# forsaken628/katib

Measured on AMD Instinct MI355X. Metric: darts_cifar10_search_wall_clock_s, lower is better.
Workload: dtype fp32; 1 GPU; model=darts-cnn-cifar10 supernet (b5: C=4, L=2, N=3, stem x1, 6 primitives + none), global_batch=128, per_gpu_batch=128, parallelism=dp1, epochs=2, steps_per_epoch=196, ops=hip, hip_graph=True, sync_bn=False, hessian=concurrent

## Files before the change

### katib_amd/csrc/hip/darts_bind.cpp

```cpp
#include <torch/extension.h>
#include <c10/hip/HIPStream.h>

#include "darts_ops.h"

using namespace katib_hip;
using at::Tensor;
using OptT = c10::optional<Tensor>;

namespace {

hipStream_t cur_stream() { return c10::hip::getCurrentHIPStream().stream(); }

void check_f32(const Tensor& t, const char* name) {
  TORCH_CHECK(t.is_cuda(), name, " must be a GPU tensor");
  TORCH_CHECK(t.scalar_type() == at::kFloat, name, " must be float32");
  TORCH_CHECK(t.is_contiguous(), name, " must be contiguous");
}

constexpr at::ScalarType kZType = kZbf16 ? at::kBFloat16 : at::kFloat;

void check_z(const Tensor& t, const char* name) {
  TORCH_CHECK(t.is_cuda(), name, " must be a GPU tensor");
  TORCH_CHECK(t.scalar_type() == kZType, name, " must be ", kZbf16 ? "bfloat16" : "float32",
              " (the per-op intermediates' storage type of this build)");
  TORCH_CHECK(t.is_contiguous(), name, " must be contiguous");
}

zt* zptr(const Tensor& t) { return reinterpret_cast<zt*>(t.data_ptr()); }

template <typename T>
T* ptr_or_null(const OptT& t) {
  return t.has_value() && t->defined() ? t->data_ptr<T>() : nullptr;
}

BNRef make_bn(const py::tuple& b, int C) {
  BNRef r{};
  TORCH_CHECK(b.size() == 8, "bn tuple has 8 fields");
  OptT sums = b[0].cast<OptT>(), rm = b[1].cast<OptT>(), rv = b[2].cast<OptT>();
  r.rep = b[6].cast<int>();
  r.rstride = b[7].cast<int>();
  TORCH_CHECK(r.rep >= 1 && r.rep <= kRep && r.rstride >= 2 * C, "bn replica layout");
  if (sums.has_value() && sums->defined()) {
    TORCH_CHECK(sums->scalar_type() == at::kDouble && sums->is_contiguous() &&
                    sums->numel() >= (int64_t)(r.rep - 1) * r.rstride + 2 * C,
                "bn sums must be f64 with rep x rstride doubles");
  }
  r.sums = ptr_or_null<double>(sums);
  r.rmean = ptr_or_null<float>(rm);
  r.rvar = ptr_or_null<float>(rv);
  r.inv_count = b[3].cast<float>();
  r.eval = b[4].cast<bool>() ? 1 : 0;
  r.eps = b[5].cast<float>();
  r.C = C;
  TORCH_CHECK(r.eval ? (r.rmean && r.rvar) : (r.sums != nullptr), "bn reference lacks its statistics");
  return r;
}

int64_t storage_doubles_after(const Tensor& t) {
  return (int64_t)(t.storage().nbytes() / sizeof(double)) - t.storage_offset();
}

int64_t gs_numel(const py::tuple& t) {
  return t[1].cast<Tensor>().numel();
}

GradSrc make_gs(const py::tuple& t, int C) {
  GradSrc g{};
  TORCH_CHECK(t.size() == 9, "grad-source tuple has 9 fields");
  Tensor gt = t[0].cast<Tensor>(), zt = t[1].cast<Tensor>();
  check_f32(gt, "g");
  check_z(zt, "z");
  g.g = gt.data_ptr<float>();
  g.z = zptr(zt);
  OptT s1 = t[2].cast<OptT>(), s2 = t[3].cast<OptT>();
  g.S1 = ptr_or_null<double>(s1);
  g.S2 = ptr_or_null<double>(s2);
  g.bn = make_bn(t[4].cast<py::tuple>(), C);
  g.eval = g.bn.eval;
  TORCH_CHECK(g.eval || (g.S1 && g.S2), "training-mode BN backward needs S1/S2 reductions");
  OptT w = t[5].cast<OptT>();
  g.w = ptr_or_null<float>(w);
  g.widx = t[6].cast<int>();
  g.rep = t[7].cast<int>();
  g.rstride = t[8].cast<int>();
  TORCH_CHECK(g.rep >= 1 && g.rep <= kRep, "replicas");
  if (!g.eval) {
    for (int k = 2; k <= 3; ++k) {
      Tensor sv = *t[k].cast<OptT>();
      TORCH_CHECK(sv.scalar_type() == at::kDouble &&
                      storage_doubles_after(sv) >= (int64_t)(g.rep - 1) * g.rstride + C,
                  "S1/S2 replicas exceed their buffer");
    }
  }
  return g;
}

struct CtrRing {
  unsigned* base = nullptr;
  int size = 0;
  int cursor = 0;
};
CtrRing g_ring[64];
bool g_selffold = false;

void set_selffold(bool on) { g_selffold = on; }

int cur_device() {
  int d = 0;
  TORCH_CHECK(hipGetDevice(&d) == hipSuccess, "hipGetDevice");
  return d;
}

void set_fold_counters(Tensor t) {
  TORCH_CHECK(t.is_cuda() && t.scalar_type() == at::kInt && t.is_contiguous() && t.numel() >= 4 * kFoldCtrSlot,
              "fold counters: contiguous int32 GPU tensor of >= 4 launch slots");
  const int d = t.get_device();
  TORCH_CHECK(d >= 0 && d < 64, "device index");
  g_ring[d] = CtrRing{reinterpret_cast<unsigned*>(t.data_ptr<int>()), (int)(t.numel() / kFoldCtrSlot), 0};
}

bool selffold_ready() { return g_selffold && g_ring[cur_device()].base != nullptr; }

void tail_begin(FoldTail& t) {
  t.nseg = 0;
  t.ctr = nullptr;
  if (!g_selffold) return;
  CtrRing& r = g_ring[cur_device()];
  if (!r.base) return;
  t.ctr = r.base + (size_t)r.cursor * kFoldCtrSlot;
  r.cursor = (r.cursor + 1) % r.size;
}

void tail_add(FoldTail& t, double* p, int n, int rs) {
  if (!t.ctr || !p) return;
  for (int s = 0; s < t.nseg; ++s)
    if (t.p[s] == p) {
      t.n[s] = std::max(t.n[s], n);
      return;
    }
  TORCH_CHECK(t.nseg < kTailSeg, "self-fold: too many reduction segments in one launch");
  t.p[t.nseg] = p;
  t.n[t.nseg] = n;
  t.rs[t.nseg] = rs;
  ++t.nseg;
}

void tail_close(FoldTail& t) {
  if (t.nseg == 0) t.ctr = nullptr;
}

int pick_chunk(int C, int per_channel_floats, int fixed_floats) {
  const int budget = 16384 - fixed_floats;
  int ch = C;
  while (ch > 1 && ch * per_channel_floats > budget) ch = (ch + 1) / 2;
  return std::max(ch, 1);
}

template <typename Bt>
void check_batch(const std::vector<py::tuple>& calls) {
  TORCH_CHECK(!calls.empty() && (int)calls.size() <= Bt::kCap, "batch of 1..", Bt::kCap, " edges");
}

#define SAME_SHAPE(b, fld) TORCH_CHECK(b.e[i].fld == b.e[0].fld, "edges in a batch must share " #fld)

static bool fill_dwpw(const py::tuple& t, DwPwFwdArgs& a, int64_t K, int64_t dil, int64_t S, int64_t pad, int nentries,
                      bool use_mfma) {
  Tensor x = t[0].cast<Tensor>(), dw = t[1].cast<Tensor>(), pw = t[2].cast<Tensor>();
  auto inbn = t[3].cast<c10::optional<py::tuple>>();
  Tensor d = t[4].cast<Tensor>(), z = t[5].cast<Tensor>();
  OptT stats = t[6].cast<OptT>();
  const bool has_inbn = t[3].cast<c10::optional<py::tuple>>().has_value();
  if (has_inbn) check_z(x, "x (previous stage z)");
  else check_f32(x, "x");
  check_f32(dw, "dw"); check_f32(pw, "pw"); check_z(d, "d"); check_z(z, "z");
  TORCH_CHECK(x.dim() == 4, "x must be NCHW");
  TORCH_CHECK((K == 3 || K == 5) && (dil == 1 || dil == 2) && (S == 1 || S == 2), "K in {3,5}, dil, S in {1,2}");
  const int N = x.size(0), C = x.size(1), H = x.size(2), W = x.size(3);
  const int Ho = z.size(2), Wo = z.size(3);
  TORCH_CHECK(dw.numel() == C * K * K && pw.numel() == C * C, "weight shapes");
  TORCH_CHECK(z.size(0) == N && z.size(1) == C && d.sizes() == z.sizes(), "output shapes");
  TORCH_CHECK(64 % Wo == 0 && Ho % (64 / Wo) == 0, "tile constraint: 64 % Wo == 0 and Ho % (64/Wo) == 0");
  TORCH_CHECK(C <= kMaxC, "C too large");
  TORCH_CHECK(Ho == (H + 2 * pad - dil * (K - 1) - 1) / S + 1, "output height mismatch");
  a.x = x.data_ptr(); a.dw = dw.data_ptr<float>(); a.pw = pw.data_ptr<float>();
  a.d = zptr(d); a.z = zptr(z); a.stats = ptr_or_null<double>(stats);
  if (a.stats) TORCH_CHECK(stats->scalar_type() == at::kDouble && stats->numel() >= kRep * 2 * C, "stats f64 [kRep][2C]");
  a.N = N; a.C = C; a.H = H; a.W = W; a.Ho = Ho; a.Wo = Wo; a.pad = pad;
  const int TR = 64 / Wo;
  const int IR = (TR - 1) * S + (K - 1) * dil + 1, IW = (Wo - 1) * S + (K - 1) * dil + 1;
  a.chunk = pick_chunk(C, IR * IW, C * 64 + 4 * C);
  if (C == 4 || C == 8 || C == 16) {
    int nb = std::max(1, std::min(Ho / 4, 2048 / std::max(N * nentries, 1)));
    auto band_bytes = [&](int b) {
      const int BR = (Ho + b - 1) / b;
      return (size_t)C * ((BR - 1) * S + (K - 1) * dil + 1) * (W + 2 * pad) * sizeof(float);
    };
    while (band_bytes(nb) > 65536 && nb < Ho) ++nb;
    a.chunk = nb;
  }
  a.use_mfma = (use_mfma && C % 16 == 0) ? 1 : 0;
  const bool prebn = inbn.has_value();
  if (prebn) a.inbn = make_bn(*inbn, C);
  a.variant = (((K == 5) * 4 + (dil == 2) * 2 + (S == 2)) * 4) + (prebn ? 2 : 0);
  return prebn;
}

void dwpw_fwd(std::vector<py::tuple> calls, int64_t K, int64_t dil, int64_t S, int64_t pad, bool use_mfma) {
  check_batch<DwPwFwdBatch>(calls);
  DwPwFwdBatch bt{};
  bt.n = calls.size();
  bool prebn = false;
  for (int i = 0; i < bt.n; ++i) {
    const bool pb = fill_dwpw(calls[i], bt.e[i], K, dil, S, pad, bt.n, use_mfma);
    if (i == 0) prebn = pb;
    TORCH_CHECK(pb == prebn, "edges in a batch must agree on the input BN");
    SAME_SHAPE(bt, N); SAME_SHAPE(bt, C); SAME_SHAPE(bt, H); SAME_SHAPE(bt, W);
  }
  tail_begin(bt.tail);
  for (int i = 0; i < bt.n; ++i) tail_add(bt.tail, bt.e[i].stats, 2 * bt.e[i].C, 2 * bt.e[i].C);
  tail_close(bt.tail);
  launch_dwpw_fwd(bt, K, dil, S, prebn, cur_stream());
}

static void fill_dwpw_multi(const std::vector<py::tuple>& calls, DwPwMultiBatch& bt, int64_t* kk, int64_t* dd,
                            int64_t* ss, int64_t* pp, bool* pre) {
  TORCH_CHECK(!calls.empty() && (int)calls.size() <= DwPwMultiBatch::kCap, "1..", DwPwMultiBatch::kCap, " entries");
  bt.n = calls.size();
  for (int i = 0; i < bt.n; ++i) {
    const py::tuple& t = calls[i];
    TORCH_CHECK(t.size() == 11, "dwpw_fwd_multi entry: (x, dw, pw, inbn, d, z, stats, K, dil, S, pad)");
    kk[i] = t[7].cast<int64_t>(); dd[i] = t[8].cast<int64_t>(); ss[i] = t[9].cast<int64_t>(); pp[i] = t[10].cast<int64_t>();
    pre[i] = fill_dwpw(t, bt.e[i], kk[i], dd[i], ss[i], pp[i], bt.n, true);
    SAME_SHAPE(bt, N); SAME_SHAPE(bt, C); SAME_SHAPE(bt, Ho); SAME_SHAPE(bt, Wo);
  }
  tail_begin(bt.tail);
  for (int i = 0; i < bt.n; ++i) tail_add(bt.tail, bt.e[i].stats, 2 * bt.e[i].C, 2 * bt.e[i].C);
  tail_close(bt.tail);
}

void dwpw_fwd_multi(std::vector<py::tuple> calls) {
  DwPwMultiBatch bt{};
  int64_t kk[DwPwMultiBatch::kCap], dd[DwPwMultiBatch::kCap], ss[DwPwMultiBatch::kCap], pp[DwPwMultiBatch::kCap];
  bool pre[DwPwMultiBatch::kCap];
  fill_dwpw_multi(calls, bt, kk, dd, ss, pp, pre);
  if (launch_dwpw_multi(bt, cur_stream())) return;
  for (int i = 0; i < bt.n; ++i) {
    DwPwFwdBatch one{};
    one.n = 1;
    one.tail = bt.tail;
    fill_dwpw(calls[i], one.e[0], kk[i], dd[i], ss[i], pp[i], 1, true);
    launch_dwpw_fwd(one, kk[i], dd[i], ss[i], pre[i], cur_stream());
  }
}

void pw_fwd(std::vector<py::tuple> calls, int64_t S) {
  check_batch<PwFwdBatch>(calls);
  PwFwdBatch bt{};
  bt.n = calls.size();
  for (int i = 0; i < bt.n; ++i) {
    const py::tuple& t = calls[i];
    Tensor x = t[0].cast<Tensor>(), pw = t[1].cast<Tensor>(), z = t[2].cast<Tensor>();
    OptT stats = t[3].cast<OptT>();
    const int co_off = t[4].cast<int>(), off = t[5].cast<int>();
    check_f32(x, "x"); check_f32(pw, "pw"); check_z(z, "z");
    const bool nm = x.dim() == 5;
    const int xnodes = nm ? x.size(0) : 1;
    const int N = nm ? x.size(1) : x.size(0), Cin = nm ? x.size(0) * x.size(2) : x.size(1);
    const int H = x.size(nm ? 3 : 2), W = x.size(nm ? 4 : 3);
    const int Cout = pw.size(0), Ho = z.size(2), Wo = z.size(3);
    TORCH_CHECK(pw.size(1) == Cin && co_off + Cout <= z.size(1) && z.size(0) == N, "pw shapes");
    TORCH_CHECK((Ho * Wo) % 64 == 0, "Ho*Wo must be a multiple of 64");
    TORCH_CHECK(Cin <= kMaxC && Cout <= kMaxC, "channels");
    PwFwdArgs& a = bt.e[i];
    a.x = x.data_ptr<float>(); a.pw = pw.data_ptr<float>(); a.z = zptr(z);
    a.stats = ptr_or_null<double>(stats);
    if (a.stats)
      TORCH_CHECK(stats->scalar_type() == at::kDouble && stats->numel() >= kRep * 2 * z.size(1), "stats [kRep][2Ctot]");
    a.N = N; a.Cin = Cin; a.Cout = Cout; a.CoutTotal = z.size(1); a.co_off = co_off;
    a.H = H; a.W = W; a.Ho = Ho; a.Wo = Wo; a.S = S; a.off = off; a.relu = 1; a.xnodes = xnodes;
    SAME_SHAPE(bt, N); SAME_SHAPE(bt, Cin); SAME_SHAPE(bt, Cout); SAME_SHAPE(bt, Ho); SAME_SHAPE(bt, Wo);
  }
  tail_begin(bt.tail);
  for (int i = 0; i < bt.n; ++i) tail_add(bt.tail, bt.e[i].stats, 2 * bt.e[i].CoutTotal, 2 * bt.e[i].CoutTotal);
  tail_close(bt.tail);
  launch_pw_fwd(bt, cur_stream());
}

static void fill_pool_fwd(const std::vector<py::tuple>& calls, int64_t S_all, PoolFwdBatch& bt) {
  check_batch<PoolFwdBatch>(calls);
  bt.n = calls.size();
  for (int i = 0; i < bt.n; ++i) {
    const py::tuple& t = calls[i];
    const int64_t S = S_all > 0 ? S_all : t[6].cast<int64_t>();
    TORCH_CHECK(S == 1 || S == 2, "pool stride must be 1 or 2");
    bt.e[i].S = (int)S;
    Tensor x = t[0].cast<Tensor>(), zavg = t[1].cast<Tensor>(), zmax = t[2].cast<Tensor>();
    OptT sa = t[3].cast<OptT>(), sm = t[4].cast<OptT>(), amax = t[5].cast<OptT>();
    check_f32(x, "x"); check_z(zavg, "zavg"); check_z(zmax, "zmax");
    PoolFwdArgs& a = bt.e[i];
    if (amax.has_value() && amax->defined()) {
      TORCH_CHECK(amax->scalar_type() == at::kByte && amax->numel() == zmax.numel(), "amax must be uint8 like zmax");
      a.amax = amax->data_ptr<uint8_t>();
    }
    a.x = x.data_ptr<float>(); a.zavg = zptr(zavg); a.zmax = zptr(zmax);
    a.stats_avg = ptr_or_null<double>(sa); a.stats_max = ptr_or_null<double>(sm);
    if (a.stats_avg) TORCH_CHECK(sa->scalar_type() == at::kDouble && sa->numel() >= kRep * 2 * x.size(1), "stats");
    if (a.stats_max) TORCH_CHECK(sm->scalar_type() == at::kDouble && sm->numel() >= kRep * 2 * x.size(1), "stats");
    a.N = x.size(0); a.C = x.size(1); a.H = x.size(2); a.W = x.size(3); a.Ho = zavg.size(2); a.Wo = zavg.size(3);
    TORCH_CHECK(a.Ho == (a.H - 1) / S + 1 && zmax.sizes() == zavg.sizes(), "pool shapes");
    SAME_SHAPE(bt, N); SAME_SHAPE(bt, C);
    if (S_all > 0) { SAME_SHAPE(bt, H); SAME_SHAPE(bt, W); }
  }
  tail_begin(bt.tail);
  for (int i = 0; i < bt.n; ++i) {
    tail_add(bt.tail, bt.e[i].stats_avg, 2 * bt.e[i].C, 2 * bt.e[i].C);
    tail_add(bt.tail, bt.e[i].stats_max, 2 * bt.e[i].C, 2 * bt.e[i].C);
  }
  tail_close(bt.tail);
}

static void pool_fwd_impl(std::vector<py::tuple> calls, int64_t S_all) {
  PoolFwdBatch bt{};
  fill_pool_fwd(calls, S_all, bt);
  if (S_all > 0) launch_pool_fwd(bt, S_all, cur_stream());
  else launch_pool_fwd_multi(bt, cur_stream());
}

void pool_fwd(std::vector<py::tuple> calls, int64_t S) { pool_fwd_impl(calls, S); }
void pool_fwd_multi(std::vector<py::tuple> calls) { pool_fwd_impl(calls, -1); }

void dwpw_pool_fwd_multi(std::vector<py::tuple> dcalls, std::vector<py::tuple> pcalls) {
  DwPwMultiBatch bt{};
  int64_t kk[DwPwMultiBatch::kCap], dd[DwPwMultiBatch::kCap], ss[DwPwMultiBatch::kCap], pp[DwPwMultiBatch::kCap];
  bool pre[DwPwMultiBatch::kCap];
  fill_dwpw_multi(dcalls, bt, kk, dd, ss, pp, pre);
  PoolFwdBatch pb{};
  fill_pool_fwd(pcalls, -1, pb);
  if (launch_dwpw_pool_multi(bt, pb, cur_stream())) return;
  dwpw_fwd_multi(dcalls);
  launch_pool_fwd_multi(pb, cur_stream());
}

void combine_fwd(std::vector<py::tuple> calls, OptT gamma, OptT beta, Tensor out, double momentum,
                 bool update_running, bool accumulate) {
  check_f32(out, "out");
  check_batch<CombineFwdBatch>(calls);
  CombineFwdBatch bt{};
  bt.n = calls.size();
  const int C = out.size(1);
  TORCH_CHECK(C <= kMaxC, "C too large");
  TORCH_CHECK((int64_t)2 * bt.n * kMaxOps * C * 4 <= 65536, "combine LDS budget exceeded");
  for (int e = 0; e < bt.n; ++e) {
    const py::tuple& t = calls[e];
    auto zs = t[0].cast<std::vector<Tensor>>();
    auto bns = t[1].cast<std::vector<py::tuple>>();
    auto widx = t[2].cast<std::vector<int64_t>>();
    OptT w = t[3].cast<OptT>();
    const int id_idx = t[4].cast<int>();
    OptT xid = t[5].cast<OptT>();
    auto upd = t[6].cast<std::vector<py::tuple>>();
    TORCH_CHECK(zs.size() == bns.size() && zs.size() == widx.size() && (int)zs.size() <= kMaxOps, "ops");
    CombineFwdArgs& a = bt.e[e];
    a.N = out.size(0); a.C = C; a.HW = out.size(2) * out.size(3);
    a.nops = zs.size();
    for (size_t k = 0; k < zs.size(); ++k) {
      check_z(zs[k], "z");
      TORCH_CHECK(zs[k].sizes() == out.sizes(), "combine input shape");
      a.z[k] = zptr(zs[k]);
      a.bn[k] = make_bn(bns[k], C);
      a.widx[k] = widx[k];
    }
    TORCH_CHECK((int)upd.size() <= kMaxUpd, "too many update-only BN layers");
    a.nupd = upd.size();
    for (size_t k = 0; k < upd.size(); ++k) a.upd[k] = make_bn(upd[k], C);
    a.w = ptr_or_null<float>(w); a.id_idx = id_idx; a.xid = ptr_or_null<float>(xid);
    if (a.xid) {
      check_f32(*xid, "xid");
      TORCH_CHECK(xid->sizes() == out.sizes(), "identity shape");
    }
    a.gamma = ptr_or_null<float>(gamma); a.beta = ptr_or_null<float>(beta);
    a.out = out.data_ptr<float>(); a.momentum = momentum; a.update_running = update_running;
    a.accumulate = accumulate;
  }
  launch_combine_fwd(bt, cur_stream());
}

void combine_bwd_reduce(std::vector<py::tuple> calls) {
  check_batch<CombineBwdBatch>(calls);
  CombineBwdBatch bt{};
  bt.n = calls.size();
  for (int i = 0; i < bt.n; ++i) {
    const py::tuple& t = calls[i];
    Tensor dout = t[0].cast<Tensor>();
    auto zs = t[1].cast<std::vector<Tensor>>();
    auto bns = t[2].cast<std::vector<py::tuple>>();
    OptT xid = t[3].cast<OptT>();
    Tensor red = t[4].cast<Tensor>();
    auto widx = t[5].cast<std::vector<int64_t>>();
    const int id_idx = t[6].cast<int>();
    OptT gw = t[7].cast<OptT>();
    check_f32(dout, "dout");
    TORCH_CHECK(red.scalar_type() == at::kDouble, "red must be f64");
    CombineBwdArgs& a = bt.e[i];
    a.N = dout.size(0); a.C = dout.size(1); a.HW = dout.size(2) * dout.size(3);
    a.nops = zs.size();
    a.rstride = (a.nops + 1) * a.C + 1;
    TORCH_CHECK(a.nops <= kMaxOps && red.numel() >= (int64_t)kRep * a.rstride, "red size [kRep][(nops+1)C+1]");
    for (int k = 0; k < a.nops; ++k) {
      TORCH_CHECK(zs[k].sizes() == dout.sizes(), "z shape");
      check_z(zs[k], "z");
      a.z[k] = zptr(zs[k]);
      a.bn[k] = make_bn(bns[k], a.C);
    }
    a.dout = dout.data_ptr<float>(); a.xid = ptr_or_null<float>(xid); a.red = red.data_ptr<double>();
    a.gw = ptr_or_null<double>(gw); a.id_idx = id_idx;
    if (a.gw) {
      TORCH_CHECK(gw->scalar_type() == at::kDouble && gw->numel() % kRep == 0, "gw must be f64 [kRep][nw]");
      a.gwstride = gw->numel() / kRep;
      TORCH_CHECK((int)widx.size() == a.nops, "widx per op");
      for (int k = 0; k < a.nops; ++k) {
        TORCH_CHECK(widx[k] >= 0 && widx[k] < a.gwstride, "widx out of range");
        a.widx[k] = widx[k];
      }
      TORCH_CHECK(id_idx < a.gwstride, "id_idx out of range");
    }
    SAME_SHAPE(bt, N); SAME_SHAPE(bt, C); SAME_SHAPE(bt, HW);
  }
  tail_begin(bt.tail);
  for (int i = 0; i < bt.n; ++i) {
    tail_add(bt.tail, bt.e[i].red, bt.e[i].rstride, bt.e[i].rstride);
    tail_add(bt.tail, bt.e[i].gw, bt.e[i].gwstride, bt.e[i].gwstride);
  }
  tail_close(bt.tail);
  launch_combine_bwd_reduce(bt, cur_stream());
}

void check_grad_sink(const OptT& gW, int64_t numel, int64_t gstride) {
  if (!gW.has_value() || !gW->defined()) return;
  TORCH_CHECK(gW->scalar_type() == at::kFloat && gW->is_contiguous() && gW->numel() == numel, "gW shape");
  TORCH_CHECK(gstride == 0 || (gstride >= numel && (int64_t)(gW->storage().nbytes() / sizeof(float)) -
                                                           gW->storage_offset() >= (kRep - 1) * gstride + numel),
              "gW replicas exceed their buffer");
}

void pw_bwd(std::vector<py::tuple> calls, int64_t S, int64_t mode, bool need_dx) {
  check_batch<PwBwdBatch>(calls);
  PwBwdBatch bt{};
  bt.n = calls.size();
  for (int i = 0; i < bt.n; ++i) {
    const py::tuple& t = calls[i];
    py::tuple gs = t[0].cast<py::tuple>();
    Tensor pw = t[1].cast<Tensor>();
    OptT ain = t[2].cast<OptT>();
    Tensor x = t[3].cast<Tensor>();
    OptT dd = t[4].cast<OptT>(), gx = t[5].cast<OptT>(), gW = t[6].cast<OptT>();
    const int co_off = t[7].cast<int>(), off = t[8].cast<int>();
    const int64_t gstride = t[9].cast<int64_t>();
    const bool overwrite = t.size() > 10 && t[10].cast<bool>();
    check_f32(pw, "pw");
    if (mode != 0) check_f32(x, "x");
    PwBwdArgs& a = bt.e[i];
    a.overwrite = overwrite;
    TORCH_CHECK(!overwrite || (mode == 1 && S == 1 && off == 0), "gx overwrite needs the stride-1 full-coverage form");
    const int Cout = pw.size(0), Cin = pw.size(1);
    Tensor g = gs[0].cast<Tensor>();
    a.N = g.size(0); a.CoutTotal = g.size(1); a.Ho = g.size(2); a.Wo = g.size(3);
    a.gs = make_gs(gs, a.CoutTotal);
    a.Cin = Cin; a.Cout = Cout; a.co_off = co_off; a.S = S; a.off = off; a.mode = mode;
    a.need_dx = need_dx;
    const bool nm = mode != 0 && x.dim() == 5;
    a.xnodes = nm ? x.size(0) : 1;
    a.H = x.size(nm ? 3 : 2); a.W = x.size(nm ? 4 : 3);
    if (mode != 0) {
      TORCH_CHECK(x.numel() == (int64_t)a.N * Cin * a.H * a.W && (!nm || x.size(1) == a.N),
                  "pw_bwd: x must be [N][Cin][H][W] or node-major [nodes][N][Cin/nodes][H][W]");
      if (gx.has_value() && gx->defined()) TORCH_CHECK(gx->sizes() == x.sizes(), "pw_bwd: gx must have the shape of x");
    }
    TORCH_CHECK(Cin * Cout <= 8192, "pw_bwd supports Cin*Cout <= 8192");
    TORCH_CHECK((a.Ho * a.Wo) % 64 == 0, "Ho*Wo % 64");
    a.pw = pw.data_ptr<float>(); a.x = mode != 0 ? x.data_ptr<float>() : nullptr;
    if (ain.has_value() && ain->defined()) check_z(*ain, "ain (depthwise output d)");
    a.ain = ain.has_value() && ain->defined() ? zptr(*ain) : nullptr;
    a.dd = ptr_or_null<float>(dd); a.gx = ptr_or_null<float>(gx);
    a.gW = ptr_or_null<float>(gW);
    if (mode == 0) {
      TORCH_CHECK(a.ain && (!need_dx || a.dd), "mode 0 needs ain (and dd)");
    } else {
      TORCH_CHECK(!need_dx || a.gx, "mode 1 needs gx");
    }
    check_grad_sink(gW, (int64_t)Cin * Cout, gstride);
    a.gstride = gstride;
    SAME_SHAPE(bt, N); SAME_SHAPE(bt, Cin); SAME_SHAPE(bt, Cout); SAME_SHAPE(bt, Ho); SAME_SHAPE(bt, Wo);
  }
  launch_pw_bwd(bt, cur_stream());
}

void dw_bwd_fill(std::vector<py::tuple>& calls, DwBwdBatch& bt, const int64_t* Ks, const int64_t* dils,
                 const int64_t* Ss, bool& prebn);

void dw_bwd(std::vector<py::tuple> calls, int64_t K, int64_t dil, int64_t S, int64_t pad) {
  check_batch<DwBwdBatch>(calls);
  DwBwdBatch bt{};
  int64_t Ks[DwBwdBatch::kCap], Ds[DwBwdBatch::kCap], Ss[DwBwdBatch::kCap];
  for (int i = 0; i < DwBwdBatch::kCap; ++i) Ks[i] = K, Ds[i] = dil, Ss[i] = S;
  TORCH_CHECK(pad == (K - 1) / 2 * dil, "dw_bwd padding must be 'same'");
  bool prebn = false;
  dw_bwd_fill(calls, bt, Ks, Ds, Ss, prebn);
  tail_close(bt.tail);
  launch_dw_bwd(bt, K, dil, S, prebn, cur_stream());
}

void dw_bwd_multi(std::vector<py::tuple> calls) {
  check_batch<DwBwdBatch>(calls);
  DwBwdBatch bt{};
  int64_t Ks[DwBwdBatch::kCap], Ds[DwBwdBatch::kCap], Ss[DwBwdBatch::kCap];
  for (size_t i = 0; i < calls.size(); ++i) {
    TORCH_CHECK(calls[i].size() == 10 || calls[i].size() == 12,
                "dw_bwd_multi entry: (x, inbn, dw, dd, gout, gW, red, gstride, overwrite, K[, dil, S])");
    Ks[i] = calls[i][9].cast<int64_t>();
    Ds[i] = calls[i].size() == 12 ? calls[i][10].cast<int64_t>() : 1;
    Ss[i] = calls[i].size() == 12 ? calls[i][11].cast<int64_t>() : 1;
    TORCH_CHECK((Ks[i] == 3 || Ks[i] == 5) && (Ds[i] == 1 || Ds[i] == 2) && (Ss[i] == 1 || Ss[i] == 2),
                "K in {3, 5}, dil and S in {1, 2}");
  }
  bool prebn = false;
  dw_bwd_fill(calls, bt, Ks, Ds, Ss, prebn);
  for (int i = 0; i < bt.n; ++i) {
    TORCH_CHECK(prebn || bt.e[i].overwrite, "dw_bwd_multi: input-gradient entries must own (overwrite) their output");
    TORCH_CHECK(!prebn || (Ds[i] == 1 && Ss[i] == 1), "dw_bwd_multi: input-BN entries are stride-1 separable stages");
    bt.e[i].variant = dw_bwd_variant((int)Ks[i], (int)Ds[i], (int)Ss[i], prebn);
  }
  for (int i = 0; i < bt.n; ++i)
    for (int j = i + 1; j < bt.n; ++j) TORCH_CHECK(bt.e[i].gout != bt.e[j].gout, "dw_bwd_multi entries share an output");
  tail_close(bt.tail);
  if (launch_dw_bwd_multi(bt, cur_stream())) return;
  for (int v = 0; v < 16; ++v) {
    DwBwdBatch one{};
    one.tail = bt.tail;
    for (int i = 0; i < bt.n; ++i)
      if (bt.e[i].variant == v) one.e[one.n++] = bt.e[i];
    if (one.n) launch_dw_bwd(one, dw_variant_k(v), dw_variant_dil(v), dw_variant_s(v), prebn, cur_stream());
  }
}

void dw_bwd_fill(std::vector<py::tuple>& calls, DwBwdBatch& bt, const int64_t* Ks, const int64_t* dils,
                 const int64_t* Ss, bool& prebn) {
  bt.n = calls.size();
  bool has_gw = false;
  for (int i = 0; i < bt.n; ++i) {
    const py::tuple& t = calls[i];
    const int64_t K = Ks[i], dil = dils[i], S = Ss[i], pad = (K - 1) / 2 * dil;
    Tensor x = t[0].cast<Tensor>();
    auto inbn = t[1].cast<c10::optional<py::tuple>>();
    Tensor dw = t[2].cast<Tensor>(), dd = t[3].cast<Tensor>(), gout = t[4].cast<Tensor>();
    OptT gW = t[5].cast<OptT>(), red = t[6].cast<OptT>();
    const int64_t gstride = t[7].cast<int64_t>();
    const bool overwrite = t[8].cast<bool>();
    if (inbn.has_value()) check_z(x, "x (stage-1 z)");
    else check_f32(x, "x");
    check_f32(dw, "dw"); check_f32(dd, "dd"); check_f32(gout, "gout");
    DwBwdArgs& a = bt.e[i];
    a.N = x.size(0); a.C = x.size(1); a.H = x.size(2); a.W = x.size(3); a.Ho = dd.size(2); a.Wo = dd.size(3);
    TORCH_CHECK(64 % a.Wo == 0 && a.Ho % (64 / a.Wo) == 0, "tile constraint");
    TORCH_CHECK(a.H == a.Ho * S && a.W == a.Wo * S, "dw_bwd needs H == Ho*S");
    TORCH_CHECK(gout.sizes() == x.sizes(), "gout shape");
    TORCH_CHECK(dw.numel() == a.C * K * K && dd.size(1) == a.C, "dw_bwd weight / grad shapes");
    a.x = x.data_ptr(); a.dw = dw.data_ptr<float>(); a.dd = dd.data_ptr<float>();
    a.gout = gout.data_ptr<float>(); a.gW = ptr_or_null<float>(gW); a.red = ptr_or_null<double>(red);
    check_grad_sink(gW, (int64_t)a.C * K * K, gstride);
    a.gstride = gstride;
    a.overwrite = overwrite;
    if (a.red) TORCH_CHECK(red->scalar_type() == at::kDouble && red->numel() >= kRep * 2 * a.C, "red [kRep][2C]");
    a.pad = pad;
    if (i == 0) {
      prebn = inbn.has_value();
      has_gw = a.gW != nullptr;
    }
    TORCH_CHECK(inbn.has_value() == prebn, "edges in a batch must agree on the input BN");
    TORCH_CHECK((a.gW != nullptr) == has_gw, "edges in a batch must agree on weight-gradient sinks");
    TORCH_CHECK(!(prebn && overwrite), "overwrite applies to the input-gradient (non-BN) form");
    const int TR = 64 / a.Wo, r = (K - 1) / 2 * dil, h = (r + S - 1) / S, OR = TR + 2 * h;
    const int IR = (TR - 1) * S + (K - 1) * dil + 1, IW = (a.Wo - 1) * S + (K - 1) * dil + 1;
    a.chunk = pick_chunk(a.C, OR * a.Wo + IR * IW, 4 * a.C + (a.gW ? a.C * (int)(K * K) : 0));
    if (prebn) a.inbn = make_bn(*inbn, a.C);
    SAME_SHAPE(bt, N); SAME_SHAPE(bt, C); SAME_SHAPE(bt, Ho); SAME_SHAPE(bt, Wo);
  }
  tail_begin(bt.tail);
  if (prebn)
    for (int i = 0; i < bt.n; ++i) tail_add(bt.tail, bt.e[i].red, 2 * bt.e[i].C, 2 * bt.e[i].C);
}

static void pool_bwd_impl(std::vector<py::tuple> calls, int64_t S_all) {
  check_batch<PoolBwdBatch>(calls);
  PoolBwdBatch bt{};
  bt.n = calls.size();
  for (int i = 0; i < bt.n; ++i) {
    const py::tuple& t = calls[i];
    const int64_t S = S_all > 0 ? S_all : t[9].cast<int64_t>();
    TORCH_CHECK(S == 1 || S == 2, "pool stride must be 1 or 2");
    bt.e[i].S = (int)S;
    auto ga = t[0].cast<c10::optional<py::tuple>>(), gm = t[1].cast<c10::optional<py::tuple>>();
    Tensor x = t[2].cast<Tensor>();
    OptT dout_id = t[3].cast<OptT>(), w = t[4].cast<OptT>();
    const int id_idx = t[5].cast<int>();
    Tensor gx = t[6].cast<Tensor>();
    OptT amax = t[7].cast<OptT>();
    check_f32(x, "x"); check_f32(gx, "gx");
    PoolBwdArgs& a = bt.e[i];
    a.N = x.size(0); a.C = x.size(1); a.H = x.size(2); a.W = x.size(3);
    a.Ho = (a.H - 1) / S + 1; a.Wo = (a.W - 1) / S + 1;
    TORCH_CHECK(a.Ho * a.Wo <= 8192, "pool_bwd stages one output plane in LDS (Ho*Wo <= 8192)");
    TORCH_CHECK(gx.sizes() == x.sizes(), "gx shape");
    TORCH_CHECK(!gm.has_value() || (amax.has_value() && amax->defined() && amax->scalar_type() == at::kByte &&
                                    amax->numel() == (int64_t)a.N * a.C * a.Ho * a.Wo),
                "max-pool backward needs the uint8 argmax from pool_fwd");
    if (amax.has_value() && amax->defined()) a.amax = amax->data_ptr<uint8_t>();
    if (ga.has_value()) a.ga = make_gs(*ga, a.C);
    if (gm.has_value()) a.gm = make_gs(*gm, a.C);
    a.x = x.data_ptr<float>(); a.dout_id = ptr_or_null<float>(dout_id); a.w = ptr_or_null<float>(w);
    if (a.dout_id) TORCH_CHECK(dout_id->sizes() == x.sizes(), "identity gradient shape");
    a.id_idx = id_idx; a.gx = gx.data_ptr<float>();
    a.overwrite = t[8].cast<bool>();
    if (S_all <= 0 && t.size() > 10) {
      auto ex = t[10].cast<std::vector<Tensor>>();
      TORCH_CHECK(ex.size() <= 4, "pool_bwd: at most 4 extra gradient parts");
      a.nextra = ex.size();
      for (size_t j = 0; j < ex.size(); ++j) {
        check_f32(ex[j], "extra");
        TORCH_CHECK(ex[j].sizes() == gx.sizes(), "extra gradient part shape");
        TORCH_CHECK(ex[j].data_ptr() != gx.data_ptr(), "extra part aliases gx");
        a.extra[j] = ex[j].data_ptr<float>();
      }
    }
    SAME_SHAPE(bt, N); SAME_SHAPE(bt, C);
    if (S_all > 0) { SAME_SHAPE(bt, H); SAME_SHAPE(bt, W); }
  }
  for (int i = 0; i < bt.n; ++i)
    for (int j = i + 1; j < bt.n; ++j) TORCH_CHECK(bt.e[i].gx != bt.e[j].gx, "pool_bwd entries share a gx buffer");
  if (S_all > 0) launch_pool_bwd(bt, S_all, cur_stream());
  else launch_pool_bwd_multi(bt, cur_stream());
}

void pool_bwd(std::vector<py::tuple> calls, int64_t S) { pool_bwd_impl(calls, S); }

bool edge_bwd(std::vector<py::tuple> calls) {
  check_batch<EdgeBwdBatch>(calls);
  EdgeBwdBatch bt{};
  bt.n = calls.size();
  const int Ks[4] = {3, 5, 3, 5};
  for (int i = 0; i < bt.n; ++i) {
    const py::tuple& t = calls[i];
    TORCH_CHECK(t.size() == 11, "edge_bwd entry: (x, gx, overwrite, convs, ga, gm, amax, dout_id, w, id_idx, S)");
    Tensor x = t[0].cast<Tensor>(), gx = t[1].cast<Tensor>();
    check_f32(x, "x"); check_f32(gx, "gx");
    TORCH_CHECK(x.dim() == 4 && gx.sizes() == x.sizes(), "gx shape");
    EdgeBwdArgs& a = bt.e[i];
    a.x = x.data_ptr<float>(); a.gx = gx.data_ptr<float>(); a.overwrite = t[2].cast<bool>();
    a.S = t[10].cast<int>();
    TORCH_CHECK(a.S == 1 || a.S == 2, "stride");
    a.N = x.size(0); a.C = x.size(1); a.H = x.size(2); a.W = x.size(3);
    a.Ho = (a.H - 1) / a.S + 1; a.Wo = (a.W - 1) / a.S + 1;
    auto convs = t[3].cast<std::vector<py::object>>();
    TORCH_CHECK(convs.size() == 4, "4 conv slots");
    for (int v = 0; v < 4; ++v) {
      if (convs[v].is_none()) continue;
      py::tuple c = convs[v].cast<py::tuple>();
      Tensor dw = c[0].cast<Tensor>(), dd = c[1].cast<Tensor>();
      OptT gW = c[2].cast<OptT>();
      const int64_t gstride = c[3].cast<int64_t>();
      check_f32(dw, "dw"); check_f32(dd, "dd");
      TORCH_CHECK(dw.numel() == a.C * Ks[v] * Ks[v], "dw shape");
      TORCH_CHECK(dd.dim() == 4 && dd.size(0) == a.N && dd.size(1) == a.C && dd.size(2) == a.Ho && dd.size(3) == a.Wo,
                  "dd shape");
      check_grad_sink(gW, (int64_t)a.C * Ks[v] * Ks[v], gstride);
      a.dw[v] = dw.data_ptr<float>(); a.dd[v] = dd.data_ptr<float>(); a.gW[v] = ptr_or_null<float>(gW);
      a.gstride[v] = gstride;
      a.conv_mask |= 1 << v;
    }
    auto ga = t[4].cast<c10::optional<py::tuple>>(), gm = t[5].cast<c10::optional<py::tuple>>();
    OptT amax = t[6].cast<OptT>(), dout_id = t[7].cast<OptT>(), w = t[8].cast<OptT>();
    if (ga.has_value()) {
      a.ga = make_gs(*ga, a.C);
      TORCH_CHECK(gs_numel(*ga) == (int64_t)a.N * a.C * a.Ho * a.Wo, "avg-pool gradient source shape");
    }
    if (gm.has_value()) {
      a.gm = make_gs(*gm, a.C);
      TORCH_CHECK(gs_numel(*gm) == (int64_t)a.N * a.C * a.Ho * a.Wo, "max-pool gradient source shape");
      TORCH_CHECK(amax.has_value() && amax->defined() && amax->scalar_type() == at::kByte &&
                      amax->numel() == (int64_t)a.N * a.C * a.Ho * a.Wo,
                  "max-pool backward needs the uint8 argmax from pool_fwd");
      a.amax = amax->data_ptr<uint8_t>();
    }
    a.dout_id = ptr_or_null<float>(dout_id); a.w = ptr_or_null<float>(w); a.id_idx = t[9].cast<int>();
    if (a.dout_id) {
      check_f32(*dout_id, "dout_id");
      TORCH_CHECK(dout_id->sizes() == x.sizes() && a.S == 1, "identity gradient shape");
    }
    SAME_SHAPE(bt, N); SAME_SHAPE(bt, C);
  }
  for (int i = 0; i < bt.n; ++i)
    for (int j = i + 1; j < bt.n; ++j) TORCH_CHECK(bt.e[i].gx != bt.e[j].gx, "edge_bwd entries share a gx buffer");
  return launch_edge_bwd(bt, cur_stream());
}
void pool_bwd_multi(std::vector<py::tuple> calls) { pool_bwd_impl(calls, -1); }

void fold_rows(Tensor buf) {
  check_f32(buf, "buf");
  TORCH_CHECK(buf.dim() == 2, "buf must be [rows][n]");
  FoldArgs a{};
  a.buf = buf.data_ptr<float>();
  a.rows = buf.size(0);
  a.n = buf.size(1);
  launch_fold_rows(a, cur_stream());
}

void fold_f64(std::vector<py::tuple> segs) {
  TORCH_CHECK(!segs.empty() && (int)segs.size() <= kMaxSeg, "1..kMaxSeg segments");
  FoldF64Args a{};
  a.nseg = segs.size();
  for (int k = 0; k < a.nseg; ++k) {
    Tensor t = segs[k][0].cast<Tensor>();
    int n = segs[k][1].cast<int>(), rs = segs[k][2].cast<int>();
    TORCH_CHECK(t.is_cuda() && t.scalar_type() == at::kDouble && t.is_contiguous(), "fold segment must be f64");
    TORCH_CHECK(n >= 1 && rs >= n && t.numel() >= (int64_t)(kRep - 1) * rs + n, "fold segment size");
    a.p[k] = t.data_ptr<double>();
    a.n[k] = n;
    a.rstride[k] = rs;
    a.total += n;
  }
  launch_fold_f64(a, cur_stream());
}

}

void register_xgmi(py::module& m);
void register_conv(py::module& m);
void register_transformer(py::module& m);
void register_batchnorm(py::module& m);
void register_mlp(py::module& m);
void register_stem(py::module& m);
void register_enas(py::module& m);
void register_dwconv(py::module& m);
void register_darts_optim(py::module& m);
void register_darts_head(py::module& m);
void register_resnet(py::module& m);

PYBIND11_MODULE(TORCH_EXTENSION_NAME, m) {
  m.doc() = "katib_amd HIP kernels for gfx950 (DARTS edge ops, implicit-GEMM conv, transformer, xGMI all-reduce)";
  m.def("dwpw_fwd", &dwpw_fwd);
  m.def("pw_fwd", &pw_fwd);
  m.def("pool_fwd", &pool_fwd);
  m.def("combine_fwd", &combine_fwd);
  m.def("combine_bwd_reduce", &combine_bwd_reduce);
  m.def("pw_bwd", &pw_bwd);
  m.def("dw_bwd", &dw_bwd);
  m.def("dw_bwd_multi", &dw_bwd_multi, "separable second-stage depthwise backward of mixed kernel size in one launch");
  m.def("pool_bwd", &pool_bwd);
  m.def("dwpw_fwd_multi", &dwpw_fwd_multi, "mixed (K, dil, S) dw-pw entries of one node stage in one launch");
  m.def("pool_fwd_multi", &pool_fwd_multi, "stride-1 and stride-2 pools in one launch");
  m.def("dwpw_pool_fwd_multi", &dwpw_pool_fwd_multi, "a node's stage-1 dw-pw entries and its pools in one launch");
  m.def("pool_bwd_multi", &pool_bwd_multi, "stride-1 and stride-2 pool backward in one launch");
  m.def("edge_bwd", &edge_bwd, "whole input gradient of a node's edges (convs, pools, identity) in one launch");
  m.def("set_max_blocks", &set_max_blocks);
  m.def("stamps_arm", [](int kind, int call, torch::Tensor buf) {
    TORCH_CHECK(!buf.defined() || kind == 0 || (buf.is_cuda() && buf.scalar_type() == torch::kInt64 &&
                                               buf.is_contiguous() && buf.numel() >= 65536 * 8),
                "stamps_arm: int64 CUDA buffer of >= 65536 * 8 entries");
    stamps_arm(kind, call, kind == 0 ? nullptr : reinterpret_cast<unsigned long long*>(buf.data_ptr<int64_t>()));
  }, "diagnostic build: phase-stamp the call-th launch of kind (StampKind) into buf[wg * 8 + phase]");
  m.def("stamps_compiled", &stamps_compiled);
  m.def("fold_rows", &fold_rows);
  m.def("fold_f64", &fold_f64);
  m.def("set_fold_counters", &set_fold_counters, "register the current device's self-fold counter ring (int32, zeroed)");
  m.def("selffold_ready", &selffold_ready, "launches on the current device fold their own f64 replicas");
  m.def("set_selffold", &set_selffold, "turn self-folding launches on / off (default off: measured slower)");
  m.attr("REP") = kRep;
  m.attr("ZBF16") = kZbf16;
  m.def("max_blocks", &max_blocks);
  register_xgmi(m);
  register_conv(m);
  register_transformer(m);
  register_batchnorm(m);
  register_enas(m);
  register_dwconv(m);
  register_mlp(m);
  register_stem(m);
  register_darts_optim(m);
  register_darts_head(m);
  register_resnet(m);
}
```

### katib_amd/csrc/hip/darts_ops.h

```cpp
#pragma once
#include <hip/hip_runtime.h>
#include <hip/hip_bf16.h>

namespace katib_hip {

#ifdef KATIB_DARTS_ZBF16
typedef __hip_bfloat16 zt;
constexpr bool kZbf16 = true;
#else
typedef float zt;
constexpr bool kZbf16 = false;
#endif
typedef float zf4 __attribute__((ext_vector_type(4)));

__device__ __forceinline__ float z2f(float v) { return v; }
__device__ __forceinline__ float z2f(__hip_bfloat16 v) { return __bfloat162float(v); }
__device__ __forceinline__ void zput(float* p, float v) { *p = v; }
__device__ __forceinline__ void zput(__hip_bfloat16* p, float v) { *p = __float2bfloat16(v); }
__device__ __forceinline__ zf4 zld4(const float* p) { return *reinterpret_cast<const zf4*>(p); }
__device__ __forceinline__ zf4 zld4(const __hip_bfloat16* p) {
  const uint2 u = *reinterpret_cast<const uint2*>(p);
  return zf4{__uint_as_float(u.x << 16), __uint_as_float(u.x & 0xffff0000u), __uint_as_float(u.y << 16),
             __uint_as_float(u.y & 0xffff0000u)};
}
__device__ __forceinline__ void zst4(float* p, zf4 v) { *reinterpret_cast<zf4*>(p) = v; }
__device__ __forceinline__ void zst4(__hip_bfloat16* p, zf4 v) {
  __hip_bfloat16 b[4] = {__float2bfloat16(v.x), __float2bfloat16(v.y), __float2bfloat16(v.z), __float2bfloat16(v.w)};
  *reinterpret_cast<uint2*>(p) = *reinterpret_cast<const uint2*>(b);
}

__host__ __device__ __forceinline__ size_t plane_off(int n, int c, int N, int C, int nodes, size_t HW) {
  if (nodes <= 1) return ((size_t)n * C + c) * HW;
  const int Cn = C / nodes, k = c / Cn;
  return (((size_t)k * N + n) * Cn + (c - k * Cn)) * HW;
}

constexpr int kMaxOps = 8;
constexpr int kMaxUpd = 4;
constexpr int kMaxC = 256;
#ifndef KATIB_HIP_REP
#define KATIB_HIP_REP 32
#endif
constexpr int kRep = KATIB_HIP_REP;

struct BNRef {
  const double* sums;
  float* rmean;
  float* rvar;
  float inv_count;
  float eps;
  int eval;
  int C;
  int rep;
  int rstride;
};

struct GradSrc {
  const float* g;
  const zt* z;
  const double* S1;
  const double* S2;
  BNRef bn;
  const float* w;
  int widx;
  int eval;
  int rep;
  int rstride;
};

struct DwPwFwdArgs {
  const void* x;
  BNRef inbn; const float* dw; const float* pw;
  zt* d; zt* z; double* stats;
  int N, C, H, W, Ho, Wo, pad, chunk, use_mfma;
  int variant;
  int nblk;
  int vout = 0;
};

struct PwFwdArgs {
  const void* x;
  const float* pw; zt* z; double* stats;
  int N, Cin, Cout, CoutTotal, co_off, H, W, Ho, Wo, S, off;
  int relu;
  int xnodes;
};

struct PoolFwdArgs {
  const float* x; zt* zavg; zt* zmax; double* stats_avg; double* stats_max; unsigned char* amax;
  int N, C, H, W, Ho, Wo;
  int S, nblk;
};

struct CombineFwdArgs {
  const zt* z[kMaxOps]; BNRef bn[kMaxOps]; int widx[kMaxOps]; int nops;
  BNRef upd[kMaxUpd]; int nupd;
  const float* w; int id_idx; const float* xid; const float* gamma; const float* beta;
  float* out; int N, C, HW; float momentum; int update_running; int accumulate;
};

struct CombineBwdArgs {
  const float* dout; const zt* z[kMaxOps]; BNRef bn[kMaxOps]; int nops;
  const float* xid; double* red; int N, C, HW;
  double* gw; int widx[kMaxOps]; int id_idx;
  int rstride, gwstride;
};

struct PwBwdArgs {
  GradSrc gs; const float* pw; const zt* ain; const float* x; float* dd; float* gx; float* gW;
  int gstride;
  int N, Cin, Cout, CoutTotal, co_off, H, W, Ho, Wo, S, off, mode, need_dx;
  int overwrite;
  int xnodes;
};

struct DwBwdArgs {
  const void* x;
  BNRef inbn; const float* dw; const float* dd; float* gout; float* gW; double* red;
  int gstride;
  int N, C, H, W, Ho, Wo, pad, chunk;
  int overwrite;
  int variant, nbands, nblk;
  int vin = 0;
};
constexpr int dw_bwd_variant(int K, int dil, int S, bool prebn) {
  return (((K == 5) * 4 + (dil == 2) * 2 + (S == 2)) << 1) | (prebn ? 1 : 0);
}
constexpr int dw_variant_k(int v) { return (v >> 3) & 1 ? 5 : 3; }
constexpr int dw_variant_dil(int v) { return (v >> 2) & 1 ? 2 : 1; }
constexpr int dw_variant_s(int v) { return (v >> 1) & 1 ? 2 : 1; }
constexpr bool dw_variant_prebn(int v) { return v & 1; }

struct FoldArgs {
  float* buf; int n; int rows;
};

constexpr int kMaxSeg = 128;
struct FoldF64Args {
  double* p[kMaxSeg]; int n[kMaxSeg]; int rstride[kMaxSeg]; int nseg; int total;
};

struct PoolBwdArgs {
  GradSrc ga; GradSrc gm; const float* x; const float* dout_id; const float* w; int id_idx; float* gx;
  const unsigned char* amax;
  const float* extra[4]; int nextra;
  int overwrite;
  int N, C, H, W, Ho, Wo;
  int S;
};

constexpr int kTailSeg = 16;
constexpr int kFoldShards = 32;
constexpr int kFoldCtrStride = 32;
constexpr int kFoldCtrSlot = (1 + kFoldShards) * kFoldCtrStride;
struct FoldTail {
  unsigned* ctr;
  int nseg;
  double* p[kTailSeg];
  int n[kTailSeg];
  int rs[kTailSeg];
};

template <typename A, int M>
struct Batch {
  A e[M];
  int n;
  FoldTail tail;
  static constexpr int kCap = M;
};
using DwPwFwdBatch = Batch<DwPwFwdArgs, 16>;
using CombineFwdBatch = Batch<CombineFwdArgs, 4>;
using PwFwdBatch = Batch<PwFwdArgs, 32>;
using PoolFwdBatch = Batch<PoolFwdArgs, 16>;
using CombineBwdBatch = Batch<CombineBwdArgs, 8>;
using PwBwdBatch = Batch<PwBwdArgs, 32>;
using DwBwdBatch = Batch<DwBwdArgs, 40>;
using PoolBwdBatch = Batch<PoolBwdArgs, 16>;
using DwPwMultiBatch = Batch<DwPwFwdArgs, 40>;

struct EdgeBwdArgs {
  const float* x; float* gx; int overwrite;
  const float* dw[4]; const float* dd[4]; float* gW[4]; int gstride[4]; int conv_mask;
  GradSrc ga; GradSrc gm; const unsigned char* amax;
  const float* dout_id; const float* w; int id_idx;
  int N, C, H, W, Ho, Wo, S, nb, nblk;
};
using EdgeBwdBatch = Batch<EdgeBwdArgs, 4>;
constexpr size_t kKernargMax = 24576;
static_assert(sizeof(EdgeBwdBatch) <= kKernargMax, "edge_bwd batch exceeds the kernarg budget");
static_assert(sizeof(DwPwFwdBatch) <= kKernargMax && sizeof(CombineFwdBatch) <= kKernargMax &&
                  sizeof(PwFwdBatch) <= kKernargMax && sizeof(PoolFwdBatch) <= kKernargMax &&
                  sizeof(CombineBwdBatch) <= kKernargMax && sizeof(PwBwdBatch) <= kKernargMax &&
                  sizeof(DwBwdBatch) <= kKernargMax && sizeof(PoolBwdBatch) <= kKernargMax &&
                  sizeof(DwPwMultiBatch) <= kKernargMax,
              "kernel argument batches exceed the kernarg budget");

void launch_dwpw_fwd(const DwPwFwdBatch& b, int K, int dil, int S, bool prebn, hipStream_t st);
void launch_dw_bwd(const DwBwdBatch& b, int K, int dil, int S, bool prebn, hipStream_t st);
bool launch_dw_bwd_multi(DwBwdBatch b, hipStream_t st);
void launch_pw_fwd(const PwFwdBatch& b, hipStream_t st);
void launch_pool_fwd(const PoolFwdBatch& b, int S, hipStream_t st);
void launch_pool_bwd(const PoolBwdBatch& b, int S, hipStream_t st);
bool launch_dwpw_multi(DwPwMultiBatch b, hipStream_t st);
void launch_pool_fwd_multi(PoolFwdBatch b, hipStream_t st);
struct PoolFwdEntries {
  PoolFwdArgs e[PoolFwdBatch::kCap];
  int n;
};
static_assert(sizeof(DwPwMultiBatch) + sizeof(PoolFwdEntries) <= kKernargMax, "kernarg budget");
bool launch_dwpw_pool_multi(DwPwMultiBatch b, const PoolFwdBatch& pb, hipStream_t st);
void launch_pool_bwd_multi(const PoolBwdBatch& b, hipStream_t st);
void launch_combine_fwd(const CombineFwdBatch& b, hipStream_t st);
bool launch_edge_bwd(EdgeBwdBatch b, hipStream_t st);
void launch_combine_bwd_reduce(const CombineBwdBatch& b, hipStream_t st);
void launch_pw_bwd(const PwBwdBatch& b, hipStream_t st);
int max_blocks();
void launch_fold_rows(const FoldArgs& a, hipStream_t st);
void launch_fold_f64(const FoldF64Args& a, hipStream_t st);
void set_max_blocks(int n);
void stamps_arm(int kind, int call, unsigned long long* buf);
bool stamps_compiled();

}
```

### katib_amd/csrc/hip/darts_ops_dev.h

```cpp
#pragma once
#include <hip/hip_runtime.h>

#include <algorithm>
#include <cmath>
#include <cstdint>
#include <cstdlib>

#include "darts_ops.h"

namespace katib_hip {

int max_blocks();

#ifdef KATIB_HIP_STAMPS
static __device__ unsigned long long* g_stamps = nullptr;
#define KSTAMP(k)                                                                          \
  do {                                                                                     \
    unsigned long long* _sp = g_stamps;                                                    \
    if (_sp != nullptr && threadIdx.x == 0) {                                              \
      const unsigned _wg = blockIdx.y * gridDim.x + blockIdx.x;                            \
      if (_wg < 65536u) _sp[(size_t)_wg * 8 + (k)] = __builtin_amdgcn_s_memrealtime();     \
    }                                                                                      \
  } while (0)
bool stamp_take(int kind);
unsigned long long* stamp_buffer();
#define KSTAMP_ARM(kind, st)                                                               \
  const bool _stamp_armed = stamp_take(kind);                                              \
  if (_stamp_armed) {                                                                      \
    static unsigned long long* _on;                                                        \
    _on = stamp_buffer();                                                                  \
    (void)hipMemcpyToSymbolAsync(HIP_SYMBOL(g_stamps), &_on, sizeof(_on), 0, hipMemcpyHostToDevice, st); \
  }
#define KSTAMP_DISARM(st)                                                                  \
  if (_stamp_armed) {                                                                      \
    static unsigned long long* _off = nullptr;                                             \
    (void)hipMemcpyToSymbolAsync(HIP_SYMBOL(g_stamps), &_off, sizeof(_off), 0, hipMemcpyHostToDevice, st); \
  }
#else
#define KSTAMP(k)
#define KSTAMP_ARM(kind, st)
#define KSTAMP_DISARM(st)
#endif
enum StampKind { kStampDwBwd = 1, kStampDwPw = 2, kStampPoolBwd = 3, kStampPoolFwd = 4, kStampCombineFwd = 5,
                 kStampCombineBwd = 6, kStampPwBwd = 7 };
#define KEEP_WEIGHT_READS_LOCAL() asm volatile("" ::: "memory")
__host__ __device__ constexpr int plane_head_floats(int C) { return (C * 25 + C * C + 3) & ~3; }
__host__ __device__ constexpr int dwb_head_floats(int C) { return (2 * C * 25 + 3) & ~3; }
__host__ __device__ constexpr int lds_pitch(int w) {
  return (((w + 3) & ~3) >> 2) & 1 ? ((w + 3) & ~3) : ((w + 3) & ~3) + 4;
}
int vec_mask();

__device__ __forceinline__ void sum_replicas(const double* p, int rep, int rs, int off2, double& s, double& s2) {
  s = 0.0;
  s2 = 0.0;
  for (int r0 = 0; r0 < rep; r0 += 8) {
    double a[8], b[8];
#pragma unroll
    for (int u = 0; u < 8; ++u) {
      const bool ok = r0 + u < rep;
      a[u] = ok ? p[(size_t)(r0 + u) * rs] : 0.0;
      b[u] = ok ? p[(size_t)(r0 + u) * rs + off2] : 0.0;
    }
#pragma unroll
    for (int u = 0; u < 8; ++u) {
      s += a[u];
      s2 += b[u];
    }
  }
}

__device__ __forceinline__ void bn_moments(const BNRef& b, int c, double& m, double& v) {
  double s, s2;
  sum_replicas(b.sums + c, b.rep, b.rstride, b.C, s, s2);
  m = s * (double)b.inv_count;
  v = s2 * (double)b.inv_count - m * m;
  if (v < 0) v = 0;
}

__device__ __forceinline__ void bn_coeffs(const BNRef& b, int c, float& mean, float& invstd) {
  if (b.eval) {
    mean = b.rmean[c];
    invstd = rsqrtf(b.rvar[c] + b.eps);
  } else {
    double m, v;
    bn_moments(b, c, m, v);
    mean = (float)m;
    invstd = rsqrtf((float)v + b.eps);
  }
}

__device__ __forceinline__ void gs_means(const GradSrc& gs, int c, float& m1, float& m2) {
  if (gs.eval) {
    m1 = m2 = 0.f;
    return;
  }
  double s1 = 0.0, s2 = 0.0;
  if (gs.rep == 1) {
    s1 = gs.S1[c];
    s2 = gs.S2[c];
  } else {
    sum_replicas(gs.S1 + c, gs.rep, gs.rstride, (int)(gs.S2 - gs.S1), s1, s2);
  }
  m1 = (float)(s1 * (double)gs.bn.inv_count);
  m2 = (float)(s2 * (double)gs.bn.inv_count);
}

__device__ __forceinline__ void coop_pair_sums(const double* p1, const double* p2, int rep, int rs, int n,
                                               double scale, float* o1, float* o2, bool bn, float eps) {
  const int tid = threadIdx.x, j = tid & 15;
  for (int cb = 0; cb < n; cb += 16) {
    const int ch = cb + (tid >> 4);
    double s = 0.0, s2 = 0.0;
    if (ch < n) {
#pragma unroll 2
      for (int r = j; r < rep; r += 16) {
        s += p1[(size_t)r * rs + ch];
        s2 += p2[(size_t)r * rs + ch];
      }
    }
#pragma unroll
    for (int o = 8; o > 0; o >>= 1) {
      s += __shfl_xor(s, o, 64);
      s2 += __shfl_xor(s2, o, 64);
    }
    if (ch < n && j == 0) {
      if (bn) {
        const double m = s * scale;
        double v = s2 * scale - m * m;
        if (v < 0) v = 0;
        o1[ch] = (float)m;
        o2[ch] = rsqrtf((float)v + eps);
      } else {
        o1[ch] = (float)(s * scale);
        o2[ch] = (float)(s2 * scale);
      }
    }
  }
}

__device__ __forceinline__ void bn_coeffs_coop(const BNRef& b, int c0, int n, float* mean, float* inv) {
  if (b.eval || b.rep == 1) {
    for (int c = threadIdx.x; c < n; c += blockDim.x) bn_coeffs(b, c0 + c, mean[c], inv[c]);
    return;
  }
  coop_pair_sums(b.sums + c0, b.sums + b.C + c0, b.rep, b.rstride, n, (double)b.inv_count, mean, inv, true, b.eps);
}

__device__ __forceinline__ void gs_means_coop(const GradSrc& gs, int c0, int n, float* m1, float* m2) {
  if (gs.eval || gs.rep == 1) {
    for (int c = threadIdx.x; c < n; c += blockDim.x) gs_means(gs, c0 + c, m1[c], m2[c]);
    return;
  }
  coop_pair_sums(gs.S1 + c0, gs.S2 + c0, gs.rep, gs.rstride, n, (double)gs.bn.inv_count, m1, m2, false, 0.f);
}

struct BnRaw {
  double s, s2;
  float rm, rv;
};
__device__ __forceinline__ BnRaw bn_raw(const BNRef& b, int c) {
  BnRaw r{0.0, 0.0, 0.f, 1.f};
  if (b.eval) {
    r.rm = b.rmean[c];
    r.rv = b.rvar[c];
  } else if (b.rep == 1) {
    r.s = b.sums[c];
    r.s2 = b.sums[b.C + c];
  } else {
    sum_replicas(b.sums + c, b.rep, b.rstride, b.C, r.s, r.s2);
  }
  return r;
}
__device__ __forceinline__ void bn_finish(const BNRef& b, const BnRaw& r, float& mean, float& invstd) {
  if (b.eval) {
    mean = r.rm;
    invstd = rsqrtf(r.rv + b.eps);
  } else {
    const double m = r.s * (double)b.inv_count;
    double v = r.s2 * (double)b.inv_count - m * m;
    if (v < 0) v = 0;
    mean = (float)m;
    invstd = rsqrtf((float)v + b.eps);
  }
}

__device__ __forceinline__ void bn_gs_coop(const GradSrc& gs, int c0, int n, float* mean, float* inv, float* m1,
                                           float* m2) {
  const BNRef& b = gs.bn;
  if (32 * n > (int)blockDim.x) {
    for (int c = threadIdx.x; c < n; c += blockDim.x) bn_coeffs(b, c0 + c, mean[c], inv[c]);
    gs_means_coop(gs, c0, n, m1, m2);
    return;
  }
  const int grp = threadIdx.x >> 4, j = threadIdx.x & 15;
  const bool stats = grp < n, act = grp < 2 * n;
  const int ch = c0 + (stats ? grp : grp - n);
  double s = 0.0, s2 = 0.0;
  if (act && stats && !b.eval) {
    for (int r = j; r < b.rep; r += 16) {
      s += b.sums[(size_t)r * b.rstride + ch];
      s2 += b.sums[(size_t)r * b.rstride + b.C + ch];
    }
  } else if (act && !stats && !gs.eval) {
    const int rs = gs.rep == 1 ? 0 : gs.rstride;
    const size_t off2 = gs.S2 - gs.S1;
    for (int r = j; r < gs.rep; r += 16) {
      s += gs.S1[(size_t)r * rs + ch];
      s2 += gs.S1[(size_t)r * rs + off2 + ch];
    }
  }
#pragma unroll
  for (int o = 8; o > 0; o >>= 1) {
    s += __shfl_xor(s, o, 64);
    s2 += __shfl_xor(s2, o, 64);
  }
  if (act && j == 0) {
    const int k = ch - c0;
    if (stats) {
      if (b.eval) {
        mean[k] = b.rmean[ch];
        inv[k] = rsqrtf(b.rvar[ch] + b.eps);
      } else {
        const double m = s * (double)b.inv_count;
        double v = s2 * (double)b.inv_count - m * m;
        if (v < 0) v = 0;
        mean[k] = (float)m;
        inv[k] = rsqrtf((float)v + b.eps);
      }
    } else {
      m1[k] = gs.eval ? 0.f : (float)(s * (double)b.inv_count);
      m2[k] = gs.eval ? 0.f : (float)(s2 * (double)b.inv_count);
    }
  }
}

__device__ __forceinline__ int rep_slot() { return blockIdx.x % kRep; }

__device__ __forceinline__ float wave_sum(float v) {
#pragma unroll
  for (int o = 32; o > 0; o >>= 1) v += __shfl_xor(v, o, 64);
  return v;
}

template <int H, int D>
__device__ __forceinline__ void reduce_scatter_level(float* acc, int lane) {
  if constexpr (H >= 1) {
    const bool up = (lane & D) != 0;
#pragma unroll
    for (int i = 0; i < H; ++i) {
      const float keep = up ? acc[i + H] : acc[i];
      const float send = up ? acc[i] : acc[i + H];
      acc[i] = keep + __shfl_xor(send, D, 64);
    }
    reduce_scatter_level<H / 2, D / 2>(acc, lane);
  }
}

template <int M>
__device__ __forceinline__ float wave_reduce_scatter(float* acc) {
  const int lane = threadIdx.x & 63;
  reduce_scatter_level<M / 2, 32>(acc, lane);
  float v = acc[0];
#pragma unroll
  for (int d = 32 / M; d >= 1; d >>= 1) v += __shfl_xor(v, d, 64);
  return v;
}

template <int M>
__device__ __forceinline__ int wave_scatter_index(int lane) {
  int idx = 0;
#pragma unroll
  for (int h = M / 2, d = 32; h >= 1; h >>= 1, d >>= 1)
    if (lane & d) idx += h;
  return idx;
}

template <int M>
__device__ __forceinline__ void wave_sums_to_lds(float* acc, float* dst, int lane) {
  if constexpr (M > 0) {
    constexpr int P = M >= 64 ? 64 : (M >= 32 ? 32 : (M >= 16 ? 16 : (M >= 8 ? 8 : (M >= 4 ? 4 : (M >= 2 ? 2 : 1)))));
    const float s = wave_reduce_scatter<P>(acc);
    if ((lane & (64 / P - 1)) == 0) atomicAdd(dst + wave_scatter_index<P>(lane), s);
    wave_sums_to_lds<M - P>(acc + P, dst + P, lane);
  }
}

__device__ __forceinline__ double wave_sum_d(double v) {
#pragma unroll
  for (int o = 32; o > 0; o >>= 1) v += __shfl_xor(v, o, 64);
  return v;
}

template <bool Z>
__device__ __forceinline__ float xval(const void* p, size_t i) {
  if constexpr (Z) return z2f(static_cast<const zt*>(p)[i]);
  else return static_cast<const float*>(p)[i];
}
template <bool Z>
__device__ __forceinline__ float4 xval4(const void* p, size_t i) {
  if constexpr (Z) {
    const zf4 t = zld4(static_cast<const zt*>(p) + i);
    return make_float4(t.x, t.y, t.z, t.w);
  } else {
    return *reinterpret_cast<const float4*>(static_cast<const float*>(p) + i);
  }
}

__device__ __forceinline__ void fold_tail(const FoldTail& t) {
  __shared__ int s_last;
  asm volatile("s_waitcnt vmcnt(0)" ::: "memory");
  __syncthreads();
  if (threadIdx.x == 0) {
    const unsigned total = gridDim.x * gridDim.y * gridDim.z;
    const unsigned L = blockIdx.x + gridDim.x * (blockIdx.y + gridDim.y * blockIdx.z);
    const unsigned sh = L % kFoldShards;
    const unsigned cnt = total / kFoldShards + (sh < total % kFoldShards ? 1u : 0u);
    unsigned* cs = t.ctr + (1 + sh) * kFoldCtrStride;
    int last = 0;
    if (__hip_atomic_fetch_add(cs, 1u, __ATOMIC_RELAXED, __HIP_MEMORY_SCOPE_AGENT) == cnt - 1) {
      __hip_atomic_store(cs, 0u, __ATOMIC_RELAXED, __HIP_MEMORY_SCOPE_AGENT);
      const unsigned nsh = total < (unsigned)kFoldShards ? total : (unsigned)kFoldShards;
      last = __hip_atomic_fetch_add(t.ctr, 1u, __ATOMIC_RELAXED, __HIP_MEMORY_SCOPE_AGENT) == nsh - 1;
    }
    s_last = last;
  }
  __syncthreads();
  if (!s_last) return;
  int tot = 0;
  for (int s = 0; s < t.nseg; ++s) tot += t.n[s];
  for (int g = threadIdx.x; g < tot; g += blockDim.x) {
    int s = 0, i = g;
    while (i >= t.n[s]) i -= t.n[s++];
    double* p = t.p[s] + i;
    const size_t rs = t.rs[s];
    double v[kRep - 1];
#pragma unroll
    for (int r = 1; r < kRep; ++r)
      v[r - 1] = __hip_atomic_exchange(p + r * rs, 0.0, __ATOMIC_RELAXED, __HIP_MEMORY_SCOPE_AGENT);
    double acc = 0.0;
#pragma unroll
    for (int r = 0; r < kRep - 1; ++r) acc += v[r];
    __hip_atomic_fetch_add(p, acc, __ATOMIC_RELAXED, __HIP_MEMORY_SCOPE_AGENT);
  }
  if (threadIdx.x == 0) __hip_atomic_store(t.ctr, 0u, __ATOMIC_RELAXED, __HIP_MEMORY_SCOPE_AGENT);
}

__device__ __forceinline__ void fr2_pair(const float* plane, int W, int Wo, int off, int p, float& v0, float& v1) {
  const int oy = p / Wo, ox = p - oy * Wo;
  const float4 v = *reinterpret_cast<const float4*>(plane + (size_t)(2 * oy + off) * W + 2 * ox);
  v0 = fmaxf(off ? v.y : v.x, 0.f);
  v1 = fmaxf(off ? v.w : v.z, 0.f);
}

__device__ __forceinline__ float bn_bwd_val(const GradSrc& gs, size_t i, float mean, float inv, float wk, float m1,
                                           float m2) {
  float zh = (z2f(gs.z[i]) - mean) * inv;
  float g = gs.g[i];
  return wk * inv * (g - m1 - zh * m2);
}

__device__ __forceinline__ void wave_lds_sync() {
  __builtin_amdgcn_fence(__ATOMIC_RELEASE, "wavefront");
  __builtin_amdgcn_wave_barrier();
  __builtin_amdgcn_fence(__ATOMIC_ACQUIRE, "wavefront");
}

static inline int per_edge_blocks(int tiles, int n) { return std::max(1, std::min(tiles, max_blocks() / std::max(n, 1))); }
static inline int channel_groups(int N, int C, int n) { return std::max(1, std::min(N, max_blocks() / (C * std::max(n, 1)))); }

}
```

### katib_amd/csrc/hip/darts_ops_dwb.hip

```cpp
#include "darts_ops_dev.h"

namespace katib_hip {

template <int K, int DIL, int S, bool PREBN>
__global__ void __launch_bounds__(256) dw_bwd_kernel(DwBwdBatch bt) {
  const DwBwdArgs& a = bt.e[blockIdx.y];
  constexpr int P = 64, KK = K * K;
  const int C = a.C, H = a.H, W = a.W, Ho = a.Ho, Wo = a.Wo;
  const int TR = P / Wo;
  const int tiles = Ho / TR;
  const int ntiles = a.N * tiles;
  const int pad = a.pad;
  const int r = (K - 1) / 2 * DIL;
  const int h = (r + S - 1) / S;
  const int OR = TR + 2 * h;
  const int IR = (TR - 1) * S + (K - 1) * DIL + 1;
  const int IW = (Wo - 1) * S + (K - 1) * DIL + 1;
  extern __shared__ __attribute__((aligned(16))) float smem[];
  float* sDD = smem;
  float* sIn = sDD + a.chunk * OR * Wo;
  float* sMean = sIn + a.chunk * IR * IW;
  float* sInv = sMean + C;
  float* sRed = sInv + C;
  float* sGW = sRed + 2 * C;
  const int tid = threadIdx.x, wave = tid >> 6, lane = tid & 63;
  for (int c = tid; c < C; c += 256) {
    if (PREBN) bn_coeffs(a.inbn, c, sMean[c], sInv[c]);
    sRed[c] = 0.f;
    sRed[C + c] = 0.f;
  }
  if (a.gW)
    for (int i = tid; i < C * KK; i += 256) sGW[i] = 0.f;
  __syncthreads();
  const int own_in = TR * S;
  const int nq = own_in * W;
  for (int t = blockIdx.x; t < ntiles; t += gridDim.x) {
    const int n = t / tiles, oy0 = (t % tiles) * TR;
    const int iy0 = oy0 * S - pad;
    const size_t xin = (size_t)n * C * H * W;
    const float* ddn = a.dd + (size_t)n * C * Ho * Wo;
    for (int c0 = 0; c0 < C; c0 += a.chunk) {
      const int cn = min(a.chunk, C - c0);
      #pragma unroll 4
      for (int i = tid; i < cn * OR * Wo; i += 256) {
        int cc = i / (OR * Wo), rr = (i / Wo) % OR, q = i % Wo;
        int oy = oy0 - h + rr;
        sDD[i] = (oy >= 0 && oy < Ho) ? ddn[((size_t)(c0 + cc) * Ho + oy) * Wo + q] : 0.f;
      }
      if (a.gW) {
        #pragma unroll 4
        for (int i = tid; i < cn * IR * IW; i += 256) {
          int cc = i / (IR * IW), rr = (i / IW) % IR, q = i % IW;
          int iy = iy0 + rr, ix = -pad + q, c = c0 + cc;
          float v = 0.f;
          if (iy >= 0 && iy < H && ix >= 0 && ix < W) {
            v = xval<PREBN>(a.x, xin + ((size_t)c * H + iy) * W + ix);
            if (PREBN) v = (v - sMean[c]) * sInv[c];
            v = fmaxf(v, 0.f);
          }
          sIn[i] = v;
        }
      }
      __syncthreads();
      if (a.gW) {
        for (int job = tid; job < cn * KK; job += 256) {
          const int cc = job / KK, tap = job % KK, ky = tap / K, kx = tap % K;
          const float* dd = sDD + (cc * OR + h) * Wo;
          const float* in = sIn + (cc * IR + ky * DIL) * IW + kx * DIL;
          float s = 0.f;
          for (int ty = 0; ty < TR; ++ty)
            for (int tx = 0; tx < Wo; ++tx) s += dd[ty * Wo + tx] * in[ty * S * IW + tx * S];
          sGW[(c0 + cc) * KK + tap] += s;
        }
      }
      const int qspan = (nq < 256 && 256 % nq == 0) ? nq : 256;
      const int G = 256 / qspan;
      for (int q0 = 0; q0 < nq; q0 += qspan) {
        const int q = q0 + tid % qspan;
        const int cg = __builtin_amdgcn_readfirstlane(tid / qspan);
        const int rr = q / W, ix = q - rr * W;
        const int iy = oy0 * S + rr;
        const bool ok = q < nq && iy < H;
        int srow[K], ocol[K];
        float mrow[K], mcol[K];
#pragma unroll
        for (int k = 0; k < K; ++k) {
          int ty = iy + pad - k * DIL;
          int oy = ty >= 0 ? ty / S : -1;
          bool v = ok && ty >= 0 && (ty % S) == 0 && oy < Ho;
          srow[k] = v ? oy - (oy0 - h) : 0;
          mrow[k] = v ? 1.f : 0.f;
          int tx = ix + pad - k * DIL;
          int ox = tx >= 0 ? tx / S : -1;
          bool u = ok && tx >= 0 && (tx % S) == 0 && ox < Wo;
          ocol[k] = u ? ox : 0;
          mcol[k] = u ? 1.f : 0.f;
        }
        for (int cc = cg; cc < cn; cc += G) {
          const int c = c0 + cc;
          const float* wk = a.dw + c * KK;
          const float* dd = sDD + cc * OR * Wo;
          float ga = 0.f;
#pragma unroll
          for (int ky = 0; ky < K; ++ky) {
            float rowacc = 0.f;
#pragma unroll
            for (int kx = 0; kx < K; ++kx) rowacc += mcol[kx] * wk[ky * K + kx] * dd[srow[ky] * Wo + ocol[kx]];
            ga += mrow[ky] * rowacc;
          }
          const size_t xi = ((size_t)(n * C + c) * H + iy) * W + ix;
          if (PREBN) {
            float g = 0.f, gy = 0.f;
            if (ok) {
              float y = (xval<true>(a.x, xi) - sMean[c]) * sInv[c];
              g = y > 0.f ? ga : 0.f;
              gy = g * y;
              a.gout[xi] = g;
            }
            if (a.red) {
              g = wave_sum(g);
              gy = wave_sum(gy);
              if (lane == 0) {
                atomicAdd(sRed + c, g);
                atomicAdd(sRed + C + c, gy);
              }
            }
          } else if (ok) {
            const float gm = xval<false>(a.x, xi) > 0.f ? ga : 0.f;
            if (a.overwrite) a.gout[xi] = gm;
            else if (gm != 0.f) a.gout[xi] += gm;
          }
        }
      }
      __syncthreads();
    }
  }
  if (PREBN && a.red)
    for (int i = tid; i < 2 * C; i += 256) atomicAdd(a.red + rep_slot() * 2 * C + i, (double)sRed[i]);
  if (a.gW)
    for (int i = tid; i < C * KK; i += 256) atomicAdd(a.gW + (size_t)rep_slot() * a.gstride + i, sGW[i]);
  if (bt.tail.ctr) fold_tail(bt.tail);
}

template <int S, bool V4 = false>
__device__ __forceinline__ void pool_bwd_body(const PoolBwdArgs& a, const int bx) {
  const int C = a.C, H = a.H, W = a.W, Ho = a.Ho, Wo = a.Wo, HWo = Ho * Wo;
  const int nc = bx, c = nc % C;
  const size_t ob = (size_t)nc * HWo;
  extern __shared__ __attribute__((aligned(16))) float smem[];
  float* sGa = smem;
  float* sGm = smem + HWo;
  unsigned char* sArg = (unsigned char*)(smem + 2 * HWo);
  __shared__ float sCo[8];
  KSTAMP(0);
  if (threadIdx.x < 64) {
    const int grp = threadIdx.x >> 4, j = threadIdx.x & 15;
    const GradSrc& gs = grp & 1 ? a.gm : a.ga;
    const bool on = gs.z != nullptr, stats = grp < 2;
    const BNRef& b = gs.bn;
    double s = 0.0, s2 = 0.0;
    if (on && stats && !b.eval) {
      for (int r = j; r < b.rep; r += 16) {
        s += b.sums[(size_t)r * b.rstride + c];
        s2 += b.sums[(size_t)r * b.rstride + b.C + c];
      }
    } else if (on && !stats && !gs.eval) {
      const int rep = gs.rep, rs = gs.rep == 1 ? 0 : gs.rstride;
      const size_t off2 = gs.S2 - gs.S1;
      for (int r = j; r < rep; r += 16) {
        s += gs.S1[(size_t)r * rs + c];
        s2 += gs.S1[(size_t)r * rs + off2 + c];
      }
    }
#pragma unroll
    for (int o = 8; o > 0; o >>= 1) {
      s += __shfl_xor(s, o, 64);
      s2 += __shfl_xor(s2, o, 64);
    }
    if (j == 0) {
      float* o = sCo + 4 * (grp & 1) + (stats ? 0 : 2);
      if (!on) {
        o[0] = 0.f;
        o[1] = stats ? 1.f : 0.f;
      } else if (stats) {
        if (b.eval) {
          o[0] = b.rmean[c];
          o[1] = rsqrtf(b.rvar[c] + b.eps);
        } else {
          const double m = s * (double)b.inv_count;
          double v = s2 * (double)b.inv_count - m * m;
          if (v < 0) v = 0;
          o[0] = (float)m;
          o[1] = rsqrtf((float)v + b.eps);
        }
      } else {
        o[0] = gs.eval ? 0.f : (float)(s * (double)gs.bn.inv_count);
        o[1] = gs.eval ? 0.f : (float)(s2 * (double)gs.bn.inv_count);
      }
    }
  }
  __syncthreads();
  KSTAMP(1);
  const float ma = sCo[0], ia = sCo[1], a1 = a.ga.z ? sCo[2] : 0.f, a2 = a.ga.z ? sCo[3] : 0.f;
  const float mm = sCo[4], im = sCo[5], m1 = a.gm.z ? sCo[6] : 0.f, m2 = a.gm.z ? sCo[7] : 0.f;
  const float wa = a.ga.w ? a.ga.w[a.ga.widx] : 0.f;
  const float wm = a.gm.w ? a.gm.w[a.gm.widx] : 0.f;
  const float wid = (a.w && a.id_idx >= 0) ? a.w[a.id_idx] : 0.f;
  if constexpr (V4) {
    typedef float f4 __attribute__((ext_vector_type(4)));
    const float* gsrc = a.ga.z ? a.ga.g : a.gm.g;
    for (int o4 = threadIdx.x * 4; o4 < HWo; o4 += 1024) {
      const f4 g = *reinterpret_cast<const f4*>(gsrc + ob + o4);
      if (a.ga.z) {
        const f4 z = zld4(a.ga.z + ob + o4);
        const f4 d = wa * ia * (g - a1 - ((z - ma) * ia) * a2);
#pragma unroll
        for (int t = 0; t < 4; ++t) {
          const int o = o4 + t, oy = o / Wo, ox = o - oy * Wo;
          const int y0 = max(oy * S - 1, 0), y1 = min(oy * S + 1, H - 1);
          const int x0 = max(ox * S - 1, 0), x1 = min(ox * S + 1, W - 1);
          sGa[o] = d[t] / (float)((y1 - y0 + 1) * (x1 - x0 + 1));
        }
      } else {
        *reinterpret_cast<f4*>(sGa + o4) = f4{0.f, 0.f, 0.f, 0.f};
      }
      if (a.gm.z) {
        const f4 z = zld4(a.gm.z + ob + o4);
        *reinterpret_cast<f4*>(sGm + o4) = wm * im * (g - m1 - ((z - mm) * im) * m2);
        *reinterpret_cast<unsigned*>(sArg + o4) = *reinterpret_cast<const unsigned*>(a.amax + ob + o4);
      } else {
        *reinterpret_cast<f4*>(sGm + o4) = f4{0.f, 0.f, 0.f, 0.f};
        *reinterpret_cast<unsigned*>(sArg + o4) = 0xffffffffu;
      }
    }
    __syncthreads();
    KSTAMP(2);
    const size_t pb = (size_t)nc * H * W;
    for (int q4 = threadIdx.x * 4; q4 < H * W; q4 += 1024) {
      f4 g = {0.f, 0.f, 0.f, 0.f};
      if (a.dout_id) g = wid * *reinterpret_cast<const f4*>(a.dout_id + pb + q4);
#pragma unroll
      for (int j = 0; j < 4; ++j)
        if (j < a.nextra) g += *reinterpret_cast<const f4*>(a.extra[j] + pb + q4);
      const int iy = q4 / W, ix0 = q4 - iy * W;
      if constexpr (S == 1) {
        float wa[3][6], wm[3][6];
        unsigned char wt[3][6];
#pragma unroll
        for (int r = 0; r < 3; ++r) {
          const int oy = iy - 1 + r;
          const bool rok = oy >= 0 && oy < Ho;
          const int o = (rok ? oy : 0) * Wo + ix0;
          const f4 ga4 = *reinterpret_cast<const f4*>(sGa + o), gm4 = *reinterpret_cast<const f4*>(sGm + o);
          const unsigned t4 = *reinterpret_cast<const unsigned*>(sArg + o);
#pragma unroll
          for (int k = 0; k < 4; ++k) {
            wa[r][k + 1] = rok ? ga4[k] : 0.f;
            wm[r][k + 1] = rok ? gm4[k] : 0.f;
            wt[r][k + 1] = rok ? (unsigned char)(t4 >> (8 * k)) : 255;
          }
          const bool lok = rok && ix0 > 0, hok = rok && ix0 + 4 < Wo;
          wa[r][0] = lok ? sGa[o - 1] : 0.f;
          wm[r][0] = lok ? sGm[o - 1] : 0.f;
          wt[r][0] = lok ? sArg[o - 1] : 255;
          wa[r][5] = hok ? sGa[o + 4] : 0.f;
          wm[r][5] = hok ? sGm[o + 4] : 0.f;
          wt[r][5] = hok ? sArg[o + 4] : 255;
        }
#pragma unroll
        for (int t = 0; t < 4; ++t) {
          float v = 0.f;
#pragma unroll
          for (int r = 0; r < 3; ++r)
#pragma unroll
            for (int cx = 0; cx < 3; ++cx) {
              v += wa[r][t + cx];
              if (wt[r][t + cx] == (2 - r) * 3 + (2 - cx)) v += wm[r][t + cx];
            }
          g[t] += v;
        }
        f4* dst = reinterpret_cast<f4*>(a.gx + pb + q4);
        *dst = a.overwrite ? g : *dst + g;
        continue;
      }
      if constexpr (S == 2) {
        float wa[2][3], wm[2][3];
        unsigned char wt[2][3];
        const int m = iy >> 1, k2 = ix0 >> 1;
#pragma unroll
        for (int r = 0; r < 2; ++r) {
          const int oy = m + r;
          const bool rok = oy < Ho && (r == 0 || (iy & 1));
          const int o = (rok ? oy : m) * Wo + k2;
          typedef float f2 __attribute__((ext_vector_type(2)));
          const f2 ga2 = *reinterpret_cast<const f2*>(sGa + o), gm2 = *reinterpret_cast<const f2*>(sGm + o);
          const unsigned short t2 = *reinterpret_cast<const unsigned short*>(sArg + o);
#pragma unroll
          for (int c = 0; c < 2; ++c) {
            wa[r][c] = rok ? ga2[c] : 0.f;
            wm[r][c] = rok ? gm2[c] : 0.f;
            wt[r][c] = rok ? (unsigned char)(t2 >> (8 * c)) : 255;
          }
          const bool hok = rok && k2 + 2 < Wo;
          wa[r][2] = hok ? sGa[o + 2] : 0.f;
          wm[r][2] = hok ? sGm[o + 2] : 0.f;
          wt[r][2] = hok ? sArg[o + 2] : 255;
        }
#pragma unroll
        for (int t = 0; t < 4; ++t) {
          float v = 0.f;
#pragma unroll
          for (int r = 0; r < 2; ++r)
#pragma unroll
            for (int c = t / 2; c <= (t + 1) / 2; ++c) {
              v += wa[r][c];
              if (wt[r][c] == (iy - 2 * (m + r) + 1) * 3 + (t - 2 * c + 1)) v += wm[r][c];
            }
          g[t] += v;
        }
        f4* dst = reinterpret_cast<f4*>(a.gx + pb + q4);
        *dst = a.overwrite ? g : *dst + g;
        continue;
      }
      const int oy_lo = iy - 1 < 0 ? 0 : (iy - 1 + S - 1) / S, oy_hi = min((iy + 1) / S, Ho - 1);
#pragma unroll
      for (int t = 0; t < 4; ++t) {
        const int ix = ix0 + t;
        const int ox_lo = ix - 1 < 0 ? 0 : (ix - 1 + S - 1) / S, ox_hi = min((ix + 1) / S, Wo - 1);
        float v = 0.f;
        for (int oy = oy_lo; oy <= oy_hi; ++oy)
          for (int ox = ox_lo; ox <= ox_hi; ++ox) {
            const int o = oy * Wo + ox;
            v += sGa[o];
            if (sArg[o] == (iy - oy * S + 1) * 3 + (ix - ox * S + 1)) v += sGm[o];
          }
        g[t] += v;
      }
      f4* dst = reinterpret_cast<f4*>(a.gx + pb + q4);
      *dst = a.overwrite ? g : *dst + g;
    }
    KSTAMP(3);
    return;
  }
  for (int o = threadIdx.x; o < HWo; o += 256) {
    int oy = o / Wo, ox = o % Wo;
    if (a.ga.z) {
      int y0 = max(oy * S - 1, 0), y1 = min(oy * S + 1, H - 1);
      int x0 = max(ox * S - 1, 0), x1 = min(ox * S + 1, W - 1);
      sGa[o] = bn_bwd_val(a.ga, ob + o, ma, ia, wa, a1, a2) / (float)((y1 - y0 + 1) * (x1 - x0 + 1));
    } else {
      sGa[o] = 0.f;
    }
    if (a.gm.z) {
      sGm[o] = bn_bwd_val(a.gm, ob + o, mm, im, wm, m1, m2);
      sArg[o] = a.amax[ob + o];
    } else {
      sGm[o] = 0.f;
      sArg[o] = 255;
    }
  }
  __syncthreads();
  for (int q = threadIdx.x; q < H * W; q += 256) {
    int iy = q / W, ix = q % W;
    float g = 0.f;
    int oy_lo = iy - 1 < 0 ? 0 : (iy - 1 + S - 1) / S, oy_hi = min((iy + 1) / S, Ho - 1);
    int ox_lo = ix - 1 < 0 ? 0 : (ix - 1 + S - 1) / S, ox_hi = min((ix + 1) / S, Wo - 1);
    for (int oy = oy_lo; oy <= oy_hi; ++oy) {
      for (int ox = ox_lo; ox <= ox_hi; ++ox) {
        int o = oy * Wo + ox;
        g += sGa[o];
        int tap = (iy - oy * S + 1) * 3 + (ix - ox * S + 1);
        if (sArg[o] == tap) g += sGm[o];
      }
    }
    if (a.dout_id) g += wid * a.dout_id[(size_t)nc * H * W + q];
#pragma unroll
    for (int j = 0; j < 4; ++j)
      if (j < a.nextra) g += a.extra[j][(size_t)nc * H * W + q];
    if (a.overwrite) a.gx[(size_t)nc * H * W + q] = g;
    else a.gx[(size_t)nc * H * W + q] += g;
  }
}
template <int S>
__global__ void __launch_bounds__(256) pool_bwd_kernel(PoolBwdBatch bt) {
  pool_bwd_body<S>(bt.e[blockIdx.y], blockIdx.x);
}

template <bool V4>
__global__ void __launch_bounds__(256) pool_bwd_multi_kernel(PoolBwdBatch bt) {
  const PoolBwdArgs a = bt.e[blockIdx.y];
  if ((int)blockIdx.x >= a.N * a.C) return;
  if (a.S == 1) pool_bwd_body<1, V4>(a, blockIdx.x);
  else pool_bwd_body<2, V4>(a, blockIdx.x);
}


template <int K, int DIL, int S, bool PREBN, int C>
__device__ __forceinline__ void dw_bwd_plane_body(const DwBwdArgs& a, const int bx, const int nb, const int dbg) {
  constexpr int KK = K * K, PAD = (K - 1) / 2 * DIL, PO = (PAD + S - 1) / S, SH = S == 2 ? 1 : 0;
  const int H = a.H, W = a.W, Ho = a.Ho, Wo = a.Wo;
  const int G = a.C / C, grp = bx % G, nbx = bx / G, c0 = grp * C;
  const int n = nbx / nb, band = nbx - n * nb;
  const int BRi = H / nb, iy0 = band * BRi, nrow = BRi;
  const int oyA = (iy0 - PAD) >> SH;
  const int oyB = (iy0 + nrow - 1 + PAD) >> SH;
  const int ODR = oyB - oyA + 1, ODW = lds_pitch(Wo + 2 * PO), NP = nrow * W;
  const bool accum = !PREBN && !a.overwrite;
  extern __shared__ __attribute__((aligned(16))) float smem[];
  float* sWt = smem;
  float* sGW = smem + C * 25;
  float* sDD = smem + dwb_head_floats(C);
  float* sIn = sDD + C * ODR * ODW;
  float* sOld = sIn + C * NP;
  __shared__ float sMean[C], sInv[C], sRed[2 * C];
  const int tid = threadIdx.x, lane = tid & 63, wave = tid >> 6;
  KSTAMP(0);
  for (int i = tid; i < C * KK; i += 256) {
    sGW[i] = 0.f;
    sWt[i] = a.dw[c0 * KK + i];
  }
  if (tid < C) {
    if (PREBN) bn_coeffs(a.inbn, c0 + tid, sMean[tid], sInv[tid]);
    sRed[tid] = 0.f;
    sRed[C + tid] = 0.f;
  }
  if (PREBN) __syncthreads();
  KSTAMP(1);
  const float* ddn = a.dd + ((size_t)n * a.C + c0) * Ho * Wo;
  const size_t xn = ((size_t)n * a.C + c0) * H * W;
  const int va = max(oyA, 0), vb = min(oyB, Ho - 1), vrows = vb - va + 1;
  {
    const int q4 = vrows * Wo / 4;
#pragma unroll 4
    for (int i = tid; i < C * q4; i += 256) {
      const int c = i / q4, o = (i - c * q4) * 4, r = o / Wo, ox = o - r * Wo;
      const float4 v = *reinterpret_cast<const float4*>(ddn + ((size_t)c * Ho + va) * Wo + o);
      float* d = sDD + (c * ODR + va - oyA + r) * ODW + PO + ox;
      d[0] = v.x;
      d[1] = v.y;
      d[2] = v.z;
      d[3] = v.w;
    }
    for (int i = tid; i < C * ODR; i += 256) {
      const int c = i / ODR, oy = oyA + i - c * ODR;
      float* d = sDD + i * ODW;
      if (oy < 0 || oy >= Ho) {
        for (int q = 0; q < ODW; ++q) d[q] = 0.f;
      } else {
        for (int q = 0; q < PO; ++q) d[q] = d[PO + Wo + q] = 0.f;
      }
    }
  }
  {
    const int q4 = NP / 4;
#pragma unroll 4
    for (int i = tid; i < C * q4; i += 256) {
      const int c = i / q4, o = (i - c * q4) * 4;
      float4 v = xval4<PREBN>(a.x, xn + ((size_t)c * H + iy0) * W + o);
      if (PREBN) {
        const float m = sMean[c], iv = sInv[c];
        v.x = (v.x - m) * iv;
        v.y = (v.y - m) * iv;
        v.z = (v.z - m) * iv;
        v.w = (v.w - m) * iv;
      }
      v.x = fmaxf(v.x, 0.f);
      v.y = fmaxf(v.y, 0.f);
      v.z = fmaxf(v.z, 0.f);
      v.w = fmaxf(v.w, 0.f);
      *reinterpret_cast<float4*>(sIn + c * NP + o) = v;
    }
    if (accum) {
      const float* gsrc = a.gout + ((size_t)n * a.C + c0) * H * W;
#pragma unroll 4
      for (int i = tid; i < C * q4; i += 256) {
        const int c = i / q4, o = (i - c * q4) * 4;
        *reinterpret_cast<float4*>(sOld + c * NP + o) =
            *reinterpret_cast<const float4*>(gsrc + ((size_t)c * H + iy0) * W + o);
      }
    }
  }
  __syncthreads();
  KSTAMP(2);
  float st1[C], st2[C];
#pragma unroll
  for (int c = 0; c < C; ++c) st1[c] = st2[c] = 0.f;
  float* gn = a.gout + ((size_t)n * a.C + c0) * H * W;
  if (S == 1 && a.vin) {
    typedef float f4 __attribute__((ext_vector_type(4)));
    constexpr int NQ = (4 + 2 * PAD + 3) / 4;
    const int NQ4 = NP / 4;
    for (int j = tid; j < ((dbg & 1) ? 0 : C * NQ4); j += 256) {
      const int c = j / NQ4, p = (j - c * NQ4) * 4;
      const int r = p / W, ix = p - r * W, iy = iy0 + r;
      int srow[K];
#pragma unroll
      for (int k = 0; k < K; ++k) srow[k] = (iy + PAD - k * DIL - oyA) * ODW + ix;
      KEEP_WEIGHT_READS_LOCAL();
      const float* wk = sWt + c * KK;
      const float* dd = sDD + c * ODR * ODW;
      f4 ga = {0.f, 0.f, 0.f, 0.f};
#pragma unroll
      for (int ky = 0; ky < K; ++ky) {
        float v[4 * NQ];
#pragma unroll
        for (int q = 0; q < NQ; ++q) {
          const float4 t = *reinterpret_cast<const float4*>(dd + srow[ky] + 4 * q);
          v[4 * q] = t.x;
          v[4 * q + 1] = t.y;
          v[4 * q + 2] = t.z;
          v[4 * q + 3] = t.w;
        }
#pragma unroll
        for (int kx = 0; kx < K; ++kx) {
          const float w = wk[ky * K + kx];
          const int o = 2 * PAD - kx * DIL;
          ga.x += w * v[o];
          ga.y += w * v[o + 1];
          ga.z += w * v[o + 2];
          ga.w += w * v[o + 3];
        }
      }
      const int li = (c * nrow + r) * W + ix;
      const f4 act = *reinterpret_cast<const f4*>(sIn + li);
      const f4 g = {act.x > 0.f ? ga.x : 0.f, act.y > 0.f ? ga.y : 0.f, act.z > 0.f ? ga.z : 0.f,
                    act.w > 0.f ? ga.w : 0.f};
      f4* dst = reinterpret_cast<f4*>(gn + ((size_t)c * H + iy) * W + ix);
      if (PREBN) {
        *dst = g;
        const float t1 = (g.x + g.y) + (g.z + g.w);
        const float t2 = (g.x * act.x + g.y * act.y) + (g.z * act.z + g.w * act.w);
#pragma unroll
        for (int cc = 0; cc < C; ++cc)
          if (cc == c) {
            st1[cc] += t1;
            st2[cc] += t2;
          }
      } else {
        *dst = accum ? *reinterpret_cast<const f4*>(sOld + li) + g : g;
      }
    }
  }
  if constexpr (S == 2) {
    const int hw2 = W / 2, NPc = (nrow / 2) * hw2;
    for (int q = tid; q < ((dbg & 1) || !a.vin ? 0 : NP); q += 256) {
      const int cls = NPc % 64 == 0 ? __builtin_amdgcn_readfirstlane(q / NPc) : q / NPc;
      const int qq = q - cls * NPc, rr = qq / hw2, xx = qq - rr * hw2;
      const int r = 2 * rr + (cls >> 1), ix = 2 * xx + (cls & 1), iy = iy0 + r;
      const int iyc = iy0 + (cls >> 1), ixc = cls & 1;
      int srow[K], scol[K];
#pragma unroll
      for (int k = 0; k < K; ++k) {
        srow[k] = (((iy + PAD - k * DIL) >> 1) - oyA) * ODW;
        scol[k] = ((ix + PAD - k * DIL) >> 1) + PO;
      }
#pragma unroll
      for (int c = 0; c < C; ++c) {
        KEEP_WEIGHT_READS_LOCAL();
        const float* wk = sWt + c * KK;
        const float* dd = sDD + c * ODR * ODW;
        float ga = 0.f;
#pragma unroll
        for (int ky = 0; ky < K; ++ky) {
          if ((iyc + PAD - ky * DIL) & 1) continue;
#pragma unroll
          for (int kx = 0; kx < K; ++kx) {
            if ((ixc + PAD - kx * DIL) & 1) continue;
            ga += wk[ky * K + kx] * dd[srow[ky] + scol[kx]];
          }
        }
        const int li = (c * nrow + r) * W + ix;
        const float act = sIn[li];
        const size_t gi = ((size_t)c * H + iy) * W + ix;
        const float g = act > 0.f ? ga : 0.f;
        if (PREBN) {
          gn[gi] = g;
          st1[c] += g;
          st2[c] += g * act;
        } else {
          gn[gi] = accum ? sOld[li] + g : g;
        }
      }
    }
  }
  for (int p = tid; p < ((dbg & 1) || a.vin ? 0 : NP); p += 256) {
    const int r = p / W, ix = p - r * W, iy = iy0 + r;
    int srow[K], scol[K];
    float mrow[K], mcol[K];
#pragma unroll
    for (int k = 0; k < K; ++k) {
      const int t = iy + PAD - k * DIL, u = ix + PAD - k * DIL;
      srow[k] = ((t >> SH) - oyA) * ODW;
      scol[k] = (u >> SH) + PO;
      mrow[k] = (S == 1 || (t & 1) == 0) ? 1.f : 0.f;
      mcol[k] = (S == 1 || (u & 1) == 0) ? 1.f : 0.f;
    }
#pragma unroll
    for (int c = 0; c < C; ++c) {
      KEEP_WEIGHT_READS_LOCAL();
        const float* wk = sWt + c * KK;
      const float* dd = sDD + c * ODR * ODW;
      float ga = 0.f;
#pragma unroll
      for (int ky = 0; ky < K; ++ky) {
        float rowacc = 0.f;
#pragma unroll
        for (int kx = 0; kx < K; ++kx) {
          const float v = wk[ky * K + kx] * dd[srow[ky] + scol[kx]];
          rowacc += S == 1 ? v : mcol[kx] * v;
        }
        ga += S == 1 ? rowacc : mrow[ky] * rowacc;
      }
      const int li = (c * nrow + r) * W + ix;
      const float act = sIn[li];
      const size_t gi = ((size_t)c * H + iy) * W + ix;
      const float g = act > 0.f ? ga : 0.f;
      if (PREBN) {
        gn[gi] = g;
        st1[c] += g;
        st2[c] += g * act;
      } else {
        gn[gi] = accum ? sOld[li] + g : g;
      }
    }
  }
  if (PREBN && a.red) {
    float st[2 * C];
#pragma unroll
    for (int c = 0; c < C; ++c) st[c] = st1[c], st[C + c] = st2[c];
    const float v = wave_reduce_scatter<2 * C>(st);
    if ((lane & (32 / C - 1)) == 0) atomicAdd(sRed + wave_scatter_index<2 * C>(lane), v);
  }
  KSTAMP(3);
  if (a.gW && !(dbg & 2) && S == 1) {
    const int JB = C * K * nrow, W4 = W / 4;
    int XP = 1;
    while (XP * 2 * JB <= 256 && W4 % (XP * 2) == 0) XP *= 2;
    const int XW = W / XP;
    for (int j = tid; j < JB * XP; j += 256) {
      const int xp = j / JB, jj = j - xp * JB;
      const int c = jj / (K * nrow), rem = jj - c * K * nrow, ky = rem / nrow, r = rem - ky * nrow;
      const float* ddr = sDD + (c * ODR + iy0 + r + PAD - ky * DIL - oyA) * ODW + PO;
      const float* inr = sIn + c * NP + r * W;
      float acc[K];
#pragma unroll
      for (int kx = 0; kx < K; ++kx) acc[kx] = 0.f;
      for (int ix = xp * XW; ix < (xp + 1) * XW; ix += 4) {
        const float4 v = *reinterpret_cast<const float4*>(inr + ix);
        constexpr int NQ = (4 + 2 * PAD + 3) / 4;
        float dseg[4 * NQ];
#pragma unroll
        for (int q = 0; q < NQ; ++q) {
          const float4 t = *reinterpret_cast<const float4*>(ddr - PO + ix + 4 * q);
          dseg[4 * q] = t.x;
          dseg[4 * q + 1] = t.y;
          dseg[4 * q + 2] = t.z;
          dseg[4 * q + 3] = t.w;
        }
#pragma unroll
        for (int kx = 0; kx < K; ++kx) {
          const int o = 2 * PAD - kx * DIL;
          acc[kx] += v.x * dseg[o] + v.y * dseg[o + 1] + v.z * dseg[o + 2] + v.w * dseg[o + 3];
        }
      }
#pragma unroll
      for (int kx = 0; kx < K; ++kx) atomicAdd(sGW + c * KK + ky * K + kx, acc[kx]);
    }
  } else if (a.gW && !(dbg & 2)) {
    constexpr int JOBS = C * KK, T = JOBS >= 256 ? 1 : 256 / JOBS;
    for (int j = tid; j < JOBS * T; j += 256) {
      const int job = j / T, part = j - job * T;
      const int c = job / KK, tap = job - c * KK, ky = tap / K, kx = tap - ky * K;
      const float* dd = sDD + c * ODR * ODW;
      const float* in = sIn + c * NP;
      float acc = 0.f;
      for (int r = 0; r < nrow; ++r) {
        const int t = iy0 + r + PAD - ky * DIL;
        if (S == 2 && (t & 1)) continue;
        const float* ddr = dd + ((t >> SH) - oyA) * ODW + PO;
        const float* inr = in + r * W;
        for (int ix = part * S + ((S == 2) ? ((PAD - kx * DIL) & 1) : 0); ix < W; ix += T * S)
          acc += inr[ix] * ddr[(ix + PAD - kx * DIL) >> SH];
      }
      atomicAdd(sGW + job, acc);
    }
  }
  KSTAMP(4);
  __syncthreads();
  if (PREBN && a.red && tid < 2 * C)
    atomicAdd(a.red + rep_slot() * 2 * a.C + (tid < C ? c0 + tid : a.C + c0 + tid - C), (double)sRed[tid]);
  if (a.gW)
    for (int i = tid; i < C * KK; i += 256) atomicAdd(a.gW + (size_t)rep_slot() * a.gstride + c0 * KK + i, sGW[i]);
  KSTAMP(5);
}

template <int K, int DIL, int S, bool PREBN, int C>
__global__ void __launch_bounds__(256) dw_bwd_plane_kernel(DwBwdBatch bt, int nb, int dbg) {
  dw_bwd_plane_body<K, DIL, S, PREBN, C>(bt.e[blockIdx.y], blockIdx.x, nb, dbg);
  if (bt.tail.ctr) fold_tail(bt.tail);
}

#define DWB_CASE(KK, DD, SS, PB) \
  case dw_bwd_variant(KK, DD, SS, PB): dw_bwd_plane_body<KK, DD, SS, PB, C>(a, blockIdx.x, a.nbands, 0); break;
template <int C>
__global__ void __launch_bounds__(256) dw_bwd_plane_multi_kernel(DwBwdBatch bt) {
  const DwBwdArgs a = bt.e[blockIdx.y];
  if ((int)blockIdx.x < a.nblk) {
    switch (a.variant) {
      DWB_CASE(3, 1, 1, true) DWB_CASE(5, 1, 1, true)
      DWB_CASE(3, 1, 1, false) DWB_CASE(3, 1, 2, false) DWB_CASE(5, 1, 1, false) DWB_CASE(5, 1, 2, false)
      DWB_CASE(3, 2, 1, false) DWB_CASE(3, 2, 2, false) DWB_CASE(5, 2, 1, false) DWB_CASE(5, 2, 2, false)
      default: break;
    }
  }
  if (bt.tail.ctr) fold_tail(bt.tail);
}
#undef DWB_CASE

template <int K, int DIL, int S, int C>
__device__ __forceinline__ void edge_conv_part(const EdgeBwdArgs& a, const int v, const int n, const int c0,
                                               const int iy0, const int nrow, float* sDD, const float* sAct,
                                               float* sGX, float* sGW) {
  constexpr int KK = K * K, PAD = (K - 1) / 2 * DIL, PO = (PAD + S - 1) / S, SH = S == 2 ? 1 : 0;
  const int W = a.W, Ho = a.Ho, Wo = a.Wo, NP = nrow * W;
  const int oyA = (iy0 - PAD) >> SH, oyB = (iy0 + nrow - 1 + PAD) >> SH;
  const int ODR = oyB - oyA + 1, ODW = Wo + 2 * PO;
  const int tid = threadIdx.x;
  const float* ddn = a.dd[v] + ((size_t)n * a.C + c0) * Ho * Wo;
  const int va = max(oyA, 0), vb = min(oyB, Ho - 1), vrows = vb - va + 1;
  {
    const int q4 = vrows * Wo / 4;
#pragma unroll 4
    for (int i = tid; i < C * q4; i += 256) {
      const int c = i / q4, o = (i - c * q4) * 4, r = o / Wo, ox = o - r * Wo;
      const float4 f = *reinterpret_cast<const float4*>(ddn + ((size_t)c * Ho + va) * Wo + o);
      float* d = sDD + (c * ODR + va - oyA + r) * ODW + PO + ox;
      d[0] = f.x;
      d[1] = f.y;
      d[2] = f.z;
      d[3] = f.w;
    }
    for (int i = tid; i < C * ODR; i += 256) {
      const int c = i / ODR, oy = oyA + i - c * ODR;
      float* d = sDD + i * ODW;
      if (oy < 0 || oy >= Ho) {
        for (int q = 0; q < ODW; ++q) d[q] = 0.f;
      } else {
        for (int q = 0; q < PO; ++q) d[q] = d[PO + Wo + q] = 0.f;
      }
    }
    for (int i = tid; i < C * KK; i += 256) sGW[i] = 0.f;
  }
  __syncthreads();
  for (int p = tid; p < NP; p += 256) {
    const int r = p / W, ix = p - r * W, iy = iy0 + r;
    int srow[K], scol[K];
    float mrow[K], mcol[K];
#pragma unroll
    for (int k = 0; k < K; ++k) {
      const int t = iy + PAD - k * DIL, u = ix + PAD - k * DIL;
      srow[k] = ((t >> SH) - oyA) * ODW;
      scol[k] = (u >> SH) + PO;
      mrow[k] = (S == 1 || (t & 1) == 0) ? 1.f : 0.f;
      mcol[k] = (S == 1 || (u & 1) == 0) ? 1.f : 0.f;
    }
#pragma unroll
    for (int c = 0; c < C; ++c) {
      const float* wk = a.dw[v] + (c0 + c) * KK;
      const float* dd = sDD + c * ODR * ODW;
      float ga = 0.f;
#pragma unroll
      for (int ky = 0; ky < K; ++ky) {
        float rowacc = 0.f;
#pragma unroll
        for (int kx = 0; kx < K; ++kx) {
          const float t = wk[ky * K + kx] * dd[srow[ky] + scol[kx]];
          rowacc += S == 1 ? t : mcol[kx] * t;
        }
        ga += S == 1 ? rowacc : mrow[ky] * rowacc;
      }
      sGX[c * NP + p] += ga;
    }
  }
  if (a.gW[v]) {
    if (S == 1) {
      const int JB = C * K * nrow;
      for (int j = tid; j < JB; j += 256) {
        const int c = j / (K * nrow), rem = j - c * K * nrow, ky = rem / nrow, r = rem - ky * nrow;
        const float* ddr = sDD + (c * ODR + iy0 + r + PAD - ky * DIL - oyA) * ODW + PO;
        const float* inr = sAct + c * NP + r * W;
        float acc[K];
#pragma unroll
        for (int kx = 0; kx < K; ++kx) acc[kx] = 0.f;
        for (int ix = 0; ix < W; ix += 4) {
          const float4 f = *reinterpret_cast<const float4*>(inr + ix);
          float dseg[4 + 2 * PAD];
#pragma unroll
          for (int m = 0; m < 4 + 2 * PAD; ++m) dseg[m] = ddr[ix - PAD + m];
#pragma unroll
          for (int kx = 0; kx < K; ++kx) {
            const int o = 2 * PAD - kx * DIL;
            acc[kx] += f.x * dseg[o] + f.y * dseg[o + 1] + f.z * dseg[o + 2] + f.w * dseg[o + 3];
          }
        }
#pragma unroll
        for (int kx = 0; kx < K; ++kx) atomicAdd(sGW + c * KK + ky * K + kx, acc[kx]);
      }
    } else {
      constexpr int JOBS = C * KK, T = JOBS >= 256 ? 1 : 256 / JOBS;
      for (int j = tid; j < JOBS * T; j += 256) {
        const int job = j / T, part = j - job * T;
        const int c = job / KK, tap = job - c * KK, ky = tap / K, kx = tap - ky * K;
        const float* dd = sDD + c * ODR * ODW;
        const float* in = sAct + c * NP;
        float acc = 0.f;
        for (int r = 0; r < nrow; ++r) {
          const int t = iy0 + r + PAD - ky * DIL;
          if (t & 1) continue;
          const float* ddr = dd + ((t >> SH) - oyA) * ODW + PO;
          const float* inr = in + r * W;
          for (int ix = part * S + ((PAD - kx * DIL) & 1); ix < W; ix += T * S)
            acc += inr[ix] * ddr[(ix + PAD - kx * DIL) >> SH];
        }
        atomicAdd(sGW + job, acc);
      }
    }
  }
  __syncthreads();
  if (a.gW[v])
    for (int i = tid; i < C * KK; i += 256) atomicAdd(a.gW[v] + (size_t)rep_slot() * a.gstride[v] + c0 * KK + i, sGW[i]);
  __syncthreads();
}

template <int S, int C>
__device__ __forceinline__ void edge_bwd_body(const EdgeBwdArgs& a, const int bx) {
  const int H = a.H, W = a.W, Ho = a.Ho, Wo = a.Wo;
  const int G = a.C / C, grp = bx % G, nbx = bx / G, c0 = grp * C;
  const int n = nbx / a.nb, band = nbx - n * a.nb;
  const int nrow = H / a.nb, iy0 = band * nrow, NP = nrow * W;
  extern __shared__ __attribute__((aligned(16))) float smem[];
  float* sAct = smem;
  float* sGX = sAct + C * NP;
  float* sDD = sGX + C * NP;
  __shared__ float sGW[C * 25];
  __shared__ float sCo[C][10];
  const int tid = threadIdx.x;
  const float* xn = a.x + ((size_t)n * a.C + c0) * H * W;
  {
    const int q4 = NP / 4;
#pragma unroll 4
    for (int i = tid; i < C * q4; i += 256) {
      const int c = i / q4, o = (i - c * q4) * 4;
      float4 f = *reinterpret_cast<const float4*>(xn + ((size_t)c * H + iy0) * W + o);
      f.x = fmaxf(f.x, 0.f);
      f.y = fmaxf(f.y, 0.f);
      f.z = fmaxf(f.z, 0.f);
      f.w = fmaxf(f.w, 0.f);
      *reinterpret_cast<float4*>(sAct + c * NP + o) = f;
      *reinterpret_cast<float4*>(sGX + c * NP + o) = float4{0.f, 0.f, 0.f, 0.f};
    }
  }
  const bool pa = a.ga.z != nullptr, pm = a.gm.z != nullptr;
  if (tid < C) {
    float* co = sCo[tid];
    co[0] = 0.f; co[1] = 1.f; co[2] = 0.f; co[3] = 0.f; co[4] = 0.f; co[5] = 1.f; co[6] = 0.f; co[7] = 0.f;
    if (pa) {
      bn_coeffs(a.ga.bn, c0 + tid, co[0], co[1]);
      gs_means(a.ga, c0 + tid, co[2], co[3]);
    }
    if (pm) {
      bn_coeffs(a.gm.bn, c0 + tid, co[4], co[5]);
      gs_means(a.gm, c0 + tid, co[6], co[7]);
    }
    co[8] = pa && a.ga.w ? a.ga.w[a.ga.widx] : 1.f;
    co[9] = pm && a.gm.w ? a.gm.w[a.gm.widx] : 1.f;
  }
  __syncthreads();
  if (a.conv_mask & 1) edge_conv_part<3, 1, S, C>(a, 0, n, c0, iy0, nrow, sDD, sAct, sGX, sGW);
  if (a.conv_mask & 2) edge_conv_part<5, 1, S, C>(a, 1, n, c0, iy0, nrow, sDD, sAct, sGX, sGW);
  if (a.conv_mask & 4) edge_conv_part<3, 2, S, C>(a, 2, n, c0, iy0, nrow, sDD, sAct, sGX, sGW);
  if (a.conv_mask & 8) edge_conv_part<5, 2, S, C>(a, 3, n, c0, iy0, nrow, sDD, sAct, sGX, sGW);
  const int poA = max(0, (iy0 - 1 + S - 1) / S), poB = min(Ho - 1, (iy0 + nrow) / S);
  const int PR = poB - poA + 1, PP = PR * Wo;
  float* sGa = sDD;
  float* sGm = sDD + C * PP;
  unsigned char* sArg = reinterpret_cast<unsigned char*>(sDD + 2 * C * PP);
  if (pa || pm) {
    for (int i = tid; i < C * PP; i += 256) {
      const int c = i / PP, o = poA * Wo + (i - c * PP), oy = o / Wo, ox = o - oy * Wo;
      const size_t idx = ((size_t)n * a.C + c0 + c) * Ho * Wo + o;
      const float* co = sCo[c];
      float gav = 0.f, gmv = 0.f;
      unsigned char arg = 255;
      if (pa) {
        const int y0 = max(oy * S - 1, 0), y1 = min(oy * S + 1, H - 1);
        const int x0 = max(ox * S - 1, 0), x1 = min(ox * S + 1, W - 1);
        gav = bn_bwd_val(a.ga, idx, co[0], co[1], co[8], co[2], co[3]) / (float)((y1 - y0 + 1) * (x1 - x0 + 1));
      }
      if (pm) {
        gmv = bn_bwd_val(a.gm, idx, co[4], co[5], co[9], co[6], co[7]);
        arg = a.amax[idx];
      }
      sGa[i] = gav;
      sGm[i] = gmv;
      sArg[i] = arg;
    }
    __syncthreads();
  }
  const float wid = (a.dout_id && a.w && a.id_idx >= 0) ? a.w[a.id_idx] : 0.f;
  for (int p = tid; p < NP; p += 256) {
    const int r = p / W, ix = p - r * W, iy = iy0 + r;
    const int oy_lo = iy - 1 < 0 ? 0 : (iy - 1 + S - 1) / S, oy_hi = min((iy + 1) / S, Ho - 1);
    const int ox_lo = ix - 1 < 0 ? 0 : (ix - 1 + S - 1) / S, ox_hi = min((ix + 1) / S, Wo - 1);
#pragma unroll
    for (int c = 0; c < C; ++c) {
      float g = sAct[c * NP + p] > 0.f ? sGX[c * NP + p] : 0.f;
      if (pa || pm) {
        for (int oy = oy_lo; oy <= oy_hi; ++oy)
          for (int ox = ox_lo; ox <= ox_hi; ++ox) {
            const int o = c * PP + (oy - poA) * Wo + ox;
            g += sGa[o];
            if (sArg[o] == (iy - oy * S + 1) * 3 + (ix - ox * S + 1)) g += sGm[o];
          }
      }
      const size_t gi = ((size_t)n * a.C + c0 + c) * H * W + (size_t)iy * W + ix;
      if (a.dout_id) g += wid * a.dout_id[gi];
      a.gx[gi] = a.overwrite ? g : a.gx[gi] + g;
    }
  }
}

template <int C>
__global__ void __launch_bounds__(256) edge_bwd_kernel(EdgeBwdBatch bt) {
  const EdgeBwdArgs a = bt.e[blockIdx.y];
  if ((int)blockIdx.x >= a.nblk) return;
  if (a.S == 1) edge_bwd_body<1, C>(a, blockIdx.x);
  else edge_bwd_body<2, C>(a, blockIdx.x);
}

static size_t edge_bwd_floats(const EdgeBwdArgs& a, int nb, int CG) {
  const int nrow = a.H / nb, S = a.S, sh = S == 2 ? 1 : 0;
  auto fdiv = [sh](int v) { return v >= 0 ? v >> sh : -((-v + (1 << sh) - 1) >> sh); };
  size_t stage = 0;
  const int pads[4] = {1, 2, 2, 4};
  for (int v = 0; v < 4; ++v) {
    if (!(a.conv_mask & (1 << v))) continue;
    const int PAD = pads[v], PO = (PAD + S - 1) / S;
    const int ODR = fdiv(nrow - 1 + PAD) - fdiv(-PAD) + 2;
    stage = std::max(stage, (size_t)CG * ODR * (a.Wo + 2 * PO));
  }
  if (a.ga.z || a.gm.z) {
    const size_t PP = (size_t)(nrow / S + 3) * a.Wo;
    stage = std::max(stage, 2 * CG * PP + (CG * PP + 3) / 4);
  }
  return 2 * (size_t)CG * nrow * a.W + stage;
}

bool launch_edge_bwd(EdgeBwdBatch b, hipStream_t st) {
  if (b.n < 1) return true;
  const int C = b.e[0].C, N = b.e[0].N;
  if (!(C == 4 || (C % 8 == 0 && C <= kMaxC))) return false;
  const int CG = C == 4 ? 4 : 8, G = C / CG;
  int maxblk = 0;
  size_t lds = 0;
  for (int i = 0; i < b.n; ++i) {
    EdgeBwdArgs& a = b.e[i];
    if (a.C != C || a.N != N || a.H != a.Ho * a.S || a.W != a.Wo * a.S || a.W % 4 || a.Wo % 4) return false;
    uintptr_t bits = (uintptr_t)a.x;
    for (int v = 0; v < 4; ++v)
      if (a.conv_mask & (1 << v)) bits |= (uintptr_t)a.dd[v];
    if (bits & 15) return false;
    constexpr int lds_kb = 48;
    constexpr int min_wg = 1024;
    int nb = 1;
    while (nb < 32 && a.H % (2 * nb) == 0 &&
           (edge_bwd_floats(a, nb, CG) * 4 > (size_t)lds_kb * 1024 || N * nb * G * b.n < min_wg))
      nb *= 2;
    if (edge_bwd_floats(a, nb, CG) * 4 > 64 * 1024) return false;
    a.nb = nb;
    a.nblk = N * nb * G;
    maxblk = std::max(maxblk, a.nblk);
    lds = std::max(lds, edge_bwd_floats(a, nb, CG) * sizeof(float));
  }
  const dim3 grid(maxblk, b.n);
  if (CG == 4) hipLaunchKernelGGL(edge_bwd_kernel<4>, grid, dim3(256), lds, st, b);
  else hipLaunchKernelGGL(edge_bwd_kernel<8>, grid, dim3(256), lds, st, b);
  return true;
}

void launch_pool_bwd_multi(const PoolBwdBatch& b, hipStream_t st) {
  int maxblk = 0;
  size_t lds = 0;
  bool v4 = true;
  auto al = [](const void* p, uintptr_t m) { return p == nullptr || (reinterpret_cast<uintptr_t>(p) & (m - 1)) == 0; };
  for (int i = 0; i < b.n; ++i) {
    const PoolBwdArgs& a = b.e[i];
    maxblk = std::max(maxblk, a.N * a.C);
    lds = std::max(lds, sizeof(float) * 2 * a.Ho * a.Wo + a.Ho * a.Wo + 16);
    v4 = v4 && (a.Ho * a.Wo) % 4 == 0 && (a.H * a.W) % 4 == 0 && a.W % 4 == 0 && al(a.ga.g, 16) && al(a.gm.g, 16) &&
         al(a.ga.z, 4 * sizeof(zt)) && al(a.gm.z, 4 * sizeof(zt)) && al(a.amax, 4) && al(a.dout_id, 16) &&
         al(a.gx, 16) && (!a.ga.z || !a.gm.z || a.ga.g == a.gm.g);
    for (int j = 0; j < a.nextra; ++j) v4 = v4 && al(a.extra[j], 16);
  }
  KSTAMP_ARM(kStampPoolBwd, st)
  if (v4) hipLaunchKernelGGL(pool_bwd_multi_kernel<true>, dim3(maxblk, b.n), dim3(256), lds, st, b);
  else hipLaunchKernelGGL(pool_bwd_multi_kernel<false>, dim3(maxblk, b.n), dim3(256), lds, st, b);
  KSTAMP_DISARM(st)
}

static size_t dw_plane_floats(const DwBwdArgs& a, int K, int DIL, int S, int nb, bool accum, int C) {
  const int PAD = (K - 1) / 2 * DIL, PO = (PAD + S - 1) / S, sh = S == 2 ? 1 : 0, BRi = a.H / nb;
  auto fdiv = [sh](int v) { return v >= 0 ? v >> sh : -((-v + (1 << sh) - 1) >> sh); };
  const int ODR = fdiv(BRi - 1 + PAD) - fdiv(-PAD) + 2;
  return (size_t)dwb_head_floats(C) + (size_t)C * ODR * lds_pitch(a.Wo + 2 * PO) +
         (size_t)C * BRi * a.W * (accum ? 2 : 1);
}

template <int K, int DIL, int S, int C>
static void launch_dw_bwd_plane_t(const DwBwdBatch& b, bool prebn, hipStream_t st) {
  const DwBwdArgs& a = b.e[0];
  bool accum = false;
  for (int i = 0; i < b.n; ++i) accum |= !prebn && !b.e[i].overwrite;
  int nb = 1;
  const int G = a.C / C;
  while (nb < 8 && a.H % (2 * nb) == 0 &&
         (dw_plane_floats(a, K, DIL, S, nb, accum, C) * 4 > 40 * 1024 || a.N * nb * G * b.n < 1024))
    nb *= 2;
  const size_t lds = sizeof(float) * dw_plane_floats(a, K, DIL, S, nb, accum, C);
  dim3 grid(a.N * nb * G, b.n);
  constexpr int dbg = 0;
  if (prebn) hipLaunchKernelGGL((dw_bwd_plane_kernel<K, DIL, S, true, C>), grid, dim3(256), lds, st, b, nb, dbg);
  else hipLaunchKernelGGL((dw_bwd_plane_kernel<K, DIL, S, false, C>), grid, dim3(256), lds, st, b, nb, dbg);
}

static bool aligned16(const DwBwdBatch& b) {
  for (int i = 0; i < b.n; ++i)
    if (((uintptr_t)b.e[i].x | (uintptr_t)b.e[i].dd | (uintptr_t)b.e[i].gout) & 15) return false;
  return true;
}

static bool dw_plane_ok(const DwBwdBatch& b, int K, int DIL, int S) {
  const DwBwdArgs& a = b.e[0];
  return (a.C == 4 || a.C == 8 || (a.C % 16 == 0 && a.C <= kMaxC)) && a.H == a.Ho * S && a.W == a.Wo * S &&
         a.pad == (K - 1) / 2 * DIL && a.Wo % 4 == 0 && aligned16(b);
}

template <int K, int DIL, int S>
static void launch_dw_bwd_t(const DwBwdBatch& b, bool prebn, hipStream_t st) {
  const DwBwdArgs& a = b.e[0];
  if (dw_plane_ok(b, K, DIL, S)) {
    constexpr int grp = 4;
    if (a.C == 4 || grp == 4) return launch_dw_bwd_plane_t<K, DIL, S, 4>(b, prebn, st);
    if (a.C == 8 || grp == 8) return launch_dw_bwd_plane_t<K, DIL, S, 8>(b, prebn, st);
    return launch_dw_bwd_plane_t<K, DIL, S, 16>(b, prebn, st);
  }
  const int TR = 64 / a.Wo;
  const int r = (K - 1) / 2 * DIL, h = (r + S - 1) / S, OR = TR + 2 * h;
  const int IR = (TR - 1) * S + (K - 1) * DIL + 1;
  const int IW = (a.Wo - 1) * S + (K - 1) * DIL + 1;
  size_t lds = sizeof(float) * (a.chunk * OR * a.Wo + a.chunk * IR * IW + 4 * a.C + (a.gW ? a.C * K * K : 0));
  dim3 grid(per_edge_blocks(a.N * (a.Ho / TR), b.n), b.n);
  if (prebn) hipLaunchKernelGGL((dw_bwd_kernel<K, DIL, S, true>), grid, dim3(256), lds, st, b);
  else hipLaunchKernelGGL((dw_bwd_kernel<K, DIL, S, false>), grid, dim3(256), lds, st, b);
}

bool launch_dw_bwd_multi(DwBwdBatch b, hipStream_t st) {
  if (b.n < 1) return true;
  const DwBwdArgs& a0 = b.e[0];
  if (!(a0.C == 4 || a0.C == 8 || (a0.C % 16 == 0 && a0.C <= kMaxC)) || !aligned16(b)) return false;
  constexpr int grp = 4;
  const int C = (a0.C == 4 || grp == 4) ? 4 : 8;
  if (a0.C % C) return false;
  int maxblk = 0;
  size_t lds = 0;
  for (int i = 0; i < b.n; ++i) {
    DwBwdArgs& a = b.e[i];
    const int K = dw_variant_k(a.variant), DIL = dw_variant_dil(a.variant), S = dw_variant_s(a.variant);
    const bool prebn = dw_variant_prebn(a.variant);
    if (a.C != a0.C || a.H != a.Ho * S || a.W != a.Wo * S || a.pad != (K - 1) / 2 * DIL || a.Wo % 4 ||
        (prebn && (DIL != 1 || S != 1)) || (!prebn && !a.overwrite))
      return false;
    int nb = 1;
    const int G = a.C / C;
    constexpr int min_wg = 512;
    while (nb < 8 && a.H % (2 * nb) == 0 &&
           (dw_plane_floats(a, K, DIL, S, nb, false, C) * 4 > 40 * 1024 || a.N * nb * G * b.n < min_wg))
      nb *= 2;
    a.nbands = nb;
    a.nblk = a.N * nb * G;
    a.vin = S == 1 ? (vec_mask() >> (C == 4 ? 2 : 3)) & 1 : (vec_mask() >> 4) & 1;
    maxblk = std::max(maxblk, a.nblk);
    lds = std::max(lds, sizeof(float) * dw_plane_floats(a, K, DIL, S, nb, false, C));
  }
  KSTAMP_ARM(kStampDwBwd, st)
  if (C == 4) hipLaunchKernelGGL(dw_bwd_plane_multi_kernel<4>, dim3(maxblk, b.n), dim3(256), lds, st, b);
  else hipLaunchKernelGGL(dw_bwd_plane_multi_kernel<8>, dim3(maxblk, b.n), dim3(256), lds, st, b);
  KSTAMP_DISARM(st)
  return true;
}

void launch_dw_bwd(const DwBwdBatch& b, int K, int dil, int S, bool prebn, hipStream_t st) {
#define DISPATCH(KK, DD, SS) \
  if (K == KK && dil == DD && S == SS) return launch_dw_bwd_t<KK, DD, SS>(b, prebn, st);
  DISPATCH(3, 1, 1) DISPATCH(3, 1, 2) DISPATCH(5, 1, 1) DISPATCH(5, 1, 2)
  DISPATCH(3, 2, 1) DISPATCH(3, 2, 2) DISPATCH(5, 2, 1) DISPATCH(5, 2, 2)
#undef DISPATCH
}
void launch_pool_bwd(const PoolBwdBatch& b, int S, hipStream_t st) {
  const PoolBwdArgs& a = b.e[0];
  size_t lds = sizeof(float) * 2 * a.Ho * a.Wo + a.Ho * a.Wo + 16;
  dim3 grid(a.N * a.C, b.n);
  if (S == 1) hipLaunchKernelGGL(pool_bwd_kernel<1>, grid, dim3(256), lds, st, b);
  else hipLaunchKernelGGL(pool_bwd_kernel<2>, grid, dim3(256), lds, st, b);
}

}
```

### katib_amd/csrc/hip/darts_ops_fwd.hip

```cpp
#include "darts_ops_fwd_k.h"

namespace katib_hip {


template <int K, int DIL, int S, int C>
static void launch_dwpw_plane_t(const DwPwFwdBatch& b, bool prebn, hipStream_t st) {
  const DwPwFwdArgs& a = b.e[0];
  const int nb = a.chunk, BR = (a.Ho + nb - 1) / nb;
  const size_t lds = sizeof(float) * (plane_head_floats(C) + C * ((BR - 1) * S + (K - 1) * DIL + 1) * lds_pitch(a.W + 2 * a.pad));
  dim3 grid(a.N * nb, b.n);
  bool vec = a.W % 4 == 0;
  for (int i = 0; i < b.n; ++i) vec &= ((uintptr_t)b.e[i].x & 15) == 0;
  if (vec) {
    if (prebn) hipLaunchKernelGGL((dwpw_plane_kernel<K, DIL, S, true, C, true>), grid, dim3(256), lds, st, b);
    else hipLaunchKernelGGL((dwpw_plane_kernel<K, DIL, S, false, C, true>), grid, dim3(256), lds, st, b);
  } else {
    if (prebn) hipLaunchKernelGGL((dwpw_plane_kernel<K, DIL, S, true, C, false>), grid, dim3(256), lds, st, b);
    else hipLaunchKernelGGL((dwpw_plane_kernel<K, DIL, S, false, C, false>), grid, dim3(256), lds, st, b);
  }
}

static bool plane_ok(const DwPwFwdArgs& a) { return a.C == 4 || a.C == 8 || a.C == 16; }

template <int CI, int CO>
static bool try_pw_fwd_wave(const PwFwdBatch& b, hipStream_t st);

template <int K, int DIL, int S, int CG>
static bool try_dwpw_split_g(const DwPwFwdBatch& b, bool prebn, hipStream_t st, bool split16);

template <int K, int DIL, int S>
static bool try_dwpw_split(const DwPwFwdBatch& b, bool prebn, hipStream_t st) {
  const DwPwFwdArgs& a = b.e[0];
  constexpr bool split16 = true;
  constexpr int grp = 8;
  if (grp == 4) return try_dwpw_split_g<K, DIL, S, 4>(b, prebn, st, split16);
  if (grp == 8) return try_dwpw_split_g<K, DIL, S, 8>(b, prebn, st, split16);
  return try_dwpw_split_g<K, DIL, S, 16>(b, prebn, st, split16);
}

template <int K, int DIL, int S, int CG>
static bool try_dwpw_split_g(const DwPwFwdBatch& b, bool prebn, hipStream_t st, bool split16) {
  const DwPwFwdArgs& a = b.e[0];
  if (a.C % 16 != 0 || a.C > 64 || (a.C == 16 && !split16) ||
      (a.Ho * a.Wo) % 64 != 0 || a.W % 4 != 0)
    return false;
  for (int i = 0; i < b.n; ++i)
    if (((uintptr_t)b.e[i].x | (uintptr_t)b.e[i].d | (uintptr_t)b.e[i].z) & 15) return false;
  const int G = a.C / CG;
  int nb = std::max(1, std::min(a.Ho / 4, 2048 / std::max(a.N * b.n * G, 1)));
  auto band_bytes = [&](int v) {
    const int BR = (a.Ho + v - 1) / v;
    return ((size_t)plane_head_floats(CG) + (size_t)CG * ((BR - 1) * S + (K - 1) * DIL + 1) * lds_pitch(a.W + 2 * a.pad)) * sizeof(float);
  };
  while (band_bytes(nb) > 65536 && nb < a.Ho) ++nb;
  DwPwFwdBatch db = b;
  db.tail.ctr = nullptr;
  for (int i = 0; i < b.n; ++i) db.e[i].chunk = nb;
  dim3 grid(a.N * nb * G, b.n);
  const size_t lds = band_bytes(nb);
  if (prebn) hipLaunchKernelGGL((dwpw_plane_kernel<K, DIL, S, true, CG, true, false>), grid, dim3(256), lds, st, db);
  else hipLaunchKernelGGL((dwpw_plane_kernel<K, DIL, S, false, CG, true, false>), grid, dim3(256), lds, st, db);
  PwFwdBatch pb{};
  pb.n = b.n;
  pb.tail = b.tail;
  for (int i = 0; i < b.n; ++i) {
    const DwPwFwdArgs& e = b.e[i];
    PwFwdArgs& p = pb.e[i];
    p.x = e.d; p.pw = e.pw; p.z = e.z; p.stats = e.stats;
    p.N = e.N; p.Cin = e.C; p.Cout = e.C; p.CoutTotal = e.C; p.co_off = 0;
    p.H = e.Ho; p.W = e.Wo; p.Ho = e.Ho; p.Wo = e.Wo; p.S = 1; p.off = 0; p.relu = 0;
  }
  if (try_pw_fwd_wave<16, 16>(pb, st) || try_pw_fwd_wave<32, 32>(pb, st) || try_pw_fwd_wave<64, 64>(pb, st))
    return true;
  launch_pw_fwd(pb, st);
  return true;
}

template <int K, int DIL, int S>
static void launch_dwpw_fwd_t(const DwPwFwdBatch& b, bool prebn, hipStream_t st) {
  const DwPwFwdArgs& a = b.e[0];
  if (try_dwpw_split<K, DIL, S>(b, prebn, st)) return;
  if (plane_ok(a)) {
    if (a.C == 4) return launch_dwpw_plane_t<K, DIL, S, 4>(b, prebn, st);
    if (a.C == 8) return launch_dwpw_plane_t<K, DIL, S, 8>(b, prebn, st);
    return launch_dwpw_plane_t<K, DIL, S, 16>(b, prebn, st);
  }
  const int TR = 64 / a.Wo;
  const int IR = (TR - 1) * S + (K - 1) * DIL + 1;
  const int IW = (a.Wo - 1) * S + (K - 1) * DIL + 1;
  size_t lds = sizeof(float) * (a.C * 64 + a.chunk * IR * IW + 4 * a.C);
  dim3 grid(per_edge_blocks(a.N * (a.Ho / TR), b.n), b.n);
  if (prebn) hipLaunchKernelGGL((dwpw_fwd_kernel<K, DIL, S, true>), grid, dim3(256), lds, st, b);
  else hipLaunchKernelGGL((dwpw_fwd_kernel<K, DIL, S, false>), grid, dim3(256), lds, st, b);
}

void launch_dwpw_fwd(const DwPwFwdBatch& b, int K, int dil, int S, bool prebn, hipStream_t st) {
#define DISPATCH(KK, DD, SS) \
  if (K == KK && dil == DD && S == SS) return launch_dwpw_fwd_t<KK, DD, SS>(b, prebn, st);
  DISPATCH(3, 1, 1) DISPATCH(3, 1, 2) DISPATCH(5, 1, 1) DISPATCH(5, 1, 2)
  DISPATCH(3, 2, 1) DISPATCH(3, 2, 2) DISPATCH(5, 2, 1) DISPATCH(5, 2, 2)
#undef DISPATCH
}


static bool dwpw_multi_prep(DwPwMultiBatch& b, bool& fused, int& maxblk, size_t& lds) {
  const int C = b.e[0].C, N = b.e[0].N;
  constexpr bool split16 = true;
  fused = C == 4 || C == 8 || (C == 16 && !split16);
  const bool split = !fused && C % 16 == 0 && C <= 64;
  if (!fused && !split) return false;
  const int CG = fused ? C : 8, G = C / CG;
  maxblk = 0;
  lds = 0;
  for (int i = 0; i < b.n; ++i) {
    DwPwFwdArgs& a = b.e[i];
    if (a.C != C || a.N != N) return false;
    const int code = a.variant >> 2;
    const int K = (code & 4) ? 5 : 3, DIL = (code & 2) ? 2 : 1, S = (code & 1) ? 2 : 1;
    const bool aligned = ((((uintptr_t)a.x) | (uintptr_t)a.d | (uintptr_t)a.z) & 15) == 0;
    if (split && (!aligned || (a.Ho * a.Wo) % 64 != 0 || a.W % 4 != 0)) return false;
    int nb = std::max(1, std::min(a.Ho / 4, 512 / std::max(N * b.n * G, 1)));
    auto band_bytes = [&](int v) {
      const int BR = (a.Ho + v - 1) / v;
      return ((size_t)plane_head_floats(CG) + (size_t)CG * ((BR - 1) * S + (K - 1) * DIL + 1) * lds_pitch(a.W + 2 * a.pad)) * sizeof(float);
    };
    while (band_bytes(nb) > 65536 && nb < a.Ho) ++nb;
    a.chunk = nb;
    a.nblk = N * nb * G;
    const bool vec = a.W % 4 == 0 && (((uintptr_t)a.x) & 15) == 0;
    a.variant = (a.variant & ~1) | (vec ? 1 : 0);
    a.vout = (vec_mask() >> (CG == 4 ? 0 : 1)) & 1;
    maxblk = std::max(maxblk, a.nblk);
    lds = std::max(lds, band_bytes(nb));
  }
  return true;
}

bool launch_dwpw_multi(DwPwMultiBatch b, hipStream_t st) {
  if (b.n < 1) return true;
  const int C = b.e[0].C;
  bool fused;
  int maxblk;
  size_t lds;
  if (!dwpw_multi_prep(b, fused, maxblk, lds)) return false;
  const dim3 grid(maxblk, b.n);
  if (fused) {
    if (C == 4) launch_dwpw_plane_multi_t<4>(true, grid, lds, st, b);
    else if (C == 8) launch_dwpw_plane_multi_t<8>(true, grid, lds, st, b);
    else launch_dwpw_plane_multi_t<16>(true, grid, lds, st, b);
    return true;
  }
  {
    DwPwMultiBatch db = b;
    db.tail.ctr = nullptr;
    launch_dwpw_plane_multi_t<8>(false, grid, lds, st, db);
  }
  PwFwdBatch pb{};
  pb.n = b.n;
  pb.tail = b.tail;
  for (int i = 0; i < b.n; ++i) {
    const DwPwFwdArgs& e = b.e[i];
    PwFwdArgs& p = pb.e[i];
    p.x = e.d; p.pw = e.pw; p.z = e.z; p.stats = e.stats;
    p.N = e.N; p.Cin = e.C; p.Cout = e.C; p.CoutTotal = e.C; p.co_off = 0;
    p.H = e.Ho; p.W = e.Wo; p.Ho = e.Ho; p.Wo = e.Wo; p.S = 1; p.off = 0; p.relu = 0;
  }
  bool same_hw = true;
  for (int i = 1; i < b.n; ++i) same_hw &= b.e[i].Ho == b.e[0].Ho && b.e[i].Wo == b.e[0].Wo;
  if (same_hw && (try_pw_fwd_wave<16, 16>(pb, st) || try_pw_fwd_wave<32, 32>(pb, st) || try_pw_fwd_wave<64, 64>(pb, st)))
    return true;
  for (int i = 0; i < b.n; ++i) {
    PwFwdBatch one{};
    one.n = 1;
    one.tail = pb.tail;
    one.e[0] = pb.e[i];
    if (!(try_pw_fwd_wave<16, 16>(one, st) || try_pw_fwd_wave<32, 32>(one, st) || try_pw_fwd_wave<64, 64>(one, st)))
      launch_pw_fwd(one, st);
  }
  return true;
}

static bool pool_fwd_prep(PoolFwdArgs* e, int n, int& maxblk, size_t& lds) {
  bool v4 = true;
  auto al = [](const void* p, uintptr_t m) { return p == nullptr || (reinterpret_cast<uintptr_t>(p) & (m - 1)) == 0; };
  maxblk = 0;
  lds = 0;
  for (int i = 0; i < n; ++i) {
    PoolFwdArgs& a = e[i];
    a.nblk = a.C * channel_groups(a.N, a.C, n);
    maxblk = std::max(maxblk, a.nblk);
    v4 = v4 && a.W % 4 == 0 && a.Wo % 4 == 0 && (a.S == 1 || a.W == 2 * a.Wo) && al(a.x, 16) &&
         al(a.zavg, 4 * sizeof(zt)) && al(a.zmax, 4 * sizeof(zt)) && al(a.amax, 4);
  }
  return v4;
}

void launch_pool_fwd_multi(PoolFwdBatch b, hipStream_t st) {
  int maxblk;
  size_t lds;
  if (pool_fwd_prep(b.e, b.n, maxblk, lds))
    hipLaunchKernelGGL(pool_fwd_multi_kernel<true>, dim3(maxblk, b.n), dim3(256), lds, st, b);
  else hipLaunchKernelGGL(pool_fwd_multi_kernel<false>, dim3(maxblk, b.n), dim3(256), 0, st, b);
}

bool launch_dwpw_pool_multi(DwPwMultiBatch b, const PoolFwdBatch& pb, hipStream_t st) {
  constexpr bool off = false;
  if (off || b.n < 1 || pb.n < 1 || b.tail.ctr || pb.tail.ctr || b.n + pb.n > 65535) return false;
  const int C = b.e[0].C;
  bool fused;
  int maxblk;
  size_t lds;
  if (!dwpw_multi_prep(b, fused, maxblk, lds) || !fused || (C != 4 && C != 8)) return false;
  PoolFwdEntries pe{};
  pe.n = pb.n;
  for (int i = 0; i < pb.n; ++i) pe.e[i] = pb.e[i];
  int pblk;
  size_t plds;
  if (!pool_fwd_prep(pe.e, pe.n, pblk, plds)) return false;
  const dim3 grid(std::max(maxblk, pblk), b.n + pb.n);
  lds = std::max(lds, plds);
  if (C == 4) launch_dwpw_pool_t<4>(grid, lds, st, b, pe);
  else launch_dwpw_pool_t<8>(grid, lds, st, b, pe);
  return true;
}

template <int CI, int CO>
static bool try_pw_fwd_wave(const PwFwdBatch& b, hipStream_t st) {
  const PwFwdArgs& a = b.e[0];
  constexpr int BO = CO / 16;
  if (a.Cin != CI || a.Cout != CO || (a.Ho * a.Wo) % 64 != 0) return false;
  for (int e = 0; e < b.n; ++e) {
    const PwFwdArgs& x = b.e[e];
    const bool flat = !x.relu || (x.S == 1 && x.off == 0 && x.H == x.Ho && x.W == x.Wo);
    if ((((uintptr_t)x.z) | (flat ? (uintptr_t)x.x : 0)) & 15) return false;
  }
  const int chunks = a.N * a.Ho * a.Wo / 64;
  int ns = 1;
  while (BO % (2 * ns) == 0 && chunks * ns * b.n < 4096) ns *= 2;
  const int per_edge = std::max(1, std::min((chunks * ns + 3) / 4, max_blocks() / std::max(b.n, 1)));
  const dim3 grid(per_edge, b.n);
  if (ns == 1) hipLaunchKernelGGL((pw_fwd_wave_kernel<CI, CO, 1>), grid, dim3(256), 0, st, b);
  else if constexpr (BO % 2 == 0) {
    if (ns == 2) hipLaunchKernelGGL((pw_fwd_wave_kernel<CI, CO, 2>), grid, dim3(256), 0, st, b);
    else if constexpr (BO % 4 == 0) hipLaunchKernelGGL((pw_fwd_wave_kernel<CI, CO, 4>), grid, dim3(256), 0, st, b);
  }
  return true;
}

void launch_pw_fwd(const PwFwdBatch& b, hipStream_t st) {
  const PwFwdArgs& a = b.e[0];
  if (try_pw_fwd_wave<48, 16>(b, st) || try_pw_fwd_wave<48, 32>(b, st) || try_pw_fwd_wave<64, 32>(b, st) ||
      try_pw_fwd_wave<32, 16>(b, st) || try_pw_fwd_wave<16, 16>(b, st) || try_pw_fwd_wave<32, 32>(b, st) ||
      try_pw_fwd_wave<64, 64>(b, st) || try_pw_fwd_wave<128, 64>(b, st))
    return;
  size_t lds = sizeof(float) * (a.Cin * 64 + 2 * a.Cout);
  dim3 grid(per_edge_blocks(a.N * a.Ho * a.Wo / 64, b.n), b.n);
  hipLaunchKernelGGL(pw_fwd_kernel, grid, dim3(256), lds, st, b);
}

void launch_pool_fwd(const PoolFwdBatch& b, int S, hipStream_t st) {
  const PoolFwdArgs& a = b.e[0];
  dim3 grid(a.C * channel_groups(a.N, a.C, b.n), b.n);
  if (S == 1) hipLaunchKernelGGL(pool_fwd_kernel<1>, grid, dim3(256), 0, st, b);
  else hipLaunchKernelGGL(pool_fwd_kernel<2>, grid, dim3(256), 0, st, b);
}

}
```

### katib_amd/csrc/hip/darts_ops_fwd_k.h

```cpp
#pragma once
#include "darts_ops_dev.h"

namespace katib_hip {

template <int K, int DIL, int S, bool PREBN>
__global__ void __launch_bounds__(256) dwpw_fwd_kernel(DwPwFwdBatch bt) {
  const DwPwFwdArgs& a = bt.e[blockIdx.y];
  constexpr int P = 64;
  const int C = a.C, H = a.H, W = a.W, Ho = a.Ho, Wo = a.Wo;
  const int TR = P / Wo;
  const int tiles = Ho / TR;
  const int ntiles = a.N * tiles;
  const int pad = a.pad;
  const int IR = (TR - 1) * S + (K - 1) * DIL + 1;
  const int IW = (Wo - 1) * S + (K - 1) * DIL + 1;
  extern __shared__ __attribute__((aligned(16))) float smem[];
  float* sD = smem;
  float* sIn = smem + C * P;
  float* sMean = sIn + a.chunk * IR * IW;
  float* sInv = sMean + C;
  float* sStat = sInv + C;
  const int tid = threadIdx.x;
  const int wave = tid >> 6, lane = tid & 63;
  for (int c = tid; c < C; c += 256) {
    if (PREBN) bn_coeffs(a.inbn, c, sMean[c], sInv[c]);
    sStat[c] = 0.f;
    sStat[C + c] = 0.f;
  }
  __syncthreads();
  for (int t = blockIdx.x; t < ntiles; t += gridDim.x) {
    const int n = t / tiles, oy0 = (t % tiles) * TR;
    const int iy0 = oy0 * S - pad, ix0 = -pad;
    const size_t xin = (size_t)n * C * H * W;
    for (int c0 = 0; c0 < C; c0 += a.chunk) {
      const int cn = min(a.chunk, C - c0);
      const int tot = cn * IR * IW;
      #pragma unroll 4
      for (int i = tid; i < tot; i += 256) {
        int cc = i / (IR * IW), r = (i / IW) % IR, q = i % IW;
        int iy = iy0 + r, ix = ix0 + q, c = c0 + cc;
        float v = 0.f;
        if (iy >= 0 && iy < H && ix >= 0 && ix < W) {
          v = xval<PREBN>(a.x, xin + ((size_t)c * H + iy) * W + ix);
          if (PREBN) v = (v - sMean[c]) * sInv[c];
          v = fmaxf(v, 0.f);
        }
        sIn[i] = v;
      }
      __syncthreads();
      for (int i = tid; i < cn * P; i += 256) {
        const int cc = __builtin_amdgcn_readfirstlane(i / P);
        const int p = i % P;
        const int c = c0 + cc;
        int ty = p / Wo, tx = p % Wo;
        const float* wk = a.dw + c * K * K;
        const float* src = sIn + (cc * IR + ty * S) * IW + tx * S;
        float acc = 0.f;
#pragma unroll
        for (int ky = 0; ky < K; ++ky)
#pragma unroll
          for (int kx = 0; kx < K; ++kx) acc += wk[ky * K + kx] * src[ky * DIL * IW + kx * DIL];
        sD[c * P + p] = acc;
        zput(a.d + (((size_t)n * C + c) * Ho + oy0 + ty) * Wo + tx, acc);
      }
      __syncthreads();
    }
    if (a.use_mfma) {
      typedef float f4 __attribute__((ext_vector_type(4)));
      for (int cob = wave * 16; cob < C; cob += 64) {
        f4 acc[4] = {{0, 0, 0, 0}, {0, 0, 0, 0}, {0, 0, 0, 0}, {0, 0, 0, 0}};
        for (int k0 = 0; k0 < C; k0 += 4) {
          float av = a.pw[(cob + (lane & 15)) * C + k0 + (lane >> 4)];
#pragma unroll
          for (int pb = 0; pb < 4; ++pb) {
            float bv = sD[(k0 + (lane >> 4)) * P + pb * 16 + (lane & 15)];
            acc[pb] = __builtin_amdgcn_mfma_f32_16x16x4f32(av, bv, acc[pb], 0, 0, 0);
          }
        }
#pragma unroll
        for (int r = 0; r < 4; ++r) {
          int co = cob + (lane >> 4) * 4 + r;
          float s = 0.f, s2 = 0.f;
#pragma unroll
          for (int pb = 0; pb < 4; ++pb) {
            int p = pb * 16 + (lane & 15);
            float v = acc[pb][r];
            zput(a.z + (((size_t)n * C + co) * Ho + oy0 + p / Wo) * Wo + p % Wo, v);
            s += v;
            s2 += v * v;
          }
#pragma unroll
          for (int o = 8; o > 0; o >>= 1) {
            s += __shfl_xor(s, o, 64);
            s2 += __shfl_xor(s2, o, 64);
          }
          if ((lane & 15) == 0) {
            sStat[co] += s;
            sStat[C + co] += s2;
          }
        }
      }
    } else {
      for (int co = wave; co < C; co += 4) {
        const int cou = __builtin_amdgcn_readfirstlane(co);
        const float* wrow = a.pw + cou * C;
        float v = 0.f;
        for (int ci = 0; ci < C; ++ci) v += wrow[ci] * sD[ci * P + lane];
        zput(a.z + (((size_t)n * C + cou) * Ho + oy0 + lane / Wo) * Wo + lane % Wo, v);
        float s = wave_sum(v), s2 = wave_sum(v * v);
        if (lane == 0) {
          sStat[cou] += s;
          sStat[C + cou] += s2;
        }
      }
    }
    __syncthreads();
  }
  if (a.stats)
    for (int i = tid; i < 2 * C; i += 256) atomicAdd(a.stats + rep_slot() * 2 * C + i, (double)sStat[i]);
  if (bt.tail.ctr) fold_tail(bt.tail);
}

template <int K, int DIL, int S, bool PREBN, int C, bool VEC, bool PW>
__device__ __forceinline__ void dwpw_plane_body(const DwPwFwdArgs& a, const int bx) {
  constexpr int KK = K * K;
  const int H = a.H, W = a.W, Ho = a.Ho, Wo = a.Wo, pad = a.pad;
  const int nb = a.chunk, BR = (Ho + nb - 1) / nb;
  const int G = PW ? 1 : a.C / C, c0 = PW ? 0 : (bx % G) * C, nbx = PW ? bx : bx / G;
  const int n = nbx / nb, band = nbx - n * nb;
  const int oy0 = band * BR, oy1 = min(Ho, oy0 + BR);
  const int HP = (BR - 1) * S + (K - 1) * DIL + 1, WP = lds_pitch(W + 2 * pad), PL = HP * WP;
  const int iyb = oy0 * S - pad;
  extern __shared__ __attribute__((aligned(16))) float smem[];
  float* sWt = smem;
  float* sPw = smem + C * 25;
  float* sIn = smem + plane_head_floats(C);
  __shared__ float sMean[C], sInv[C], sStat[2 * C];
  const int tid = threadIdx.x, lane = tid & 63, wave = tid >> 6;
  KSTAMP(0);
  for (int i = tid; i < C * KK; i += 256) sWt[i] = a.dw[c0 * KK + i];
  if (PW)
    for (int i = tid; i < C * C; i += 256) sPw[i] = a.pw[i];
  if (PREBN) bn_coeffs_coop(a.inbn, c0, C, sMean, sInv);
  if (tid < C) {
    sStat[tid] = 0.f;
    sStat[C + tid] = 0.f;
  }
  if (PREBN) __syncthreads();
  KSTAMP(1);
  const size_t xin = ((size_t)n * a.C + c0) * H * W;
  if (VEC) {
    const int va = max(iyb, 0), vb = min(iyb + HP, H), q4 = (vb - va) * W / 4;
#pragma unroll 4
    for (int i = tid; i < C * q4; i += 256) {
      const int c = i / q4, o = (i - c * q4) * 4, r = o / W, ix = o - r * W;
      float4 v = xval4<PREBN>(a.x, xin + ((size_t)c * H + va) * W + o);
      if (PREBN) {
        const float m = sMean[c], iv = sInv[c];
        v.x = (v.x - m) * iv;
        v.y = (v.y - m) * iv;
        v.z = (v.z - m) * iv;
        v.w = (v.w - m) * iv;
      }
      float* d = sIn + (c * HP + va - iyb + r) * WP + pad + ix;
      d[0] = fmaxf(v.x, 0.f);
      d[1] = fmaxf(v.y, 0.f);
      d[2] = fmaxf(v.z, 0.f);
      d[3] = fmaxf(v.w, 0.f);
    }
    for (int i = tid; i < C * HP; i += 256) {
      const int iy = iyb + i % HP;
      float* d = sIn + i * WP;
      if (iy < 0 || iy >= H) {
        for (int q = 0; q < WP; ++q) d[q] = 0.f;
      } else {
        for (int q = 0; q < pad; ++q) d[q] = d[pad + W + q] = 0.f;
      }
    }
  } else {
#pragma unroll 4
    for (int row = wave; row < C * HP; row += 4) {
      const int c = row / HP, r = row - c * HP, iy = iyb + r;
      const bool rok = iy >= 0 && iy < H;
      const size_t src = xin + ((size_t)c * H + (rok ? iy : 0)) * W;
      for (int q = lane; q < WP; q += 64) {
        const int ix = q - pad;
        float v = 0.f;
        if (rok && ix >= 0 && ix < W) {
          v = xval<PREBN>(a.x, src + ix);
          if (PREBN) v = (v - sMean[c]) * sInv[c];
          v = fmaxf(v, 0.f);
        }
        sIn[row * WP + q] = v;
      }
    }
  }
  __syncthreads();
  KSTAMP(2);
  float st1[C], st2[C];
#pragma unroll
  for (int c = 0; c < C; ++c) st1[c] = st2[c] = 0.f;
  const int HWo = Ho * Wo;
  zt* dn = a.d + ((size_t)n * a.C + c0) * HWo;
  zt* zn = a.z + (size_t)n * C * HWo;
  const bool vout = VEC && Wo % 4 == 0 && a.vout;
  if (vout) {
    constexpr int SPAN = 3 * S + (K - 1) * DIL + 1, NQ = (SPAN + 3) / 4;
    for (int p = oy0 * Wo + 4 * tid; p < oy1 * Wo; p += 1024) {
      const int oy = p / Wo, ox0 = p - oy * Wo;
      zf4 d[C];
#pragma unroll
      for (int c = 0; c < C; ++c) {
        const float* src = sIn + c * PL + ((oy - oy0) * S) * WP + ox0 * S;
        KEEP_WEIGHT_READS_LOCAL();
        const float* wk = sWt + c * KK;
        zf4 acc = {0.f, 0.f, 0.f, 0.f};
#pragma unroll
        for (int ky = 0; ky < K; ++ky) {
          float v[4 * NQ];
#pragma unroll
          for (int q = 0; q < NQ; ++q) {
            const float4 t = *reinterpret_cast<const float4*>(src + ky * DIL * WP + 4 * q);
            v[4 * q] = t.x;
            v[4 * q + 1] = t.y;
            v[4 * q + 2] = t.z;
            v[4 * q + 3] = t.w;
          }
#pragma unroll
          for (int kx = 0; kx < K; ++kx) {
            const float w = wk[ky * K + kx];
            acc.x += w * v[kx * DIL];
            acc.y += w * v[kx * DIL + S];
            acc.z += w * v[kx * DIL + 2 * S];
            acc.w += w * v[kx * DIL + 3 * S];
          }
        }
        d[c] = acc;
        zst4(dn + (size_t)c * HWo + p, acc);
      }
      if (!PW) continue;
#pragma unroll
      for (int co = 0; co < C; ++co) {
        KEEP_WEIGHT_READS_LOCAL();
        zf4 z = {0.f, 0.f, 0.f, 0.f};
#pragma unroll
        for (int ci = 0; ci < C; ++ci) z += sPw[co * C + ci] * d[ci];
        zst4(zn + (size_t)co * HWo + p, z);
        st1[co] += (z.x + z.y) + (z.z + z.w);
        st2[co] += (z.x * z.x + z.y * z.y) + (z.z * z.z + z.w * z.w);
      }
    }
  }
  for (int p = oy0 * Wo + tid; p < (vout ? 0 : oy1 * Wo); p += 256) {
    const int oy = p / Wo, ox = p - oy * Wo;
    float d[C];
#pragma unroll
    for (int c = 0; c < C; ++c) {
      const float* src = sIn + c * PL + ((oy - oy0) * S) * WP + ox * S;
      KEEP_WEIGHT_READS_LOCAL();
        const float* wk = sWt + c * KK;
      float acc = 0.f;
#pragma unroll
      for (int ky = 0; ky < K; ++ky)
#pragma unroll
        for (int kx = 0; kx < K; ++kx) acc += wk[ky * K + kx] * src[ky * DIL * WP + kx * DIL];
      d[c] = acc;
      zput(dn + (size_t)c * HWo + p, acc);
    }
    if (!PW) continue;
#pragma unroll
    for (int co = 0; co < C; ++co) {
      KEEP_WEIGHT_READS_LOCAL();
      float z = 0.f;
#pragma unroll
      for (int ci = 0; ci < C; ++ci) z += sPw[co * C + ci] * d[ci];
      zput(zn + (size_t)co * HWo + p, z);
      st1[co] += z;
      st2[co] += z * z;
    }
  }
  KSTAMP(3);
  if (!PW || !a.stats) return;
  {
    float st[2 * C];
#pragma unroll
    for (int c = 0; c < C; ++c) st[c] = st1[c], st[C + c] = st2[c];
    const float v = wave_reduce_scatter<2 * C>(st);
    if ((lane & (32 / C - 1)) == 0) atomicAdd(sStat + wave_scatter_index<2 * C>(lane), v);
  }
  __syncthreads();
  if (tid < 2 * C) atomicAdd(a.stats + (bx % kRep) * 2 * C + tid, (double)sStat[tid]);
  KSTAMP(4);
}
template <int K, int DIL, int S, bool PREBN, int C, bool VEC, bool PW = true>
__global__ void __launch_bounds__(256) dwpw_plane_kernel(DwPwFwdBatch bt) {
  dwpw_plane_body<K, DIL, S, PREBN, C, VEC, PW>(bt.e[blockIdx.y], blockIdx.x);
  if (bt.tail.ctr) fold_tail(bt.tail);
}

#define DWPW_CASE(KK, DD, SS)                                                                      \
  case ((KK == 5) * 4 + (DD == 2) * 2 + (SS == 2)) * 4 + 0: dwpw_plane_body<KK, DD, SS, false, C, false, PW>(a, bx); break; \
  case ((KK == 5) * 4 + (DD == 2) * 2 + (SS == 2)) * 4 + 1: dwpw_plane_body<KK, DD, SS, false, C, true, PW>(a, bx); break;  \
  case ((KK == 5) * 4 + (DD == 2) * 2 + (SS == 2)) * 4 + 2: dwpw_plane_body<KK, DD, SS, true, C, false, PW>(a, bx); break;  \
  case ((KK == 5) * 4 + (DD == 2) * 2 + (SS == 2)) * 4 + 3: dwpw_plane_body<KK, DD, SS, true, C, true, PW>(a, bx); break;
template <int C, bool PW>
__global__ void __launch_bounds__(256) dwpw_plane_multi_kernel(DwPwMultiBatch bt) {
  const DwPwFwdArgs a = bt.e[blockIdx.y];
  const int bx = blockIdx.x;
  if (bx < a.nblk) {
    switch (a.variant) {
      DWPW_CASE(3, 1, 1) DWPW_CASE(3, 1, 2) DWPW_CASE(5, 1, 1) DWPW_CASE(5, 1, 2)
      DWPW_CASE(3, 2, 1) DWPW_CASE(3, 2, 2) DWPW_CASE(5, 2, 1) DWPW_CASE(5, 2, 2)
      default: break;
    }
  }
  if (bt.tail.ctr) fold_tail(bt.tail);
}



template <int CI, int CO, int NS = 1>
__global__ void __launch_bounds__(256) pw_fwd_wave_kernel(PwFwdBatch bt) {
  static_assert(CI % 16 == 0 && CO % 16 == 0 && CI <= 128 && CO <= 64 && (CO / 16) % NS == 0, "16-channel blocks");
  constexpr int BO = CO / 16 / NS, KS = CI / 4;
  typedef float f4 __attribute__((ext_vector_type(4)));
  const PwFwdArgs& a = bt.e[blockIdx.y];
  const int HWo = a.Ho * a.Wo, Wo = a.Wo;
  const int nchunks = a.N * HWo / 64;
  __shared__ float sStat[2 * CO];
  const int tid = threadIdx.x, wave = tid >> 6, lane = tid & 63, c16 = lane & 15, q = lane >> 4;
  for (int i = tid; i < 2 * CO; i += 256) sStat[i] = 0.f;
  __syncthreads();
  const int grp = (blockIdx.x * 4 + wave) % NS, cb0 = grp * BO * 16;
  float wA[BO][KS];
#pragma unroll
  for (int bo = 0; bo < BO; ++bo)
#pragma unroll
    for (int k = 0; k < KS; ++k) wA[bo][k] = a.pw[(cb0 + bo * 16 + c16) * CI + 4 * k + q];
  const bool flat = !a.relu || (a.S == 1 && a.off == 0 && a.H == a.Ho && a.W == a.Wo);
  const bool fr2 = a.S == 2 && a.H == 2 * a.Ho && a.W == 2 * a.Wo && a.W % 4 == 0 && a.off <= 1 &&
                   ((uintptr_t)a.x & 15) == 0;
  f4 s1[BO], s2[BO];
#pragma unroll
  for (int bo = 0; bo < BO; ++bo) s1[bo] = s2[bo] = f4{0.f, 0.f, 0.f, 0.f};
  for (int w = blockIdx.x * 4 + wave; w < nchunks * NS; w += gridDim.x * 4) {
    const int pix0 = (w / NS) * 64, n = pix0 / HWo, prem = pix0 - n * HWo;
    const int pp = prem + 4 * c16;
    f4 acc[BO][4];
#pragma unroll
    for (int bo = 0; bo < BO; ++bo)
#pragma unroll
      for (int t = 0; t < 4; ++t) acc[bo][t] = f4{0.f, 0.f, 0.f, 0.f};
#pragma unroll
    for (int k = 0; k < KS; ++k) {
      const int ci = 4 * k + q;
      f4 v;
      if (flat) {
        if (a.relu) {
          const size_t o = plane_off(n, ci, a.N, CI, a.xnodes, HWo) + pp;
          v = *reinterpret_cast<const f4*>(static_cast<const float*>(a.x) + o);
          v = f4{fmaxf(v.x, 0.f), fmaxf(v.y, 0.f), fmaxf(v.z, 0.f), fmaxf(v.w, 0.f)};
        } else {
          v = zld4(static_cast<const zt*>(a.x) + ((size_t)n * CI + ci) * HWo + pp);
        }
      } else if (fr2) {
        const float* plane = static_cast<const float*>(a.x) + plane_off(n, ci, a.N, CI, a.xnodes, (size_t)a.H * a.W);
        float v0, v1, v2, v3;
        fr2_pair(plane, a.W, Wo, a.off, pp, v0, v1);
        fr2_pair(plane, a.W, Wo, a.off, pp + 2, v2, v3);
        v = f4{v0, v1, v2, v3};
      } else {
#pragma unroll
        for (int t = 0; t < 4; ++t) {
          const int p = pp + t, oy = p / Wo, ox = p - oy * Wo, iy = oy * a.S + a.off, ix = ox * a.S + a.off;
          v[t] = (iy < a.H && ix < a.W)
                     ? fmaxf(static_cast<const float*>(a.x)[plane_off(n, ci, a.N, CI, a.xnodes, (size_t)a.H * a.W) +
                                                             (size_t)iy * a.W + ix], 0.f)
                     : 0.f;
        }
      }
#pragma unroll
      for (int bo = 0; bo < BO; ++bo)
#pragma unroll
        for (int t = 0; t < 4; ++t) acc[bo][t] = __builtin_amdgcn_mfma_f32_16x16x4f32(wA[bo][k], v[t], acc[bo][t], 0, 0, 0);
    }
#pragma unroll
    for (int bo = 0; bo < BO; ++bo)
#pragma unroll
      for (int r = 0; r < 4; ++r) {
        const f4 z = f4{acc[bo][0][r], acc[bo][1][r], acc[bo][2][r], acc[bo][3][r]};
        zst4(a.z + ((size_t)n * a.CoutTotal + a.co_off + cb0 + bo * 16 + 4 * q + r) * HWo + pp, z);
        s1[bo][r] += (z.x + z.y) + (z.z + z.w);
        s2[bo][r] += (z.x * z.x + z.y * z.y) + (z.z * z.z + z.w * z.w);
      }
  }
  if (a.stats) {
#pragma unroll
  for (int bo = 0; bo < BO; ++bo)
#pragma unroll
    for (int r = 0; r < 4; ++r) {
      float u = s1[bo][r], w = s2[bo][r];
#pragma unroll
      for (int o = 8; o > 0; o >>= 1) {
        u += __shfl_xor(u, o, 64);
        w += __shfl_xor(w, o, 64);
      }
      if (c16 == 0) {
        atomicAdd(sStat + cb0 + bo * 16 + 4 * q + r, u);
        atomicAdd(sStat + CO + cb0 + bo * 16 + 4 * q + r, w);
      }
    }
  __syncthreads();
  for (int i = tid; i < 2 * CO; i += 256) {
    const int hi = i >= CO;
    atomicAdd(a.stats + rep_slot() * 2 * a.CoutTotal + hi * a.CoutTotal + a.co_off + (i - hi * CO), (double)sStat[i]);
  }
  }
  if (bt.tail.ctr) fold_tail(bt.tail);
}

static __global__ void __launch_bounds__(256) pw_fwd_kernel(PwFwdBatch bt) {
  const PwFwdArgs& a = bt.e[blockIdx.y];
  constexpr int P = 64;
  const int Cin = a.Cin, Cout = a.Cout, H = a.H, W = a.W, Ho = a.Ho, Wo = a.Wo;
  const int HWo = Ho * Wo;
  const int ntiles = a.N * HWo / P;
  extern __shared__ __attribute__((aligned(16))) float smem[];
  float* sX = smem;
  float* sStat = sX + Cin * P;
  const int tid = threadIdx.x, wave = tid >> 6, lane = tid & 63;
  for (int i = tid; i < 2 * Cout; i += 256) sStat[i] = 0.f;
  for (int t = blockIdx.x; t < ntiles; t += gridDim.x) {
    const int pix0 = t * P;
    const int n = pix0 / HWo, prem = pix0 % HWo;
    #pragma unroll 4
    for (int i = tid; i < Cin * P; i += 256) {
      int ci = i / P, p = i % P;
      int pp = prem + p, oy = pp / Wo, ox = pp % Wo;
      int iy = oy * a.S + a.off, ix = ox * a.S + a.off;
      float v = 0.f;
      if (iy < H && ix < W) {
        const size_t xi = a.relu ? plane_off(n, ci, a.N, Cin, a.xnodes, (size_t)H * W) + (size_t)iy * W + ix
                                 : (((size_t)n * Cin + ci) * H + iy) * W + ix;
        v = a.relu ? fmaxf(static_cast<const float*>(a.x)[xi], 0.f) : z2f(static_cast<const zt*>(a.x)[xi]);
      }
      sX[i] = v;
    }
    __syncthreads();
    for (int co = wave; co < Cout; co += 4) {
      const int cou = __builtin_amdgcn_readfirstlane(co);
      const float* wrow = a.pw + cou * Cin;
      float v = 0.f;
      for (int ci = 0; ci < Cin; ++ci) v += wrow[ci] * sX[ci * P + lane];
      zput(a.z + ((size_t)n * a.CoutTotal + a.co_off + cou) * HWo + prem + lane, v);
      float s = wave_sum(v), s2 = wave_sum(v * v);
      if (lane == 0) {
        sStat[cou] += s;
        sStat[Cout + cou] += s2;
      }
    }
    __syncthreads();
  }
  if (a.stats)
    for (int i = tid; i < 2 * Cout; i += 256) {
      int hi = i >= Cout;
      atomicAdd(a.stats + rep_slot() * 2 * a.CoutTotal + hi * a.CoutTotal + a.co_off + (i - hi * Cout),
                (double)sStat[i]);
    }
  if (bt.tail.ctr) fold_tail(bt.tail);
}

template <int S, bool V4 = false>
__device__ __forceinline__ void pool_fwd_body(const PoolFwdArgs& a, const int bx, const int gx) {
  const int C = a.C, H = a.H, W = a.W, Ho = a.Ho, Wo = a.Wo;
  const int c = bx % C, g0 = bx / C, G = gx / C;
  float sa = 0, sa2 = 0, sm = 0, sm2 = 0;
  if constexpr (V4) {
    constexpr int WC = S == 1 ? 6 : 9;
    const int HWo = Ho * Wo;
    for (int n = g0; n < a.N; n += G) {
      const int nc = n * C + c;
      const float* xp = a.x + (size_t)nc * H * W;
      for (int o4 = threadIdx.x * 4; o4 < HWo; o4 += 1024) {
        const int oy = o4 / Wo, ox0 = o4 - oy * Wo, ib = ox0 * S;
        float win[3][WC];
        bool rv[3];
#pragma unroll
        for (int r = 0; r < 3; ++r) {
          const int iy = oy * S - 1 + r;
          rv[r] = iy >= 0 && iy < H;
          const float* row = xp + (size_t)(rv[r] ? iy : 0) * W;
          const float4 m0 = *reinterpret_cast<const float4*>(row + ib);
          win[r][1] = m0.x;
          win[r][2] = m0.y;
          win[r][3] = m0.z;
          win[r][4] = m0.w;
          if (S == 1) {
            win[r][5] = ib + 4 < W ? row[ib + 4] : 0.f;
          } else {
            const float4 m1 = *reinterpret_cast<const float4*>(row + ib + 4);
            win[r][5] = m1.x;
            win[r][6] = m1.y;
            win[r][7] = m1.z;
            win[r][8] = m1.w;
          }
          win[r][0] = ib > 0 ? row[ib - 1] : 0.f;
        }
        const bool lv = ib > 0, hv = S == 2 || ib + 4 < W;
        zf4 av, mv;
        unsigned args = 0;
#pragma unroll
        for (int t = 0; t < 4; ++t) {
          float sum = 0.f, mx = -INFINITY;
          int cnt = 0, arg = 0;
#pragma unroll
          for (int ky = 0; ky < 3; ++ky) {
            if (!rv[ky]) continue;
#pragma unroll
            for (int kx = 0; kx < 3; ++kx) {
              const int wc = t * S + kx;
              if ((wc == 0 && !lv) || (wc == WC - 1 && !hv)) continue;
              const float v = win[ky][wc];
              sum += v;
              cnt++;
              if (v > mx || v != v) {
                mx = v;
                arg = ky * 3 + kx;
              }
            }
          }
          av[t] = sum / (float)cnt;
          mv[t] = mx;
          args |= (unsigned)arg << (8 * t);
        }
        const size_t oo = (size_t)nc * HWo + o4;
        zst4(a.zavg + oo, av);
        zst4(a.zmax + oo, mv);
        if (a.amax) *reinterpret_cast<unsigned*>(a.amax + oo) = args;
        sa += (av.x + av.y) + (av.z + av.w);
        sa2 += (av.x * av.x + av.y * av.y) + (av.z * av.z + av.w * av.w);
        sm += (mv.x + mv.y) + (mv.z + mv.w);
        sm2 += (mv.x * mv.x + mv.y * mv.y) + (mv.z * mv.z + mv.w * mv.w);
      }
    }
  }
  for (int n = V4 ? a.N : g0; n < a.N; n += G) {
    const int nc = n * C + c;
    const float* xp = a.x + (size_t)nc * H * W;
    for (int o = threadIdx.x; o < Ho * Wo; o += 256) {
      int oy = o / Wo, ox = o % Wo;
      float sum = 0.f, mx = -INFINITY;
      int cnt = 0, arg = 0;
      for (int ky = 0; ky < 3; ++ky) {
        int iy = oy * S - 1 + ky;
        if (iy < 0 || iy >= H) continue;
        for (int kx = 0; kx < 3; ++kx) {
          int ix = ox * S - 1 + kx;
          if (ix < 0 || ix >= W) continue;
          float v = xp[iy * W + ix];
          sum += v;
          cnt++;
          if (v > mx || v != v) {
            mx = v;
            arg = ky * 3 + kx;
          }
        }
      }
      float av = sum / (float)cnt;
      zput(a.zavg + (size_t)nc * Ho * Wo + o, av);
      zput(a.zmax + (size_t)nc * Ho * Wo + o, mx);
      if (a.amax) a.amax[(size_t)nc * Ho * Wo + o] = (unsigned char)arg;
      sa += av;
      sa2 += av * av;
      sm += mx;
      sm2 += mx * mx;
    }
  }
  if (!a.stats_avg && !a.stats_max) return;
  __shared__ float red[4][4];
  int wave = threadIdx.x >> 6, lane = threadIdx.x & 63;
  {
    float v[4] = {sa, sa2, sm, sm2};
    const float t = wave_reduce_scatter<4>(v);
    if ((lane & 15) == 0) red[wave][wave_scatter_index<4>(lane)] = t;
  }
  __syncthreads();
  if (threadIdx.x < 4) {
    float t = red[0][threadIdx.x] + red[1][threadIdx.x] + red[2][threadIdx.x] + red[3][threadIdx.x];
    double* dst = threadIdx.x < 2 ? a.stats_avg : a.stats_max;
    if (dst) atomicAdd(dst + (bx % kRep) * 2 * C + (threadIdx.x & 1) * C + c, (double)t);
  }
}
template <int S>
__global__ void __launch_bounds__(256) pool_fwd_kernel(PoolFwdBatch bt) {
  pool_fwd_body<S>(bt.e[blockIdx.y], blockIdx.x, gridDim.x);
  if (bt.tail.ctr) fold_tail(bt.tail);
}

template <bool V4>
__global__ void __launch_bounds__(256) pool_fwd_multi_kernel(PoolFwdBatch bt) {
  const PoolFwdArgs a = bt.e[blockIdx.y];
  if ((int)blockIdx.x < a.nblk) {
    if (a.S == 1) pool_fwd_body<1, V4>(a, blockIdx.x, a.nblk);
    else pool_fwd_body<2, V4>(a, blockIdx.x, a.nblk);
  }
  if (bt.tail.ctr) fold_tail(bt.tail);
}


template <int C, bool PV4>
__global__ void __launch_bounds__(256) dwpw_pool_multi_kernel(DwPwMultiBatch bt, PoolFwdEntries pe) {
  constexpr bool PW = true;
  const int bx = blockIdx.x;
  if ((int)blockIdx.y < bt.n) {
    const DwPwFwdArgs a = bt.e[blockIdx.y];
    if (bx < a.nblk) {
      switch (a.variant) {
        DWPW_CASE(3, 1, 1) DWPW_CASE(3, 1, 2) DWPW_CASE(5, 1, 1) DWPW_CASE(5, 1, 2)
        DWPW_CASE(3, 2, 1) DWPW_CASE(3, 2, 2) DWPW_CASE(5, 2, 1) DWPW_CASE(5, 2, 2)
        default: break;
      }
    }
  } else {
    const PoolFwdArgs a = pe.e[blockIdx.y - bt.n];
    if (bx < a.nblk) {
      if (a.S == 1) pool_fwd_body<1, PV4>(a, bx, a.nblk);
      else pool_fwd_body<2, PV4>(a, bx, a.nblk);
    }
  }
}
#undef DWPW_CASE


template <int C>
void launch_dwpw_plane_multi_t(bool pw, dim3 grid, size_t lds, hipStream_t st, const DwPwMultiBatch& b);
template <int C>
void launch_dwpw_pool_t(dim3 grid, size_t lds, hipStream_t st, const DwPwMultiBatch& b, const PoolFwdEntries& pe);
template <>
void launch_dwpw_plane_multi_t<4>(bool pw, dim3 grid, size_t lds, hipStream_t st, const DwPwMultiBatch& b);
template <>
void launch_dwpw_plane_multi_t<8>(bool pw, dim3 grid, size_t lds, hipStream_t st, const DwPwMultiBatch& b);
template <>
void launch_dwpw_plane_multi_t<16>(bool pw, dim3 grid, size_t lds, hipStream_t st, const DwPwMultiBatch& b);
template <>
void launch_dwpw_pool_t<4>(dim3 grid, size_t lds, hipStream_t st, const DwPwMultiBatch& b, const PoolFwdEntries& pe);
template <>
void launch_dwpw_pool_t<8>(dim3 grid, size_t lds, hipStream_t st, const DwPwMultiBatch& b, const PoolFwdEntries& pe);

}
```

Measured before the change: 2.173 s.

## Tile stride-1 depthwise plane kernels into bank-conflict-free LDS cells

Adds a new LDS plane layout for stride-1 depthwise plane kernels. The pitch is changed so that each ds_read_b128 lane group covers one 8-row by 2-quad cell, and compile-time checks assert there are no bank conflicts for the DARTS shapes. Forward and backward input-gradient loops and the weight-gradient reduction are remapped to this cell order, and the weight-gradient reduction now uses wave shuffles instead of per-thread LDS atomics. It also flattens the multi-edge backward grid so edges are packed by block offset instead of a 2D grid, and raises the band LDS budget to 48KB. The risks are extra index arithmetic, more LDS per band, and relaxed tile checks.

```diff
diff --git a/katib_amd/csrc/hip/darts_bind.cpp b/katib_amd/csrc/hip/darts_bind.cpp
--- a/katib_amd/csrc/hip/darts_bind.cpp
+++ b/katib_amd/csrc/hip/darts_bind.cpp
@@ -2,6 +2,7 @@
 #include <c10/hip/HIPStream.h>
 
 #include "darts_ops.h"
+#include "darts_plane_layout.h"
 
 using namespace katib_hip;
 using at::Tensor;
@@ -179,7 +180,8 @@
   const int Ho = z.size(2), Wo = z.size(3);
   TORCH_CHECK(dw.numel() == C * K * K && pw.numel() == C * C, "weight shapes");
   TORCH_CHECK(z.size(0) == N && z.size(1) == C && d.sizes() == z.sizes(), "output shapes");
-  TORCH_CHECK(64 % Wo == 0 && Ho % (64 / Wo) == 0, "tile constraint: 64 % Wo == 0 and Ho % (64/Wo) == 0");
+  TORCH_CHECK(C == 4 || C == 8 || C == 16 || (64 % Wo == 0 && Ho % (64 / Wo) == 0),
+              "tile constraint: 64 % Wo == 0 and Ho % (64/Wo) == 0");
   TORCH_CHECK(C <= kMaxC, "C too large");
   TORCH_CHECK(Ho == (H + 2 * pad - dil * (K - 1) - 1) / S + 1, "output height mismatch");
   a.x = x.data_ptr(); a.dw = dw.data_ptr<float>(); a.pw = pw.data_ptr<float>();
@@ -193,7 +195,7 @@
     int nb = std::max(1, std::min(Ho / 4, 2048 / std::max(N * nentries, 1)));
     auto band_bytes = [&](int b) {
       const int BR = (Ho + b - 1) / b;
-      return (size_t)C * ((BR - 1) * S + (K - 1) * dil + 1) * (W + 2 * pad) * sizeof(float);
+      return (size_t)C * ((BR - 1) * S + (K - 1) * dil + 1) * plane_pitch(W + 2 * pad, S) * sizeof(float);
     };
     while (band_bytes(nb) > 65536 && nb < Ho) ++nb;
     a.chunk = nb;
@@ -561,12 +563,14 @@
     check_f32(dw, "dw"); check_f32(dd, "dd"); check_f32(gout, "gout");
     DwBwdArgs& a = bt.e[i];
     a.N = x.size(0); a.C = x.size(1); a.H = x.size(2); a.W = x.size(3); a.Ho = dd.size(2); a.Wo = dd.size(3);
-    TORCH_CHECK(64 % a.Wo == 0 && a.Ho % (64 / a.Wo) == 0, "tile constraint");
     TORCH_CHECK(a.H == a.Ho * S && a.W == a.Wo * S, "dw_bwd needs H == Ho*S");
     TORCH_CHECK(gout.sizes() == x.sizes(), "gout shape");
     TORCH_CHECK(dw.numel() == a.C * K * K && dd.size(1) == a.C, "dw_bwd weight / grad shapes");
     a.x = x.data_ptr(); a.dw = dw.data_ptr<float>(); a.dd = dd.data_ptr<float>();
     a.gout = gout.data_ptr<float>(); a.gW = ptr_or_null<float>(gW); a.red = ptr_or_null<double>(red);
+    const bool plane = (a.C == 4 || a.C == 8 || (a.C % 16 == 0 && a.C <= kMaxC)) && a.Wo % 4 == 0 &&
+                       (((uintptr_t)a.x | (uintptr_t)a.dd | (uintptr_t)a.gout) & 15) == 0;
+    TORCH_CHECK(plane || (64 % a.Wo == 0 && a.Ho % (64 / a.Wo) == 0), "tile constraint");
     check_grad_sink(gW, (int64_t)a.C * K * K, gstride);
     a.gstride = gstride;
     a.overwrite = overwrite;
diff --git a/katib_amd/csrc/hip/darts_ops.h b/katib_amd/csrc/hip/darts_ops.h
--- a/katib_amd/csrc/hip/darts_ops.h
+++ b/katib_amd/csrc/hip/darts_ops.h
@@ -122,6 +122,7 @@
   int overwrite;
   int variant, nbands, nblk;
   int vin = 0;
+  int blk0 = 0;
 };
 constexpr int dw_bwd_variant(int K, int dil, int S, bool prebn) {
   return (((K == 5) * 4 + (dil == 2) * 2 + (S == 2)) << 1) | (prebn ? 1 : 0);
diff --git a/katib_amd/csrc/hip/darts_ops_dev.h b/katib_amd/csrc/hip/darts_ops_dev.h
--- a/katib_amd/csrc/hip/darts_ops_dev.h
+++ b/katib_amd/csrc/hip/darts_ops_dev.h
@@ -7,6 +7,7 @@
 #include <cstdlib>
 
 #include "darts_ops.h"
+#include "darts_plane_layout.h"
 
 namespace katib_hip {
 
@@ -46,9 +47,6 @@
 #define KEEP_WEIGHT_READS_LOCAL() asm volatile("" ::: "memory")
 __host__ __device__ constexpr int plane_head_floats(int C) { return (C * 25 + C * C + 3) & ~3; }
 __host__ __device__ constexpr int dwb_head_floats(int C) { return (2 * C * 25 + 3) & ~3; }
-__host__ __device__ constexpr int lds_pitch(int w) {
-  return (((w + 3) & ~3) >> 2) & 1 ? ((w + 3) & ~3) : ((w + 3) & ~3) + 4;
-}
 int vec_mask();
 
 __device__ __forceinline__ void sum_replicas(const double* p, int rep, int rs, int off2, double& s, double& s2) {
diff --git a/katib_amd/csrc/hip/darts_ops_dwb.hip b/katib_amd/csrc/hip/darts_ops_dwb.hip
--- a/katib_amd/csrc/hip/darts_ops_dwb.hip
+++ b/katib_amd/csrc/hip/darts_ops_dwb.hip
@@ -404,14 +404,14 @@
   const int BRi = H / nb, iy0 = band * BRi, nrow = BRi;
   const int oyA = (iy0 - PAD) >> SH;
   const int oyB = (iy0 + nrow - 1 + PAD) >> SH;
-  const int ODR = oyB - oyA + 1, ODW = lds_pitch(Wo + 2 * PO), NP = nrow * W;
+  const int ODR = oyB - oyA + 1, ODW = plane_pitch(Wo + 2 * PO, S), PIN = plane_pitch(W, S), NP = nrow * W;
   const bool accum = !PREBN && !a.overwrite;
   extern __shared__ __attribute__((aligned(16))) float smem[];
   float* sWt = smem;
   float* sGW = smem + C * 25;
   float* sDD = smem + dwb_head_floats(C);
   float* sIn = sDD + C * ODR * ODW;
-  float* sOld = sIn + C * NP;
+  float* sOld = sIn + C * nrow * PIN;
   __shared__ float sMean[C], sInv[C], sRed[2 * C];
   const int tid = threadIdx.x, lane = tid & 63, wave = tid >> 6;
   KSTAMP(0);
@@ -452,10 +452,10 @@
     }
   }
   {
-    const int q4 = NP / 4;
+    const int q4 = NP / 4, w4 = W / 4;
 #pragma unroll 4
     for (int i = tid; i < C * q4; i += 256) {
-      const int c = i / q4, o = (i - c * q4) * 4;
+      const int c = i / q4, oq = i - c * q4, o = oq * 4, r = oq / w4, lo = (c * nrow + r) * PIN + (oq - r * w4) * 4;
       float4 v = xval4<PREBN>(a.x, xn + ((size_t)c * H + iy0) * W + o);
       if (PREBN) {
         const float m = sMean[c], iv = sInv[c];
@@ -468,14 +468,14 @@
       v.y = fmaxf(v.y, 0.f);
       v.z = fmaxf(v.z, 0.f);
       v.w = fmaxf(v.w, 0.f);
-      *reinterpret_cast<float4*>(sIn + c * NP + o) = v;
+      *reinterpret_cast<float4*>(sIn + lo) = v;
     }
     if (accum) {
       const float* gsrc = a.gout + ((size_t)n * a.C + c0) * H * W;
 #pragma unroll 4
       for (int i = tid; i < C * q4; i += 256) {
-        const int c = i / q4, o = (i - c * q4) * 4;
-        *reinterpret_cast<float4*>(sOld + c * NP + o) =
+        const int c = i / q4, oq = i - c * q4, o = oq * 4, r = oq / w4;
+        *reinterpret_cast<float4*>(sOld + (c * nrow + r) * PIN + (oq - r * w4) * 4) =
             *reinterpret_cast<const float4*>(gsrc + ((size_t)c * H + iy0) * W + o);
       }
     }
@@ -486,13 +486,16 @@
 #pragma unroll
   for (int c = 0; c < C; ++c) st1[c] = st2[c] = 0.f;
   float* gn = a.gout + ((size_t)n * a.C + c0) * H * W;
-  if (S == 1 && a.vin) {
+  const bool tiled = S == 1 && (W & 7) == 0;
+  const bool vin = a.vin && (S == 2 || tiled);
+  if (S == 1 && vin) {
     typedef float f4 __attribute__((ext_vector_type(4)));
     constexpr int NQ = (4 + 2 * PAD + 3) / 4;
-    const int NQ4 = NP / 4;
-    for (int j = tid; j < ((dbg & 1) ? 0 : C * NQ4); j += 256) {
-      const int c = j / NQ4, p = (j - c * NQ4) * 4;
-      const int r = p / W, ix = p - r * W, iy = iy0 + r;
+    const int npair = W >> 3, nrb = (nrow + kCellRows - 1) / kCellRows;
+    for (int j = 4 * wave + tile_cell(lane); j < ((dbg & 1) ? 0 : C * nrb * npair); j += kBlockCells) {
+      const TileItem it = tile_item(j, lane, nrb, npair);
+      if (it.row >= nrow) continue;
+      const int c = it.c, r = it.row, ix = 4 * it.quad, iy = iy0 + r;
       int srow[K];
 #pragma unroll
       for (int k = 0; k < K; ++k) srow[k] = (iy + PAD - k * DIL - oyA) * ODW + ix;
@@ -521,7 +524,7 @@
           ga.w += w * v[o + 3];
         }
       }
-      const int li = (c * nrow + r) * W + ix;
+      const int li = (c * nrow + r) * PIN + ix;
       const f4 act = *reinterpret_cast<const f4*>(sIn + li);
       const f4 g = {act.x > 0.f ? ga.x : 0.f, act.y > 0.f ? ga.y : 0.f, act.z > 0.f ? ga.z : 0.f,
                     act.w > 0.f ? ga.w : 0.f};
@@ -543,7 +546,7 @@
   }
   if constexpr (S == 2) {
     const int hw2 = W / 2, NPc = (nrow / 2) * hw2;
-    for (int q = tid; q < ((dbg & 1) || !a.vin ? 0 : NP); q += 256) {
+    for (int q = tid; q < ((dbg & 1) || !vin ? 0 : NP); q += 256) {
       const int cls = NPc % 64 == 0 ? __builtin_amdgcn_readfirstlane(q / NPc) : q / NPc;
       const int qq = q - cls * NPc, rr = qq / hw2, xx = qq - rr * hw2;
       const int r = 2 * rr + (cls >> 1), ix = 2 * xx + (cls & 1), iy = iy0 + r;
@@ -569,7 +572,7 @@
             ga += wk[ky * K + kx] * dd[srow[ky] + scol[kx]];
           }
         }
-        const int li = (c * nrow + r) * W + ix;
+        const int li = (c * nrow + r) * PIN + ix;
         const float act = sIn[li];
         const size_t gi = ((size_t)c * H + iy) * W + ix;
         const float g = act > 0.f ? ga : 0.f;
@@ -583,7 +586,7 @@
       }
     }
   }
-  for (int p = tid; p < ((dbg & 1) || a.vin ? 0 : NP); p += 256) {
+  for (int p = tid; p < ((dbg & 1) || vin ? 0 : NP); p += 256) {
     const int r = p / W, ix = p - r * W, iy = iy0 + r;
     int srow[K], scol[K];
     float mrow[K], mcol[K];
@@ -611,7 +614,7 @@
         }
         ga += S == 1 ? rowacc : mrow[ky] * rowacc;
       }
-      const int li = (c * nrow + r) * W + ix;
+      const int li = (c * nrow + r) * PIN + ix;
       const float act = sIn[li];
       const size_t gi = ((size_t)c * H + iy) * W + ix;
       const float g = act > 0.f ? ga : 0.f;
@@ -632,39 +635,55 @@
     if ((lane & (32 / C - 1)) == 0) atomicAdd(sRed + wave_scatter_index<2 * C>(lane), v);
   }
   KSTAMP(3);
-  if (a.gW && !(dbg & 2) && S == 1) {
-    const int JB = C * K * nrow, W4 = W / 4;
-    int XP = 1;
-    while (XP * 2 * JB <= 256 && W4 % (XP * 2) == 0) XP *= 2;
-    const int XW = W / XP;
-    for (int j = tid; j < JB * XP; j += 256) {
-      const int xp = j / JB, jj = j - xp * JB;
-      const int c = jj / (K * nrow), rem = jj - c * K * nrow, ky = rem / nrow, r = rem - ky * nrow;
-      const float* ddr = sDD + (c * ODR + iy0 + r + PAD - ky * DIL - oyA) * ODW + PO;
-      const float* inr = sIn + c * NP + r * W;
-      float acc[K];
-#pragma unroll
-      for (int kx = 0; kx < K; ++kx) acc[kx] = 0.f;
-      for (int ix = xp * XW; ix < (xp + 1) * XW; ix += 4) {
-        const float4 v = *reinterpret_cast<const float4*>(inr + ix);
-        constexpr int NQ = (4 + 2 * PAD + 3) / 4;
-        float dseg[4 * NQ];
-#pragma unroll
-        for (int q = 0; q < NQ; ++q) {
-          const float4 t = *reinterpret_cast<const float4*>(ddr - PO + ix + 4 * q);
-          dseg[4 * q] = t.x;
-          dseg[4 * q + 1] = t.y;
-          dseg[4 * q + 2] = t.z;
-          dseg[4 * q + 3] = t.w;
-        }
+  if (a.gW && !(dbg & 2) && tiled) {
+    constexpr int KP = K == 3 ? 4 : 8;
+    const int npair = W >> 3, nrb = (nrow + kCellRows - 1) / kCellRows;
+    const int xp = wgrad_parts(C * K * nrb, npair), ncell = C * K * nrb * xp;
+    const bool wave_job = ((nrb * xp) & 3) == 0;
+    for (int u0 = 4 * wave; u0 < ncell; u0 += kBlockCells) {
+      const int u = u0 + tile_cell(lane);
+      const WgradJob jb = wgrad_job(u, lane, K, nrb, xp);
+      float acc[KP];
+#pragma unroll
+      for (int kx = 0; kx < KP; ++kx) acc[kx] = 0.f;
+      if (u < ncell && jb.row < nrow) {
+        const float* ddr = sDD + (jb.c * ODR + iy0 + jb.row + PAD - jb.ky * DIL - oyA) * ODW;
+        const float* inr = sIn + (jb.c * nrow + jb.row) * PIN;
+        for (int ix = 4 * jb.q0; ix < W; ix += 8 * xp) {
+          const float4 v = *reinterpret_cast<const float4*>(inr + ix);
+          constexpr int NQ = (4 + 2 * PAD + 3) / 4;
+          float dseg[4 * NQ];
+#pragma unroll
+          for (int q = 0; q < NQ; ++q) {
+            const float4 t = *reinterpret_cast<const float4*>(ddr + ix + 4 * q);
+            dseg[4 * q] = t.x;
+            dseg[4 * q + 1] = t.y;
+            dseg[4 * q + 2] = t.z;
+            dseg[4 * q + 3] = t.w;
+          }
+#pragma unroll
+          for (int kx = 0; kx < K; ++kx) {
+            const int o = 2 * PAD - kx * DIL;
+            acc[kx] += v.x * dseg[o] + v.y * dseg[o + 1] + v.z * dseg[o + 2] + v.w * dseg[o + 3];
+          }
+        }
+      }
+      float* gw = sGW + jb.c * KK + jb.ky * K;
+      if (wave_job) {
+        const float sum = wave_reduce_scatter<KP>(acc);
+        const int kx = wave_scatter_index<KP>(lane);
+        if ((lane & (64 / KP - 1)) == 0 && kx < K) atomicAdd(gw + kx, sum);
+      } else {
 #pragma unroll
         for (int kx = 0; kx < K; ++kx) {
-          const int o = 2 * PAD - kx * DIL;
-          acc[kx] += v.x * dseg[o] + v.y * dseg[o + 1] + v.z * dseg[o + 2] + v.w * dseg[o + 3];
-        }
-      }
-#pragma unroll
-      for (int kx = 0; kx < K; ++kx) atomicAdd(sGW + c * KK + ky * K + kx, acc[kx]);
+          float v = acc[kx];
+          v += __shfl_xor(v, 1, 64);
+          v += __shfl_xor(v, 2, 64);
+          v += __shfl_xor(v, 12, 64);
+          v += __shfl_xor(v, 20, 64);
+          if ((lane & 27) == 0 && u < ncell) atomicAdd(gw + kx, v);
+        }
+      }
     }
   } else if (a.gW && !(dbg & 2)) {
     constexpr int JOBS = C * KK, T = JOBS >= 256 ? 1 : 256 / JOBS;
@@ -672,13 +691,13 @@
       const int job = j / T, part = j - job * T;
       const int c = job / KK, tap = job - c * KK, ky = tap / K, kx = tap - ky * K;
       const float* dd = sDD + c * ODR * ODW;
-      const float* in = sIn + c * NP;
+      const float* in = sIn + c * nrow * PIN;
       float acc = 0.f;
       for (int r = 0; r < nrow; ++r) {
         const int t = iy0 + r + PAD - ky * DIL;
         if (S == 2 && (t & 1)) continue;
         const float* ddr = dd + ((t >> SH) - oyA) * ODW + PO;
-        const float* inr = in + r * W;
+        const float* inr = in + r * PIN;
         for (int ix = part * S + ((S == 2) ? ((PAD - kx * DIL) & 1) : 0); ix < W; ix += T * S)
           acc += inr[ix] * ddr[(ix + PAD - kx * DIL) >> SH];
       }
@@ -688,9 +707,9 @@
   KSTAMP(4);
   __syncthreads();
   if (PREBN && a.red && tid < 2 * C)
-    atomicAdd(a.red + rep_slot() * 2 * a.C + (tid < C ? c0 + tid : a.C + c0 + tid - C), (double)sRed[tid]);
+    atomicAdd(a.red + (bx % kRep) * 2 * a.C + (tid < C ? c0 + tid : a.C + c0 + tid - C), (double)sRed[tid]);
   if (a.gW)
-    for (int i = tid; i < C * KK; i += 256) atomicAdd(a.gW + (size_t)rep_slot() * a.gstride + c0 * KK + i, sGW[i]);
+    for (int i = tid; i < C * KK; i += 256) atomicAdd(a.gW + (size_t)(bx % kRep) * a.gstride + c0 * KK + i, sGW[i]);
   KSTAMP(5);
 }
 
@@ -701,17 +720,19 @@
 }
 
 #define DWB_CASE(KK, DD, SS, PB) \
-  case dw_bwd_variant(KK, DD, SS, PB): dw_bwd_plane_body<KK, DD, SS, PB, C>(a, blockIdx.x, a.nbands, 0); break;
+  case dw_bwd_variant(KK, DD, SS, PB): dw_bwd_plane_body<KK, DD, SS, PB, C>(a, bx, a.nbands, 0); break;
 template <int C>
 __global__ void __launch_bounds__(256) dw_bwd_plane_multi_kernel(DwBwdBatch bt) {
-  const DwBwdArgs a = bt.e[blockIdx.y];
-  if ((int)blockIdx.x < a.nblk) {
-    switch (a.variant) {
-      DWB_CASE(3, 1, 1, true) DWB_CASE(5, 1, 1, true)
-      DWB_CASE(3, 1, 1, false) DWB_CASE(3, 1, 2, false) DWB_CASE(5, 1, 1, false) DWB_CASE(5, 1, 2, false)
-      DWB_CASE(3, 2, 1, false) DWB_CASE(3, 2, 2, false) DWB_CASE(5, 2, 1, false) DWB_CASE(5, 2, 2, false)
-      default: break;
-    }
+  int ei = 0;
+  for (int i = 1; i < bt.n; ++i)
+    if ((int)blockIdx.x >= bt.e[i].blk0) ei = i;
+  const DwBwdArgs a = bt.e[ei];
+  const int bx = blockIdx.x - a.blk0;
+  switch (a.variant) {
+    DWB_CASE(3, 1, 1, true) DWB_CASE(5, 1, 1, true)
+    DWB_CASE(3, 1, 1, false) DWB_CASE(3, 1, 2, false) DWB_CASE(5, 1, 1, false) DWB_CASE(5, 1, 2, false)
+    DWB_CASE(3, 2, 1, false) DWB_CASE(3, 2, 2, false) DWB_CASE(5, 2, 1, false) DWB_CASE(5, 2, 2, false)
+    default: break;
   }
   if (bt.tail.ctr) fold_tail(bt.tail);
 }
@@ -1008,12 +1029,16 @@
   KSTAMP_DISARM(st)
 }
 
+#ifndef KATIB_DWB_BAND_KB
+#define KATIB_DWB_BAND_KB 48
+#endif
+constexpr int kDwbBandKB = KATIB_DWB_BAND_KB;
 static size_t dw_plane_floats(const DwBwdArgs& a, int K, int DIL, int S, int nb, bool accum, int C) {
   const int PAD = (K - 1) / 2 * DIL, PO = (PAD + S - 1) / S, sh = S == 2 ? 1 : 0, BRi = a.H / nb;
   auto fdiv = [sh](int v) { return v >= 0 ? v >> sh : -((-v + (1 << sh) - 1) >> sh); };
   const int ODR = fdiv(BRi - 1 + PAD) - fdiv(-PAD) + 2;
-  return (size_t)dwb_head_floats(C) + (size_t)C * ODR * lds_pitch(a.Wo + 2 * PO) +
-         (size_t)C * BRi * a.W * (accum ? 2 : 1);
+  return (size_t)dwb_head_floats(C) + (size_t)C * ODR * plane_pitch(a.Wo + 2 * PO, S) +
+         (size_t)C * BRi * plane_pitch(a.W, S) * (accum ? 2 : 1);
 }
 
 template <int K, int DIL, int S, int C>
@@ -1024,7 +1049,7 @@
   int nb = 1;
   const int G = a.C / C;
   while (nb < 8 && a.H % (2 * nb) == 0 &&
-         (dw_plane_floats(a, K, DIL, S, nb, accum, C) * 4 > 40 * 1024 || a.N * nb * G * b.n < 1024))
+         (dw_plane_floats(a, K, DIL, S, nb, accum, C) * 4 > kDwbBandKB * 1024 || a.N * nb * G * b.n < 1024))
     nb *= 2;
   const size_t lds = sizeof(float) * dw_plane_floats(a, K, DIL, S, nb, accum, C);
   dim3 grid(a.N * nb * G, b.n);
@@ -1071,7 +1096,7 @@
   constexpr int grp = 4;
   const int C = (a0.C == 4 || grp == 4) ? 4 : 8;
   if (a0.C % C) return false;
-  int maxblk = 0;
+  int total = 0;
   size_t lds = 0;
   for (int i = 0; i < b.n; ++i) {
     DwBwdArgs& a = b.e[i];
@@ -1084,17 +1109,18 @@
     const int G = a.C / C;
     constexpr int min_wg = 512;
     while (nb < 8 && a.H % (2 * nb) == 0 &&
-           (dw_plane_floats(a, K, DIL, S, nb, false, C) * 4 > 40 * 1024 || a.N * nb * G * b.n < min_wg))
+           (dw_plane_floats(a, K, DIL, S, nb, false, C) * 4 > kDwbBandKB * 1024 || a.N * nb * G * b.n < min_wg))
       nb *= 2;
     a.nbands = nb;
     a.nblk = a.N * nb * G;
     a.vin = S == 1 ? (vec_mask() >> (C == 4 ? 2 : 3)) & 1 : (vec_mask() >> 4) & 1;
-    maxblk = std::max(maxblk, a.nblk);
+    a.blk0 = total;
+    total += a.nblk;
     lds = std::max(lds, sizeof(float) * dw_plane_floats(a, K, DIL, S, nb, false, C));
   }
   KSTAMP_ARM(kStampDwBwd, st)
-  if (C == 4) hipLaunchKernelGGL(dw_bwd_plane_multi_kernel<4>, dim3(maxblk, b.n), dim3(256), lds, st, b);
-  else hipLaunchKernelGGL(dw_bwd_plane_multi_kernel<8>, dim3(maxblk, b.n), dim3(256), lds, st, b);
+  if (C == 4) hipLaunchKernelGGL(dw_bwd_plane_multi_kernel<4>, dim3(total), dim3(256), lds, st, b);
+  else hipLaunchKernelGGL(dw_bwd_plane_multi_kernel<8>, dim3(total), dim3(256), lds, st, b);
   KSTAMP_DISARM(st)
   return true;
 }
diff --git a/katib_amd/csrc/hip/darts_ops_fwd.hip b/katib_amd/csrc/hip/darts_ops_fwd.hip
--- a/katib_amd/csrc/hip/darts_ops_fwd.hip
+++ b/katib_amd/csrc/hip/darts_ops_fwd.hip
@@ -7,7 +7,7 @@
 static void launch_dwpw_plane_t(const DwPwFwdBatch& b, bool prebn, hipStream_t st) {
   const DwPwFwdArgs& a = b.e[0];
   const int nb = a.chunk, BR = (a.Ho + nb - 1) / nb;
-  const size_t lds = sizeof(float) * (plane_head_floats(C) + C * ((BR - 1) * S + (K - 1) * DIL + 1) * lds_pitch(a.W + 2 * a.pad));
+  const size_t lds = sizeof(float) * (plane_head_floats(C) + C * ((BR - 1) * S + (K - 1) * DIL + 1) * plane_pitch(a.W + 2 * a.pad, S));
   dim3 grid(a.N * nb, b.n);
   bool vec = a.W % 4 == 0;
   for (int i = 0; i < b.n; ++i) vec &= ((uintptr_t)b.e[i].x & 15) == 0;
@@ -50,7 +50,7 @@
   int nb = std::max(1, std::min(a.Ho / 4, 2048 / std::max(a.N * b.n * G, 1)));
   auto band_bytes = [&](int v) {
     const int BR = (a.Ho + v - 1) / v;
-    return ((size_t)plane_head_floats(CG) + (size_t)CG * ((BR - 1) * S + (K - 1) * DIL + 1) * lds_pitch(a.W + 2 * a.pad)) * sizeof(float);
+    return ((size_t)plane_head_floats(CG) + (size_t)CG * ((BR - 1) * S + (K - 1) * DIL + 1) * plane_pitch(a.W + 2 * a.pad, S)) * sizeof(float);
   };
   while (band_bytes(nb) > 65536 && nb < a.Ho) ++nb;
   DwPwFwdBatch db = b;
@@ -122,7 +122,7 @@
     int nb = std::max(1, std::min(a.Ho / 4, 512 / std::max(N * b.n * G, 1)));
     auto band_bytes = [&](int v) {
       const int BR = (a.Ho + v - 1) / v;
-      return ((size_t)plane_head_floats(CG) + (size_t)CG * ((BR - 1) * S + (K - 1) * DIL + 1) * lds_pitch(a.W + 2 * a.pad)) * sizeof(float);
+      return ((size_t)plane_head_floats(CG) + (size_t)CG * ((BR - 1) * S + (K - 1) * DIL + 1) * plane_pitch(a.W + 2 * a.pad, S)) * sizeof(float);
     };
     while (band_bytes(nb) > 65536 && nb < a.Ho) ++nb;
     a.chunk = nb;
diff --git a/katib_amd/csrc/hip/darts_ops_fwd_k.h b/katib_amd/csrc/hip/darts_ops_fwd_k.h
--- a/katib_amd/csrc/hip/darts_ops_fwd_k.h
+++ b/katib_amd/csrc/hip/darts_ops_fwd_k.h
@@ -129,7 +129,7 @@
   const int G = PW ? 1 : a.C / C, c0 = PW ? 0 : (bx % G) * C, nbx = PW ? bx : bx / G;
   const int n = nbx / nb, band = nbx - n * nb;
   const int oy0 = band * BR, oy1 = min(Ho, oy0 + BR);
-  const int HP = (BR - 1) * S + (K - 1) * DIL + 1, WP = lds_pitch(W + 2 * pad), PL = HP * WP;
+  const int HP = (BR - 1) * S + (K - 1) * DIL + 1, WP = plane_pitch(W + 2 * pad, S), PL = HP * WP;
   const int iyb = oy0 * S - pad;
   extern __shared__ __attribute__((aligned(16))) float smem[];
   float* sWt = smem;
@@ -206,7 +206,16 @@
   const bool vout = VEC && Wo % 4 == 0 && a.vout;
   if (vout) {
     constexpr int SPAN = 3 * S + (K - 1) * DIL + 1, NQ = (SPAN + 3) / 4;
-    for (int p = oy0 * Wo + 4 * tid; p < oy1 * Wo; p += 1024) {
+    const bool tiled = S == 1 && (Wo & 7) == 0;
+    const int nrowo = oy1 - oy0, npair = Wo >> 3, nrb = (nrowo + kCellRows - 1) / kCellRows;
+    const int nit = tiled ? nrb * npair : nrowo * Wo / 4;
+    for (int j = tiled ? 4 * wave + tile_cell(lane) : tid; j < nit; j += tiled ? kBlockCells : 256) {
+      int p = oy0 * Wo + 4 * j;
+      if (tiled) {
+        const TileItem it = tile_item(j, lane, nrb, npair);
+        if (it.row >= nrowo) continue;
+        p = (oy0 + it.row) * Wo + 4 * it.quad;
+      }
       const int oy = p / Wo, ox0 = p - oy * Wo;
       zf4 d[C];
 #pragma unroll
diff --git a/katib_amd/csrc/hip/darts_plane_layout.h b/katib_amd/csrc/hip/darts_plane_layout.h
--- /dev/null
+++ b/katib_amd/csrc/hip/darts_plane_layout.h
@@ -0,0 +1,153 @@
+#pragma once
+#include <hip/hip_runtime.h>
+
+namespace katib_hip {
+
+__host__ __device__ constexpr int lds_pitch(int w) {
+  return (((w + 3) & ~3) >> 2) & 1 ? ((w + 3) & ~3) : ((w + 3) & ~3) + 4;
+}
+__host__ __device__ constexpr int tile_pitch(int w) {
+  const int q = (w + 3) >> 2;
+  return 4 * (q + ((2 - q) & 3));
+}
+__host__ __device__ constexpr int plane_pitch(int w, int S) { return S == 1 ? tile_pitch(w) : lds_pitch(w); }
+
+constexpr int kCellRows = 8, kCellLanes = 16, kWaveCells = 4, kBlockCells = 16;
+__host__ __device__ constexpr int tile_qlo(int lane) { return lane & 1; }
+__host__ __device__ constexpr int tile_row(int lane) { return ((lane >> 1) & 1) | (((lane >> 3) & 3) << 1); }
+__host__ __device__ constexpr int tile_cell(int lane) {
+  return (((lane >> 2) ^ (lane >> 3) ^ (lane >> 4)) & 1) | (((lane >> 5) & 1) << 1);
+}
+struct TileItem {
+  int c, row, quad;
+};
+__host__ __device__ constexpr TileItem tile_item(int u, int lane, int nrb, int npair) {
+  const int t = u / npair, pair = u - t * npair, c = t / nrb, rb = t - c * nrb;
+  return TileItem{c, rb * kCellRows + tile_row(lane), 2 * pair + tile_qlo(lane)};
+}
+struct WgradJob {
+  int c, ky, row, q0;
+};
+__host__ __device__ constexpr WgradJob wgrad_job(int u, int lane, int K, int nrb, int xp) {
+  const int t = u / xp, part = u - t * xp, t2 = t / nrb, rb = t - t2 * nrb, c = t2 / K, ky = t2 - c * K;
+  return WgradJob{c, ky, rb * kCellRows + tile_row(lane), 2 * part + tile_qlo(lane)};
+}
+__host__ __device__ constexpr int wgrad_parts(int cells, int npair) {
+  int best = 1, cost = ((cells + kBlockCells - 1) / kBlockCells) * npair;
+  for (int xp = 2; xp <= npair && npair % xp == 0; xp *= 2) {
+    const int c = ((cells * xp + kBlockCells - 1) / kBlockCells) * (npair / xp);
+    if (c < cost) best = xp, cost = c;
+  }
+  return best;
+}
+
+__host__ __device__ constexpr int b128_group(int lane) {
+  constexpr int set[8] = {0, 1, 1, 0, 1, 0, 0, 1};
+  return 2 * (lane >> 5) + set[(lane >> 2) & 7];
+}
+struct B128Groups {
+  int lane[4][16];
+};
+__host__ __device__ constexpr B128Groups b128_groups() {
+  B128Groups t{};
+  int n[4] = {0, 0, 0, 0};
+  for (int lane = 0; lane < 64; ++lane) t.lane[b128_group(lane)][n[b128_group(lane)]++] = lane;
+  return t;
+}
+__host__ __device__ constexpr int b128_multiplicity(const int (&addr)[64], const B128Groups& grp) {
+  int worst = 0;
+  for (int g = 0; g < 4; ++g) {
+    int first[16] = {}, cnt[16] = {};
+    for (int i = 0; i < 16; ++i) {
+      const int a = addr[grp.lane[g][i]];
+      if (a < 0) continue;
+      const int s = (a >> 2) & 15;
+      if (cnt[s] == 0) {
+        first[s] = a;
+        cnt[s] = 1;
+      } else if (a != first[s]) {
+        bool dup = false;
+        for (int j = 0; j < i; ++j) dup = dup || addr[grp.lane[g][j]] == a;
+        if (!dup) ++cnt[s];
+      }
+      worst = cnt[s] > worst ? cnt[s] : worst;
+    }
+  }
+  return worst;
+}
+__host__ __device__ constexpr int plane_worst_multiplicity(int K, int DIL, int W, int rows) {
+  const int PAD = (K - 1) / 2 * DIL, NQ = (4 + 2 * PAD + 3) / 4;
+  const int pd = tile_pitch(W + 2 * PAD), pi = tile_pitch(W), odr = rows + 2 * PAD;
+  const int nrb = (rows + kCellRows - 1) / kCellRows, npair = W / 8, C = 4;
+  const B128Groups grp = b128_groups();
+  int worst = 0;
+  for (int wave = 0; wave < 4; ++wave) {
+    for (int ky = 0; ky < K; ++ky)
+      for (int q = 0; q <= NQ; ++q) {
+        int addr[64] = {};
+        for (int lane = 0; lane < 64; ++lane) {
+          const int u = 4 * wave + tile_cell(lane);
+          const TileItem it = tile_item(u, lane, nrb, npair);
+          const bool on = u < C * nrb * npair && it.row < rows;
+          addr[lane] = !on ? -1
+                       : q < NQ ? (it.c * odr + it.row + 2 * PAD - ky * DIL) * pd + 4 * it.quad + 4 * q
+                                : (it.c * rows + it.row) * pi + 4 * it.quad;
+        }
+        const int m = b128_multiplicity(addr, grp);
+        worst = m > worst ? m : worst;
+      }
+    const int xp = wgrad_parts(C * K * nrb, npair);
+    for (int step = 0; step < npair / xp; ++step)
+      for (int q = 0; q <= NQ; ++q) {
+        int addr[64] = {};
+        for (int lane = 0; lane < 64; ++lane) {
+          const int u = 4 * wave + tile_cell(lane);
+          const WgradJob j = wgrad_job(u, lane, K, nrb, xp);
+          const bool on = u < C * K * nrb * xp && j.row < rows;
+          const int quad = j.q0 + 2 * xp * step;
+          addr[lane] = !on ? -1
+                       : q < NQ ? (j.c * odr + j.row + 2 * PAD - j.ky * DIL) * pd + 4 * quad + 4 * q
+                                : (j.c * rows + j.row) * pi + 4 * quad;
+        }
+        const int m = b128_multiplicity(addr, grp);
+        worst = m > worst ? m : worst;
+      }
+  }
+  return worst;
+}
+
+__host__ __device__ constexpr bool tile_groups_are_cells() {
+  for (int g = 0; g < 4; ++g) {
+    int cell = -1, mask = 0;
+    for (int lane = 0; lane < 64; ++lane) {
+      if (b128_group(lane) != g) continue;
+      if (cell >= 0 && cell != tile_cell(lane)) return false;
+      cell = tile_cell(lane);
+      mask |= 1 << (2 * tile_row(lane) + tile_qlo(lane));
+    }
+    if (mask != 0xffff) return false;
+  }
+  return true;
+}
+static_assert(tile_groups_are_cells(), "a ds_read_b128 lane group must be one 8-row x 2-quad cell");
+static_assert(tile_pitch(34) == 40 && tile_pitch(36) == 40 && tile_pitch(40) == 40 && tile_pitch(32) == 40 &&
+                  tile_pitch(18) == 24 && tile_pitch(20) == 24 && tile_pitch(24) == 24 && tile_pitch(16) == 24,
+              "stride-1 plane pitches of the 32- and 16-wide DARTS layers");
+#define PLANE_CONFLICT_FREE_AT(K, D, W, R) \
+  static_assert(plane_worst_multiplicity(K, D, W, R) == 1, \
+                "ds_read_b128 bank conflicts in a stride-1 plane kernel: (K, dil, W, band rows) = (" #K ", " #D ", " #W ", " #R ")")
+#define PLANE_CONFLICT_FREE(K, D)     \
+  PLANE_CONFLICT_FREE_AT(K, D, 32, 32); \
+  PLANE_CONFLICT_FREE_AT(K, D, 32, 16); \
+  PLANE_CONFLICT_FREE_AT(K, D, 32, 4);  \
+  PLANE_CONFLICT_FREE_AT(K, D, 16, 16); \
+  PLANE_CONFLICT_FREE_AT(K, D, 16, 8);  \
+  PLANE_CONFLICT_FREE_AT(K, D, 16, 2)
+PLANE_CONFLICT_FREE(3, 1);
+PLANE_CONFLICT_FREE(5, 1);
+PLANE_CONFLICT_FREE(3, 2);
+PLANE_CONFLICT_FREE(5, 2);
+#undef PLANE_CONFLICT_FREE_AT
+#undef PLANE_CONFLICT_FREE
+
+}
```

Measured after the change: 2.133 s (median of 6 runs). -1.9%, faster.
